# freudh/lbt

Measured on NVIDIA B200. Metric: quantized train imgs/sec, higher is better.
Workload: dtype s8/u8 mantissas, s32 accumulate (8-bit dfxp); fp32 master weights

## Files before the change

include/lbt.h:

```cpp
#ifndef LBT_H_
#define LBT_H_

#include <stddef.h>
#include <stdint.h>

#ifdef __cplusplus
extern "C" {
#endif

#define LBT_VERSION 100

enum lbt_status {
  LBT_OK = 0,
  LBT_EINVAL = -1,
  LBT_EUNSUPPORTED = -2,
  LBT_EARCH = -3,
  LBT_ECUDA = -4,
  LBT_EWORKSPACE = -5
};

enum lbt_round_mode {
  LBT_ROUND_NEAREST = 0,
  LBT_ROUND_STOCHASTIC_NOISE = 1,
  LBT_ROUND_STOCHASTIC_PHILOX = 2,
  LBT_STATS_MINMAX = 0x100
};

enum lbt_mant_kind {
  LBT_MANT_NONE = 0,
  LBT_MANT_S8 = 1,
  LBT_MANT_U8 = 2,
  LBT_MANT_S16 = 3,
  LBT_MANT_S9C3 = 4,
  LBT_MANT_PREPARED = 0x100
};

#define LBT_CNT_OVER 0
#define LBT_CNT_OVER_HALF 1
#define LBT_CNT_NUMEL 2
#define LBT_CNT_TICKET 3
#define LBT_CNT_WORDS 4

int lbt_version(void);
const char* lbt_strerror(int status);
const char* lbt_last_cuda_error(void);
uint64_t lbt_launch_count(void);

int lbt_quantize(const float* x, size_t n_outer, size_t n_inner, int bits, int32_t* integer_bits,
                 float target_overflow_rate, int mode, const float* noise, uint64_t seed,
                 uint64_t offset, const uint64_t* dev_step, float* out_fp32, void* out_mant,
                 int mant_kind, uint64_t* counters, int update_range, void* stream);

int lbt_noise_fill(float* u, size_t n_inner, uint64_t seed, uint64_t offset, const uint64_t* dev_step,
                   void* stream);

int lbt_update_ranges(int32_t* ranges, uint64_t* counters, const int32_t* bits, const float* target,
                      size_t n, void* stream);

int lbt_step_advance(uint64_t* dev_step, void* stream);

typedef struct lbt_qsite {
  int32_t bits;
  int32_t stats_minmax;
  const int32_t* ib;
  const float* noise;
  uint64_t seed, offset;
  const uint64_t* dev_step;
  uint64_t* counters;
} lbt_qsite;

enum lbt_gemm_epilogue {
  LBT_EPI_F32 = 0,
  LBT_EPI_ACC64 = 1
};

int lbt_gemm_i8(const void* A, int a_kind, size_t lda, const void* B, int b_kind, size_t ldb, size_t M,
                size_t N, size_t K, int epilogue, const int32_t* ibA, const int32_t* ibB, int exp_const,
                const float* bias, float* out_f32, int64_t* acc64, size_t ldc, int alpha, int k_splits,
                const lbt_qsite* q_out, int8_t* k_out, int64_t* sums, size_t rows_per_image, const float* addend,
                void* stream);

int lbt_gemm_i8_dual(const int8_t* A_hi, const uint8_t* A_lo, size_t lda, const void* B, int b_kind, size_t ldb, size_t M,
                     size_t N, size_t K, const int32_t* ibA, const int32_t* ibB, int exp_const, float* out_f32, size_t ldc,
                     const float* addend, void* stream);

int lbt_acc64_finalize(const int64_t* acc64, size_t n, const int32_t* ibA, const int32_t* ibB, int exp_const,
                       const float* add, float add_scale, float* out, void* stream);

int lbt_im2col_i8(const void* src, int src_kind, int N, int H, int W, int C, int OH, int OW, int kh, int kw,
                  int sh, int sw, int pad_top, int pad_left, int transposed, void* out, size_t ld,
                  void* stream);

int lbt_conv_i8_fprop(const void* src, int src_kind, int N, int H, int W, int C, const void* wp, int w_kind,
                      size_t ldw, int Cout, int kh, int kw, int sh, int sw, int pad_top, int pad_left, int OH,
                      int OW, const int32_t* ib_src, const int32_t* ib_w, int exp_const, const float* bias,
                      float* out, size_t ldc, const lbt_qsite* q_out, int8_t* k_out, int64_t* sums, const float* addend,
                      void* stream);

int lbt_conv_i8_fprop_dual(const int8_t* src_hi, const uint8_t* src_lo, int N, int H, int W, int C, const void* wp, int w_kind,
                           size_t ldw, int Cout, int kh, int kw, int pad_top, int pad_left, int OH, int OW,
                           const int32_t* ib_src, const int32_t* ib_w, int exp_const, float* out, size_t ldc,
                           const float* addend, void* stream);

int lbt_conv_i8_dgrad(const void* g, int g_kind, int N, int OH, int OW, int Cout, const void* wp, int w_kind,
                      size_t ldw, int Cin, int kh, int kw, int sh, int sw, int pad_top, int pad_left, int H, int W,
                      const int32_t* ib_g, const int32_t* ib_w, int exp_const, float* dx, size_t ldc, const float* addend,
                      void* stream);

int lbt_conv_i8_wgrad(const void* src, int src_kind, int N, int H, int W, int C, const void* g, int g_kind, int Cout,
                      int kh, int kw, int sh, int sw, int pad_top, int pad_left, int OH, int OW, int64_t* acc64,
                      int alpha, int k_splits, void* stream);

int lbt_conv_i8_wgrad_dual(const void* src, int src_kind, int N, int H, int W, int C, const int8_t* g_hi, const uint8_t* g_lo,
                           int Cout, int kh, int kw, int sh, int sw, int pad_top, int pad_left, int OH, int OW,
                           int64_t* acc64, int alpha, int k_splits, void* stream);

size_t lbt_stem_pack8_bytes(int N, int H, int OW);
int lbt_stem_pack8(const int8_t* x16, int N, int H, int W, int OW, int pad_left, int8_t* work8, void* stream);
int lbt_conv_i8_wgrad_c3(const int8_t* x16, int N, int H, int W, const void* g, int g_kind, int Cout, int kh, int kw,
                         int pad_top, int pad_left, int OH, int OW, int8_t* work8, int repack, int64_t* acc8, int alpha,
                         void* stream);

int lbt_split_s16(const int16_t* in, size_t n, int8_t* hi, uint8_t* lo, void* stream);

int lbt_transpose_i8(const void* in, size_t R, size_t C, size_t ld_in, void* out, size_t ld_out,
                     void* stream);

int lbt_colsum_i(const void* in, int kind, size_t R, size_t C, int64_t* acc64, void* stream);

typedef struct lbt_finalize_job {
  const int64_t* acc64;
  uint64_t n;
  const int32_t* ibA;
  const int32_t* ibB;
  int32_t exp_const;
  float add_scale;
  const float* add;
  float* out;
  uint64_t start;
} lbt_finalize_job;
int lbt_finalize_multi(const lbt_finalize_job* jobs_dev, size_t njobs, uint64_t total, void* stream);

typedef struct lbt_noise_job {
  float* u;
  uint64_t n;
  uint64_t offset;
  uint64_t start;
} lbt_noise_job;
int lbt_noise_fill_multi(const lbt_noise_job* jobs_dev, size_t njobs, uint64_t total_groups, uint64_t seed,
                         const uint64_t* dev_step, void* stream);

enum lbt_prep_layout { LBT_PREP_VECTOR = 0, LBT_PREP_CONV = 1, LBT_PREP_DENSE = 2 };
typedef struct lbt_prep_job {
  const float* x;
  uint64_t n_outer, n_inner;
  const int32_t* ib;
  uint64_t* counters;
  uint64_t offset;
  float* out_f32;
  int8_t* out_a;
  int8_t* out_b;
  uint64_t ld_a, ld_b;
  int32_t bits, layout;
  uint32_t kh, kw, Cin, Cout;
  int32_t c3pad, rot180;
  int32_t sh, sw;
} lbt_prep_job;
int lbt_param_prep(const lbt_prep_job* jobs_dev, const uint32_t* block_job_dev, const uint32_t* block_chunk_dev,
                   size_t nblocks, uint32_t chunk_elems, uint64_t seed, const uint64_t* dev_step, void* stream);

int lbt_sgd_momentum(float* w, float* accum, const float* grad, size_t n, float lr, const float* dev_lr,
                     float momentum, float grad_scale, void* stream);

int lbt_bn_fwd_quant_stats(const float* x, size_t n_outer, size_t n_inner, int C, int bits, const int32_t* ib,
                           const float* noise, uint64_t seed, uint64_t offset, const uint64_t* dev_step,
                           int8_t* k1, int64_t* sums, uint64_t* counters, int stats_minmax, void* stream);
int lbt_bn_fwd_apply(const int8_t* k1, size_t n_outer, size_t n_inner, int C, int bits1, const int32_t* ib1,
                     const int64_t* sums, float eps, int bits2, const int32_t* ib2, const float* noise2,
                     uint64_t seed, uint64_t offset2, const uint64_t* dev_step, uint64_t* counters2,
                     const float* gamma_q, const float* beta_q, const float* add, int relu, int8_t* k2,
                     float* out, float* batch_mean, float* batch_var, float* run_mean, float* run_var,
                     double momentum, int stats_minmax, const lbt_qsite* q_next, void* next_mant, int next_kind,
                     void* stream);
int lbt_bn_fwd_apply2(const int8_t* k1, size_t n_outer, size_t n_inner, int C, int bits1, const int32_t* ib1,
                      const int64_t* sums, float eps, int bits2, const int32_t* ib2, const float* noise2,
                      uint64_t seed, uint64_t offset2, const uint64_t* dev_step, uint64_t* counters2,
                      const float* gamma_q, const float* beta_q, const float* add, int relu, int8_t* k2,
                      float* out, float* batch_mean, float* batch_var, float* run_mean, float* run_var,
                      double momentum, int stats_minmax, const lbt_qsite* q_next, void* next_mant, int next_kind,
                      const lbt_qsite* q_next2, void* next_mant2, int next_kind2, void* stream);
int lbt_bn_fwd_apply_pooled(const int8_t* k1, size_t n_outer, int H, int W, int C, int bits1, const int32_t* ib1,
                            const int64_t* sums, float eps, int bits2, const int32_t* ib2, const float* noise2,
                            uint64_t seed, uint64_t offset2, const uint64_t* dev_step, uint64_t* counters2,
                            const float* gamma_q, const float* beta_q, int relu, int8_t* k2, float* run_mean,
                            float* run_var, double momentum, int stats_minmax, int k, int s, int pad_top, int pad_left,
                            int POH, int POW, float* pooled, uint8_t* pidx, const lbt_qsite* q_next, void* next_mant,
                            int next_kind, void* stream);
int lbt_bn_fwd_apply_running(const int8_t* k1, size_t n_outer, size_t n_inner, int C, int bits1, const int32_t* ib1,
                             const float* run_mean, const float* run_var, float eps, int bits2, const int32_t* ib2,
                             const float* noise2, uint64_t seed, uint64_t offset2, const uint64_t* dev_step,
                             uint64_t* counters2, const float* gamma_q, const float* beta_q, const float* add, int relu,
                             int8_t* k2, float* out, int stats_minmax, const lbt_qsite* q_next, void* next_mant,
                             int next_kind, const lbt_qsite* q_next2, void* next_mant2, int next_kind2, void* stream);
int lbt_bn_fwd_apply_running_pooled(const int8_t* k1, size_t n_outer, int H, int W, int C, int bits1, const int32_t* ib1,
                                    const float* run_mean, const float* run_var, float eps, int bits2, const int32_t* ib2,
                                    const float* noise2, uint64_t seed, uint64_t offset2, const uint64_t* dev_step,
                                    uint64_t* counters2, const float* gamma_q, const float* beta_q, int relu, int8_t* k2,
                                    int stats_minmax, int k, int s, int pad_top, int pad_left, int POH, int POW,
                                    float* pooled, uint8_t* pidx, const lbt_qsite* q_next, void* next_mant, int next_kind,
                                    void* stream);
int lbt_bn_bwd_quant_stats(const float* g, const float* out, int relu, const int8_t* k2, const int8_t* k1,
                           size_t n_outer, size_t n_inner, int C, int bits2, const int32_t* ib2,
                           const float* gamma_q, const float* beta_q, int bits_g2, const int32_t* ib_g2,
                           const float* noise_g2, uint64_t offset_g2, uint64_t* counters_g2, int bits_g1,
                           const int32_t* ib_g1, const float* noise_g1, uint64_t offset_g1,
                           uint64_t* counters_g1, uint64_t seed, const uint64_t* dev_step, float* d_add,
                           void* kg1, int64_t* sums, int stats_minmax, int kg1_kind, void* stream);
typedef struct lbt_pool_geom {
  const uint8_t* idx;
  int32_t H, W;
  int32_t k, s, pad_top, pad_left;
  int32_t OH, OW;
} lbt_pool_geom;
int lbt_bn_bwd_quant_stats_pooled(const float* g_pooled, const lbt_pool_geom* pool, int relu, const int8_t* k2,
                                  const int8_t* k1, size_t n_outer, size_t n_inner, int C, int bits2, const int32_t* ib2,
                                  const float* gamma_q, const float* beta_q, int bits_g2, const int32_t* ib_g2,
                                  const float* noise_g2, uint64_t offset_g2, uint64_t* counters_g2, int bits_g1,
                                  const int32_t* ib_g1, const float* noise_g1, uint64_t offset_g1,
                                  uint64_t* counters_g1, uint64_t seed, const uint64_t* dev_step, void* kg1,
                                  int64_t* sums, int stats_minmax, int kg1_kind, void* stream);
int lbt_bn_bwd_apply(const void* kg1, const int8_t* k1, size_t n_outer, size_t n_inner, int C, int bits1,
                     const int32_t* ib1, const int64_t* fwd_sums, float eps, int bits_g1, const int32_t* ib_g1,
                     const int64_t* bwd_sums, float* dx, const lbt_qsite* q_grad, int8_t* g_mant, int kg1_kind,
                     uint8_t* g_mant_lo, void* stream);

typedef struct lbt_bn_bwd_args {
  const float* g;
  const float* out;
  const int8_t* k2;
  const int8_t* k1;
  uint64_t n_outer, n_inner;
  int32_t C, relu;
  int32_t bits2, bits1;
  const int32_t* ib2;
  const int32_t* ib1;
  const float* gamma_q;
  const float* beta_q;
  lbt_qsite q_g2, q_g1;
  float* d_add;
  int64_t* bwd_sums;
  const int64_t* fwd_sums;
  float eps;
  int32_t has_q_grad;
  lbt_qsite q_grad;
  float* dx;
  int8_t* g_mant;
  uint64_t* barrier;
} lbt_bn_bwd_args;
int lbt_bn_bwd_fused(const lbt_bn_bwd_args* args, void* stream);

int lbt_maxpool_fwd(const float* x, int N, int H, int W, int C, int k, int s, int pad_top, int pad_left, int OH, int OW,
                    float* out, uint8_t* idx, void* stream);
int lbt_maxpool_bwd(const float* g, const uint8_t* idx, int N, int H, int W, int C, int k, int s, int pad_top,
                    int pad_left, int OH, int OW, float* dx, void* stream);

int lbt_avgpool_fwd(const float* x, int N, int H, int W, int C, int k, int s, int OH, int OW, float* out, void* stream);
int lbt_avgpool_bwd(const float* g, int N, int H, int W, int C, int k, int s, int OH, int OW, float* dx, void* stream);

int lbt_softmax_xent_fwd(const float* logits, const int64_t* labels, int B, int C, float* probs, float* loss, void* stream);
int lbt_softmax_xent_bwd(const float* probs, const int64_t* labels, const float* grad_loss, int B, int C, float* dlogits,
// ... 65 lines not shown
```

lbt_b200/_lib.py:

```python
import ctypes
import os

import torch

_HERE = os.path.dirname(os.path.abspath(__file__))
LIB_PATH = os.environ.get('LBT_LIB') or os.path.join(_HERE, 'liblbt_b200.so')

c_void_p, c_int, c_size_t, c_float = ctypes.c_void_p, ctypes.c_int, ctypes.c_size_t, ctypes.c_float
c_u64, c_char_p = ctypes.c_uint64, ctypes.c_char_p

SIGNATURES = {
    'lbt_version': (c_int, []),
    'lbt_strerror': (c_char_p, [c_int]),
    'lbt_last_cuda_error': (c_char_p, []),
    'lbt_launch_count': (c_u64, []),
    'lbt_quantize': (c_int, [c_void_p, c_size_t, c_size_t, c_int, c_void_p, c_float, c_int, c_void_p, c_u64, c_u64,
                             c_void_p, c_void_p, c_void_p, c_int, c_void_p, c_int, c_void_p]),
    'lbt_noise_fill': (c_int, [c_void_p, c_size_t, c_u64, c_u64, c_void_p, c_void_p]),
    'lbt_update_ranges': (c_int, [c_void_p, c_void_p, c_void_p, c_void_p, c_size_t, c_void_p]),
    'lbt_step_advance': (c_int, [c_void_p, c_void_p]),
    'lbt_gemm_i8': (c_int, [c_void_p, c_int, c_size_t, c_void_p, c_int, c_size_t, c_size_t, c_size_t, c_size_t, c_int,
                            c_void_p, c_void_p, c_int, c_void_p, c_void_p, c_void_p, c_size_t, c_int, c_int,
                            c_void_p, c_void_p, c_void_p, c_size_t, c_void_p, c_void_p]),
    'lbt_gemm_i8_dual': (c_int, [c_void_p, c_void_p, c_size_t, c_void_p, c_int, c_size_t, c_size_t, c_size_t, c_size_t, c_void_p,
                                 c_void_p, c_int, c_void_p, c_size_t, c_void_p, c_void_p]),
    'lbt_acc64_finalize': (c_int, [c_void_p, c_size_t, c_void_p, c_void_p, c_int, c_void_p, c_float, c_void_p,
                                   c_void_p]),
    'lbt_im2col_i8': (c_int, [c_void_p, c_int] + [c_int] * 13 + [c_void_p, c_size_t, c_void_p]),
    'lbt_conv_i8_fprop': (c_int, [c_void_p, c_int, c_int, c_int, c_int, c_int, c_void_p, c_int, c_size_t] + [c_int] * 9 +
                          [c_void_p, c_void_p, c_int, c_void_p, c_void_p, c_size_t, c_void_p, c_void_p, c_void_p, c_void_p,
                           c_void_p]),
    'lbt_conv_i8_fprop_dual': (c_int, [c_void_p, c_void_p, c_int, c_int, c_int, c_int, c_void_p, c_int, c_size_t] + [c_int] * 7 +
                               [c_void_p, c_void_p, c_int, c_void_p, c_size_t, c_void_p, c_void_p]),
    'lbt_conv_i8_dgrad': (c_int, [c_void_p, c_int, c_int, c_int, c_int, c_int, c_void_p, c_int, c_size_t] + [c_int] * 9 +
                          [c_void_p, c_void_p, c_int, c_void_p, c_size_t, c_void_p, c_void_p]),
    'lbt_conv_i8_wgrad': (c_int, [c_void_p, c_int, c_int, c_int, c_int, c_int, c_void_p, c_int] + [c_int] * 9 +
                          [c_void_p, c_int, c_int, c_void_p]),
    'lbt_conv_i8_wgrad_dual': (c_int, [c_void_p, c_int, c_int, c_int, c_int, c_int, c_void_p, c_void_p] + [c_int] * 9 +
                               [c_void_p, c_int, c_int, c_void_p]),
    'lbt_stem_pack8_bytes': (c_size_t, [c_int, c_int, c_int]),
    'lbt_stem_pack8': (c_int, [c_void_p, c_int, c_int, c_int, c_int, c_int, c_void_p, c_void_p]),
    'lbt_conv_i8_wgrad_c3': (c_int, [c_void_p, c_int, c_int, c_int, c_void_p] + [c_int] * 8 + [c_void_p, c_int, c_void_p, c_int, c_void_p]),
    'lbt_split_s16': (c_int, [c_void_p, c_size_t, c_void_p, c_void_p, c_void_p]),
    'lbt_transpose_i8': (c_int, [c_void_p, c_size_t, c_size_t, c_size_t, c_void_p, c_size_t, c_void_p]),
    'lbt_colsum_i': (c_int, [c_void_p, c_int, c_size_t, c_size_t, c_void_p, c_void_p]),
    'lbt_bn_bwd_fused': (c_int, [c_void_p, c_void_p]),
    'lbt_maxpool_fwd': (c_int, [c_void_p] + [c_int] * 10 + [c_void_p, c_void_p, c_void_p]),
    'lbt_maxpool_bwd': (c_int, [c_void_p, c_void_p] + [c_int] * 10 + [c_void_p, c_void_p]),
    'lbt_avgpool_fwd': (c_int, [c_void_p] + [c_int] * 8 + [c_void_p, c_void_p]),
    'lbt_avgpool_bwd': (c_int, [c_void_p] + [c_int] * 8 + [c_void_p, c_void_p]),
    'lbt_softmax_xent_fwd': (c_int, [c_void_p, c_void_p, c_int, c_int, c_void_p, c_void_p, c_void_p]),
    'lbt_softmax_xent_bwd': (c_int, [c_void_p, c_void_p, c_void_p, c_int, c_int, c_void_p, c_void_p]),
    'lbt_relu': (c_int, [c_void_p, c_void_p, c_void_p, c_size_t, c_void_p]),
    'lbt_dropout': (c_int, [c_void_p, c_void_p, c_float, c_u64, c_u64, c_void_p, c_void_p, c_size_t, c_void_p]),
    'lbt_sgd_momentum': (c_int, [c_void_p, c_void_p, c_void_p, c_size_t, c_float, c_void_p, c_float, c_float,
                                 c_void_p]),
    'lbt_finalize_multi': (c_int, [c_void_p, c_size_t, c_u64, c_void_p]),
    'lbt_noise_fill_multi': (c_int, [c_void_p, c_size_t, c_u64, c_u64, c_void_p, c_void_p]),
    'lbt_param_prep': (c_int, [c_void_p, c_void_p, c_void_p, c_size_t, ctypes.c_uint32, c_u64, c_void_p, c_void_p]),
    'lbt_bn_fwd_quant_stats': (c_int, [c_void_p, c_size_t, c_size_t, c_int, c_int, c_void_p, c_void_p, c_u64, c_u64,
                                       c_void_p, c_void_p, c_void_p, c_void_p, c_int, c_void_p]),
    'lbt_bn_fwd_apply': (c_int, [c_void_p, c_size_t, c_size_t, c_int, c_int, c_void_p, c_void_p, c_float, c_int,
                                 c_void_p, c_void_p, c_u64, c_u64, c_void_p, c_void_p, c_void_p, c_void_p, c_void_p,
                                 c_int, c_void_p, c_void_p, c_void_p, c_void_p, c_void_p, c_void_p, ctypes.c_double, c_int,
                                 c_void_p, c_void_p, c_int, c_void_p]),
    'lbt_bn_fwd_apply2': (c_int, [c_void_p, c_size_t, c_size_t, c_int, c_int, c_void_p, c_void_p, c_float, c_int,
                                  c_void_p, c_void_p, c_u64, c_u64, c_void_p, c_void_p, c_void_p, c_void_p, c_void_p,
                                  c_int, c_void_p, c_void_p, c_void_p, c_void_p, c_void_p, c_void_p, ctypes.c_double, c_int,
                                  c_void_p, c_void_p, c_int, c_void_p, c_void_p, c_int, c_void_p]),
    'lbt_bn_fwd_apply_pooled': (c_int, [c_void_p, c_size_t, c_int, c_int, c_int, c_int, c_void_p, c_void_p, c_float, c_int,
                                        c_void_p, c_void_p, c_u64, c_u64, c_void_p, c_void_p, c_void_p, c_void_p, c_int,
                                        c_void_p, c_void_p, c_void_p, ctypes.c_double, c_int, c_int, c_int, c_int, c_int,
                                        c_int, c_int, c_void_p, c_void_p, c_void_p, c_void_p, c_int, c_void_p]),
    'lbt_bn_fwd_apply_running': (c_int, [c_void_p, c_size_t, c_size_t, c_int, c_int, c_void_p, c_void_p, c_void_p, c_float, c_int,
                                         c_void_p, c_void_p, c_u64, c_u64, c_void_p, c_void_p, c_void_p, c_void_p, c_void_p, c_int,
                                         c_void_p, c_void_p, c_int, c_void_p, c_void_p, c_int, c_void_p, c_void_p, c_int, c_void_p]),
    'lbt_bn_fwd_apply_running_pooled': (c_int, [c_void_p, c_size_t, c_int, c_int, c_int, c_int, c_void_p, c_void_p, c_void_p,
                                                c_float, c_int, c_void_p, c_void_p, c_u64, c_u64, c_void_p, c_void_p, c_void_p,
                                                c_void_p, c_int, c_void_p, c_int, c_int, c_int, c_int, c_int, c_int, c_int,
                                                c_void_p, c_void_p, c_void_p, c_void_p, c_int, c_void_p]),
    'lbt_bn_bwd_quant_stats': (c_int, [c_void_p, c_void_p, c_int, c_void_p, c_void_p, c_size_t, c_size_t, c_int, c_int,
                                       c_void_p, c_void_p, c_void_p, c_int, c_void_p, c_void_p, c_u64, c_void_p, c_int,
                                       c_void_p, c_void_p, c_u64, c_void_p, c_u64, c_void_p, c_void_p, c_void_p,
                                       c_void_p, c_int, c_int, c_void_p]),
    'lbt_bn_bwd_quant_stats_pooled': (c_int, [c_void_p, c_void_p, c_int, c_void_p, c_void_p, c_size_t, c_size_t, c_int, c_int,
                                              c_void_p, c_void_p, c_void_p, c_int, c_void_p, c_void_p, c_u64, c_void_p, c_int,
                                              c_void_p, c_void_p, c_u64, c_void_p, c_u64, c_void_p, c_void_p,
                                              c_void_p, c_int, c_int, c_void_p]),
    'lbt_bn_bwd_apply': (c_int, [c_void_p, c_void_p, c_size_t, c_size_t, c_int, c_int, c_void_p, c_void_p, c_float,
                                 c_int, c_void_p, c_void_p, c_void_p, c_void_p, c_void_p, c_int, c_void_p, c_void_p]),
    'lbt_conv_i8_dgrad_strided_dual': (c_int, [c_void_p, c_void_p, c_int, c_int, c_int, c_int, c_void_p, c_int, c_size_t] + [c_int] * 9 +
                                       [c_void_p, c_void_p, c_int, c_void_p, c_size_t, c_void_p, c_void_p]),
    'lbt_conv_i8_dgrad_strided': (c_int, [c_void_p, c_int, c_int, c_int, c_int, c_int, c_void_p, c_int, c_size_t, c_int, c_int, c_int,
                                          c_int, c_int, c_int, c_int, c_int, c_int, c_void_p, c_void_p, c_int, c_void_p, c_size_t,
                                          c_void_p, c_void_p]),
    'lbt_dp_step': (c_int, [c_void_p, c_void_p, c_size_t, c_float, c_void_p, c_float, c_int, c_void_p, c_void_p, c_void_p,
                            c_size_t, c_void_p, c_void_p]),
    'lbt_dp_export': (c_int, [c_void_p, c_void_p, c_void_p]),
    'lbt_dp_open': (c_int, [c_void_p, c_void_p]),
    'lbt_dp_close': (c_int, [c_void_p]),
    'lbt_conv_i8_dgrad_bn': (c_int, [c_void_p, c_int, c_int, c_int, c_int, c_int, c_void_p, c_int, c_size_t] + [c_int] * 7 +
                             [c_void_p, c_void_p, c_int, c_void_p, c_void_p]),
    'lbt_quantize_residual': (c_int, [c_void_p, c_size_t, c_void_p, c_size_t, c_size_t, c_int, c_void_p, c_int, c_void_p, c_u64,
                                      c_u64, c_void_p, c_void_p, c_void_p, c_void_p]),
    'lbt_augment_batch': (c_int, [c_void_p, c_void_p, c_void_p, c_int, c_int, c_int, c_int, c_int, c_int, c_void_p, c_u64, c_u64,
                                  c_void_p, c_void_p, c_void_p, c_void_p]),
}

_INTERNAL = {
    'lbt_quantize_tune': (c_int, [c_int, c_int]),
    'lbt_gemm_debug_error': (c_int, []),
    'lbt_conv_debug_error': (c_int, []),
    'lbt_conv_ldg_debug_error': (c_int, []),
    'lbt_conv_set_path': (c_int, [c_int]),
    'lbt_conv_set_halo': (c_int, [c_int]),
    'lbt_conv_halo_launches': (ctypes.c_longlong, []),
    'lbt_gemm_set_pair': (c_int, [c_int]),
    'lbt_set_pdl': (c_int, [c_int]),
    'lbt_set_carveout': (c_int, [c_int]),
    'lbt_test_fdiv': (c_int, [c_u64, c_u64, c_void_p, c_void_p, c_void_p]),
    'lbt_bn_set_debug': (c_int, [c_void_p]),
    'lbt_conv_ldg_set_debug': (c_int, [c_void_p]),
    'lbt_dp_tune': (c_int, [c_int]),
    'lbt_dp_emulate_scratch_bytes': (c_size_t, [c_int]),
    'lbt_dp_step_emulate': (c_int, [c_int, c_void_p, c_void_p, c_size_t, c_float, c_void_p, c_float, c_int, c_void_p, c_void_p,
                                    c_void_p, c_size_t, c_void_p, c_void_p, c_void_p]),
    'lbt_bn_debug_error': (c_int, []),
}


class LbtError(RuntimeError):
    pass


class FinalizeJob(ctypes.Structure):
    _fields_ = [('acc64', c_void_p), ('n', c_u64), ('ibA', c_void_p), ('ibB', c_void_p), ('exp_const', ctypes.c_int32),
                ('add_scale', c_float), ('add', c_void_p), ('out', c_void_p), ('start', c_u64)]


class QSiteStruct(ctypes.Structure):
    _fields_ = [('bits', ctypes.c_int32), ('stats_minmax', ctypes.c_int32), ('ib', c_void_p), ('noise', c_void_p),
                ('seed', c_u64), ('offset', c_u64), ('dev_step', c_void_p), ('counters', c_void_p)]


class PoolGeom(ctypes.Structure):
    _fields_ = [('idx', c_void_p), ('H', ctypes.c_int32), ('W', ctypes.c_int32), ('k', ctypes.c_int32), ('s', ctypes.c_int32),
                ('pad_top', ctypes.c_int32), ('pad_left', ctypes.c_int32), ('OH', ctypes.c_int32), ('OW', ctypes.c_int32)]


class BnBwdLink(ctypes.Structure):
    _fields_ = [('q_g2', QSiteStruct), ('q_g1', QSiteStruct), ('bits2', ctypes.c_int32), ('relu', ctypes.c_int32), ('ib2', c_void_p),
                ('gamma_q', c_void_p), ('beta_q', c_void_p), ('k2', c_void_p), ('k1', c_void_p), ('kg1', c_void_p), ('sums', c_void_p)]


class BnBwdArgs(ctypes.Structure):
    _fields_ = [('g', c_void_p), ('out', c_void_p), ('k2', c_void_p), ('k1', c_void_p), ('n_outer', c_u64), ('n_inner', c_u64),
                ('C', ctypes.c_int32), ('relu', ctypes.c_int32), ('bits2', ctypes.c_int32), ('bits1', ctypes.c_int32),
                ('ib2', c_void_p), ('ib1', c_void_p), ('gamma_q', c_void_p), ('beta_q', c_void_p), ('q_g2', QSiteStruct),
                ('q_g1', QSiteStruct), ('d_add', c_void_p), ('bwd_sums', c_void_p), ('fwd_sums', c_void_p), ('eps', c_float),
                ('has_q_grad', ctypes.c_int32), ('q_grad', QSiteStruct), ('dx', c_void_p), ('g_mant', c_void_p),
                ('barrier', c_void_p)]


DP_MAX_WORLD, DP_PAD_WORDS, DP_PAD_ERROR, DP_HANDLE_BYTES = 8, 32, 18, 64


class DpPeers(ctypes.Structure):
    _fields_ = [('world', ctypes.c_int32), ('rank', ctypes.c_int32), ('grad', c_void_p * DP_MAX_WORLD),
                ('w', c_void_p * DP_MAX_WORLD), ('counters', c_void_p * DP_MAX_WORLD), ('pad', c_void_p * DP_MAX_WORLD)]


class NoiseJob(ctypes.Structure):
    _fields_ = [('u', c_void_p), ('n', c_u64), ('offset', c_u64), ('start', c_u64)]


class PrepJob(ctypes.Structure):
    _fields_ = [('x', c_void_p), ('n_outer', c_u64), ('n_inner', c_u64), ('ib', c_void_p), ('counters', c_void_p),
                ('offset', c_u64), ('out_f32', c_void_p), ('out_a', c_void_p), ('out_b', c_void_p), ('ld_a', c_u64),
                ('ld_b', c_u64), ('bits', ctypes.c_int32), ('layout', ctypes.c_int32), ('kh', ctypes.c_uint32),
                ('kw', ctypes.c_uint32), ('Cin', ctypes.c_uint32), ('Cout', ctypes.c_uint32), ('c3pad', ctypes.c_int32),
                ('rot180', ctypes.c_int32), ('sh', ctypes.c_int32), ('sw', ctypes.c_int32)]


def to_device_table(structs, device, keep=None):
    arr = (type(structs[0]) * len(structs))(*structs)
    host = torch.frombuffer(bytearray(bytes(arr)), dtype=torch.uint8).pin_memory()
    if keep is not None:
        keep.append(host)
    return host.to(device, non_blocking=True)


_lib = None


# ... 96 lines not shown
```

lbt_b200/csrc/conv_i8.cu:

```cuda
#include "conv_internal.h"
#include "qsite.cuh"
#include "tcgen05.cuh"

namespace lbt {
namespace {

using namespace tc;

constexpr int kBlockM = 128;
constexpr int kStageK = 128;
constexpr int kThreads = 192;
constexpr int kEpiWarps = 8;
constexpr int kThreadsF = 32 * (2 + kEpiWarps);

__device__ int g_conv_error = 0;

struct ConvParams {
  uint32_t M, N;
  uint32_t OW, OHW;
  FastDiv d_OW, d_OHW;
  int lower_w, lower_h;
  int sw, sh;
  uint32_t kw;
  uint32_t taps, cchunks;
// ... 442 lines not shown
      bool ok = true;
      for (uint32_t item = blockIdx.x; item < total_items && ok; item += gridDim.x) {
        const uint32_t ks = (item / p.m_tiles) / p.n_tiles;
        const uint32_t pb0 = ks * p.blocks_per_split, pb1 = min(pb0 + p.blocks_per_split, p.pix_blocks);
        if (!(ok = mbar_wait(&tmem_empty_bar[acc], acc_phase ^ 1, abort_flag, &g_conv_error))) break;
        fence_after();
        const uint32_t d_tmem = tmem_base + acc * C::kAccW;
        for (uint32_t pb = pb0; pb < pb1; ++pb) {
          if (!(ok = mbar_wait(&full_bar[stage], phase, abort_flag, &g_conv_error))) break;
          fence_after();
          const uint32_t sa = smem_u32(smem + stage * C::kStageBytes);
          const uint32_t sb = sa + C::kStageA;
#pragma unroll
          for (uint32_t kk = 0; kk < kBlockM / 32; ++kk) {
            const uint64_t da = make_desc_mnmajor(sa + kk * 32 * p.cb, (int)p.mode_a, a_block);
            umma_i8(d_tmem, da, make_desc_mnmajor(sb + kk * 32 * p.cbn, (int)p.mode_b, b_block), p.idesc, (pb > pb0 || kk > 0) ? 1u : 0u);
            if (DUAL)
              umma_i8(d_tmem + BN, da, make_desc_mnmajor(sb + C::kStageB1 + kk * 32 * p.cbn, (int)p.mode_b, b_block), p.idesc2,
                      (pb > pb0 || kk > 0) ? 1u : 0u);
          }
          umma_commit(&empty_bar[stage]);
          if (++stage == C::kStages) {
            stage = 0;
            phase ^= 1;
          }
        }
        if (!ok) break;
        umma_commit(&tmem_full_bar[acc]);
        if (++acc == C::kAccStages) {
          acc = 0;
          acc_phase ^= 1;
        }
      }
    }
  } else {
    const uint32_t quad = warp & 3;
    uint32_t acc = 0, acc_phase = 0;
    bool ok = true;
    for (uint32_t item = blockIdx.x; item < total_items && ok; item += gridDim.x) {
      const uint32_t m_tile = item % p.m_tiles, rest = item / p.m_tiles;
      const uint32_t n_tile = rest % p.n_tiles;
      ok = mbar_wait(&tmem_full_bar[acc], acc_phase, abort_flag, &g_conv_error);
      ok = __all_sync(0xffffffffu, ok);
      if (!ok) break;
      fence_after();
      const uint32_t row = m_tile * kBlockM + quad * 32 + lane;
      const uint32_t col0 = n_tile * BN;
      const uint32_t taddr = tmem_base + acc * C::kAccW + ((quad * 32u) << 16);
#pragma unroll 1
      for (int c = 0; c < BN; c += 16) {
        uint32_t v[16], w[DUAL ? 16 : 1];
        tmem_ld16(taddr + c, v);
        if constexpr (DUAL) tmem_ld16(taddr + BN + c, w);
        tmem_ld_wait();
        if (row < p.Kf && col0 + c < p.N) {
          const uint32_t ncol = min(16u, p.N - (col0 + c));
          unsigned long long* o = reinterpret_cast<unsigned long long*>(p.acc64) + (size_t)row * p.N + col0 + c;
#pragma unroll
          for (int j = 0; j < 16; ++j)
            if (j < (int)ncol) {
              long long a = (long long)(int)v[j];
              if constexpr (DUAL) a = a * 256ll + (long long)(int)w[j];
              a *= (long long)p.alpha;
              if (a != 0) atomicAdd(o + j, (unsigned long long)a);
            }
        }
      }
      fence_before();
      __syncwarp();
      if (lane == 0) mbar_arrive(&tmem_empty_bar[acc]);
      if (++acc == C::kAccStages) {
        acc = 0;
        acc_phase ^= 1;
      }
    }
  }

  fence_before();
  __syncthreads();
  fence_after();
  if (warp == 1) tmem_dealloc(tmem_base, C::kTmemCols);
}

typedef CUresult (*EncodeTiledFn)(CUtensorMap*, CUtensorMapDataType, cuuint32_t, void*, const cuuint64_t*, const cuuint64_t*,
                                  const cuuint32_t*, const cuuint32_t*, CUtensorMapInterleave, CUtensorMapSwizzle,
                                  CUtensorMapL2promotion, CUtensorMapFloatOOBfill);
typedef CUresult (*EncodeIm2colFn)(CUtensorMap*, CUtensorMapDataType, cuuint32_t, void*, const cuuint64_t*, const cuuint64_t*,
                                   const int*, const int*, cuuint32_t, cuuint32_t, const cuuint32_t*, CUtensorMapInterleave,
                                   CUtensorMapSwizzle, CUtensorMapL2promotion, CUtensorMapFloatOOBfill);

void* driver_fn(const char* name) {
  void* f = nullptr;
  cudaDriverEntryPointQueryResult q;
  if (cudaGetDriverEntryPoint(name, &f, cudaEnableDefault, &q) != cudaSuccess || q != cudaDriverEntryPointSuccess) return nullptr;
  return f;
}

CUtensorMapSwizzle swizzle_of(uint32_t mode) {
  switch (mode) {
    case 0: return CU_TENSOR_MAP_SWIZZLE_NONE;
    case 1: return CU_TENSOR_MAP_SWIZZLE_32B;
    case 2: return CU_TENSOR_MAP_SWIZZLE_64B;
    default: return CU_TENSOR_MAP_SWIZZLE_128B;
  }
}

template <int BN, bool DUAL = false>
int launch(const CUtensorMap& ta, const CUtensorMap& ta2, const CUtensorMap& tb, const ConvParams& p, unsigned grid, cudaStream_t st) {
  static bool attr_done[16] = {};
  const int dev = device_info().device;
  if (!attr_done[dev]) {
    cudaError_t e = cudaFuncSetAttribute(conv_fprop_kernel<BN, DUAL>, cudaFuncAttributeMaxDynamicSharedMemorySize, FCfg<BN, DUAL>::kSmemBytes);
    if (e != cudaSuccess) {
      set_cuda_error(e, "cudaFuncSetAttribute(conv_fprop_kernel)");
      return LBT_ECUDA;
    }
    attr_done[dev] = true;
  }
  launch_pdl(conv_fprop_kernel<BN, DUAL>, grid, kThreadsF, FCfg<BN, DUAL>::kSmemBytes, st, ta, ta2, tb, p);
  return check_launch(DUAL ? "lbt_conv_i8_fprop_dual" : "lbt_conv_i8_fprop");
}

}
}

using namespace lbt;

extern "C" int lbt_conv_i8_fprop(const void* src, int src_kind, int N, int H, int W, int C, const void* wp, int w_kind,
                                 size_t ldw, int Cout, int kh, int kw, int sh, int sw, int pad_top, int pad_left, int OH,
                                 int OW, const int32_t* ib_src, const int32_t* ib_w, int exp_const, const float* bias,
                                 float* out, size_t ldc, const lbt_qsite* q_out, int8_t* k_out, int64_t* sums,
                                 const float* addend, void* stream) {
  return conv_fprop_run(src, src_kind, N, H, W, C, wp, w_kind, ldw, Cout, kh, kw, sh, sw, pad_top, pad_left, OH, OW, ib_src, ib_w,
                        exp_const, bias, out, ldc, q_out, k_out, sums, addend, stream, nullptr, nullptr);
}

extern "C" int lbt_conv_i8_fprop_dual(const int8_t* src_hi, const uint8_t* src_lo, int N, int H, int W, int C, const void* wp, int w_kind,
                                      size_t ldw, int Cout, int kh, int kw, int pad_top, int pad_left, int OH, int OW,
                                      const int32_t* ib_src, const int32_t* ib_w, int exp_const, float* out, size_t ldc,
                                      const float* addend, void* stream) {
  if (!src_hi || !src_lo || !wp || !out) return LBT_EINVAL;
  if (ldc < (size_t)Cout) return LBT_EINVAL;
  return conv_fprop_run(src_hi, LBT_MANT_S8, N, H, W, C, wp, w_kind, ldw, Cout, kh, kw, 1, 1, pad_top, pad_left, OH, OW, ib_src, ib_w,
                        exp_const, nullptr, out, ldc, nullptr, nullptr, nullptr, addend, stream, nullptr, src_lo);
}

int lbt::conv_fprop_run(const void* src, int src_kind, int N, int H, int W, int C, const void* wp, int w_kind, size_t ldw, int Cout,
                        int kh, int kw, int sh, int sw, int pad_top, int pad_left, int OH, int OW, const int32_t* ib_src,
                        const int32_t* ib_w, int exp_const, const float* bias, float* out, size_t ldc, const lbt_qsite* q_out,
                        int8_t* k_out, int64_t* sums, const float* addend, void* stream, const OutRemap* remap, const void* src_lo) {
  const bool w_prepared = (w_kind & LBT_MANT_PREPARED) != 0;
  w_kind &= ~LBT_MANT_PREPARED;
  const bool dual = src_lo != nullptr;
  if (!src || !wp) return LBT_EINVAL;
  if (dual && (q_out || bias || !out || src_kind != LBT_MANT_S8 || (reinterpret_cast<uintptr_t>(src_lo) & 15))) return LBT_EUNSUPPORTED;
  if (q_out) {
    if (!k_out || !sums || !q_out->ib) return LBT_EINVAL;
    if (q_out->bits < 2 || q_out->bits > 8 || (Cout & 3)) return LBT_EUNSUPPORTED;
  } else if (!out) {
    return LBT_EINVAL;
  }
  if ((src_kind != LBT_MANT_S8 && src_kind != LBT_MANT_U8) || (w_kind != LBT_MANT_S8 && w_kind != LBT_MANT_U8)) return LBT_EINVAL;
  if (N <= 0 || H <= 0 || W <= 0 || C <= 0 || Cout <= 0 || kh <= 0 || kw <= 0 || sh <= 0 || sw <= 0 || OH <= 0 || OW <= 0)
    return LBT_EINVAL;
  if (C % 16) return LBT_EUNSUPPORTED;
  if (remap && q_out) return LBT_EINVAL;
  if (!dual && !remap && conv_ldg_enabled() && (C <= 32 || (C == 64 && conv_ldg_c64_halo() && conv_ldg_halo_applies(N, OH, OW, kh, kw, sh, sw, C))) &&
      conv_ldg_ok(C, Cout, kh, kw) && !(reinterpret_cast<uintptr_t>(src) & 15) &&
      !(reinterpret_cast<uintptr_t>(wp) & 15) && !(ldw & 15) && ldw >= (size_t)kh * kw * C && (q_out || ldc >= (size_t)Cout)) {
    LBT_REQUIRE_ARCH();
    return conv_ldg_run(src, src_kind, N, H, W, C, wp, w_kind, ldw, Cout, kh, kw, sh, sw, pad_top, pad_left, OH, OW, 0, ib_src,
                        ib_w, exp_const, bias, out, ldc, q_out, k_out, sums, addend, stream, nullptr, w_prepared);
  }
  const uint32_t cb = C >= 128 ? 128u : (uint32_t)C;
  if (cb != 16 && cb != 32 && cb != 64 && cb != 128) return LBT_EUNSUPPORTED;
  if (C % cb) return LBT_EUNSUPPORTED;
  if ((reinterpret_cast<uintptr_t>(src) & 15) || (reinterpret_cast<uintptr_t>(wp) & 15) || (ldw & 15)) return LBT_EUNSUPPORTED;
  if (!q_out && ldc < (size_t)Cout) return LBT_EINVAL;
  const size_t Ktot = (size_t)kh * kw * C;
  if (ldw < Ktot) return LBT_EINVAL;
  if (conv_halo_applies(N, OH, OW, C, Cout, kh, kw, sh, sw)) {
    LBT_REQUIRE_ARCH();
    const int rc = conv_halo_run(src, src_kind, N, H, W, C, wp, w_kind, ldw, Cout, kh, kw, pad_top, pad_left, OH, OW, ib_src, ib_w,
                                 exp_const, bias, out, ldc, q_out, k_out, sums, addend, stream, remap, src_lo);
    if (!(dual && rc == LBT_EUNSUPPORTED)) return rc;
  }
  if (Ktot > 65536) return LBT_EUNSUPPORTED;
  if (kh > 255 || kw > 255) return LBT_EUNSUPPORTED;
  LBT_REQUIRE_ARCH();
  const DeviceInfo& di = device_info();
  static EncodeTiledFn enc_tiled = reinterpret_cast<EncodeTiledFn>(driver_fn("cuTensorMapEncodeTiled"));
  static EncodeIm2colFn enc_im2col = reinterpret_cast<EncodeIm2colFn>(driver_fn("cuTensorMapEncodeIm2col"));
  if (!enc_tiled || !enc_im2col) return LBT_ECUDA;

  int bn = 256;
  for (int c : {16, 32, 64, 128, 256})
    if (c >= Cout) {
      bn = c;
      break;
    }
  if (dual && bn > 128) bn = 128;
  if (dual && bn < 64) return LBT_EUNSUPPORTED;
  uint32_t mode = 0;
  while ((16u << mode) < cb) ++mode;

  ConvParams p{};
  p.M = (uint32_t)((size_t)N * OH * OW);
  p.N = (uint32_t)Cout;
  p.OW = (uint32_t)OW;
  p.OHW = (uint32_t)(OH * OW);
  p.d_OW = make_fastdiv(p.OW);
  p.d_OHW = make_fastdiv(p.OHW);
  if ((size_t)N * OH * OW >= (1ull << 31)) return LBT_EUNSUPPORTED;
  p.lower_w = -pad_left;
  p.lower_h = -pad_top;
  p.sw = sw;
  p.sh = sh;
  p.kw = (uint32_t)kw;
  p.taps = (uint32_t)(kh * kw);
  p.cchunks = (uint32_t)C / cb;
  p.ksteps_real = p.taps * p.cchunks;
  p.ksteps = p.ksteps_real + ((cb == 16 && (p.ksteps_real & 1)) ? 1 : 0);
  p.cb = cb;
  p.mode = mode;
  p.C = (uint32_t)C;
  p.m_tiles = (p.M + kBlockM - 1) / kBlockM;
  p.n_tiles = ((uint32_t)Cout + bn - 1) / bn;
  p.ibA = ib_src;
  p.ibB = ib_w;
  p.exp_const = exp_const;
  p.bias = bias;
  p.addend = q_out ? nullptr : addend;
  p.out = out;
  p.ldc = ldc;
  p.idesc = tc::make_idesc_i8(src_kind == LBT_MANT_S8, w_kind == LBT_MANT_S8, false, false, bn, kBlockM);
  p.idesc2 = tc::make_idesc_i8(false, w_kind == LBT_MANT_S8, false, false, bn, kBlockM);
  p.bnq.q = site_from_abi(q_out);
  p.bnq.k = k_out;
  p.bnq.sums = reinterpret_cast<long long*>(sums);
  p.bnq.rows_per_image = (uint32_t)(OH * OW);
  if (remap) {
    p.remap = 1;
    p.rs_n = remap->sn;
    p.rs_y = remap->sy;
    p.rs_x = remap->sx;
  }

  CUtensorMap ta, ta2, tb;
  {
    cuuint64_t gdim[4] = {(cuuint64_t)C, (cuuint64_t)W, (cuuint64_t)H, (cuuint64_t)N};
    cuuint64_t gstr[3] = {(cuuint64_t)C, (cuuint64_t)W * C, (cuuint64_t)H * W * C};
    const int upper_w = (OW - 1) * sw + 1 - W - pad_left;
    const int upper_h = (OH - 1) * sh + 1 - H - pad_top;
    int lower[2] = {-pad_left, -pad_top};
    int upper[2] = {upper_w, upper_h};
    cuuint32_t estr[4] = {1, (cuuint32_t)sw, (cuuint32_t)sh, 1};
    CUresult r = enc_im2col(&ta, CU_TENSOR_MAP_DATA_TYPE_UINT8, 4, const_cast<void*>(src), gdim, gstr, lower, upper, cb, kBlockM,
                            estr, CU_TENSOR_MAP_INTERLEAVE_NONE, swizzle_of(mode), CU_TENSOR_MAP_L2_PROMOTION_L2_128B,
                            CU_TENSOR_MAP_FLOAT_OOB_FILL_NONE);
    if (r != CUDA_SUCCESS) {
      set_cuda_error(cudaErrorInvalidValue, "cuTensorMapEncodeIm2col");
      return LBT_ECUDA;
    }
    ta2 = ta;
    if (dual) {
      r = enc_im2col(&ta2, CU_TENSOR_MAP_DATA_TYPE_UINT8, 4, const_cast<void*>(src_lo), gdim, gstr, lower, upper, cb, kBlockM,
                     estr, CU_TENSOR_MAP_INTERLEAVE_NONE, swizzle_of(mode), CU_TENSOR_MAP_L2_PROMOTION_L2_128B,
                     CU_TENSOR_MAP_FLOAT_OOB_FILL_NONE);
      if (r != CUDA_SUCCESS) {
        set_cuda_error(cudaErrorInvalidValue, "cuTensorMapEncodeIm2col(low plane)");
        return LBT_ECUDA;
      }
    }
  }
  {
    cuuint64_t gdim[2] = {(cuuint64_t)Ktot, (cuuint64_t)Cout};
    cuuint64_t gstr[1] = {(cuuint64_t)ldw};
    cuuint32_t box[2] = {cb, (cuuint32_t)bn};
    cuuint32_t estr[2] = {1, 1};
    CUresult r = enc_tiled(&tb, CU_TENSOR_MAP_DATA_TYPE_UINT8, 2, const_cast<void*>(wp), gdim, gstr, box, estr,
                           CU_TENSOR_MAP_INTERLEAVE_NONE, swizzle_of(mode), CU_TENSOR_MAP_L2_PROMOTION_L2_256B,
                           CU_TENSOR_MAP_FLOAT_OOB_FILL_NONE);
    if (r != CUDA_SUCCESS) {
      set_cuda_error(cudaErrorInvalidValue, "cuTensorMapEncodeTiled(weights)");
      return LBT_ECUDA;
    }
  }
  const uint64_t tiles = (uint64_t)p.m_tiles * p.n_tiles;
  const uint64_t cap = (uint64_t)di.sm_count * (dual ? 1 : ctas_per_sm(bn));
  const unsigned grid = (unsigned)(tiles < cap ? tiles : cap);
  cudaStream_t st = reinterpret_cast<cudaStream_t>(stream);
  if (dual) return bn == 64 ? launch<64, true>(ta, ta2, tb, p, grid, st) : launch<128, true>(ta, ta2, tb, p, grid, st);
  switch (bn) {
    case 16: return launch<16>(ta, ta2, tb, p, grid, st);
    case 32: return launch<32>(ta, ta2, tb, p, grid, st);
    case 64: return launch<64>(ta, ta2, tb, p, grid, st);
    case 128: return launch<128>(ta, ta2, tb, p, grid, st);
    default: return launch<256>(ta, ta2, tb, p, grid, st);
  }
}

namespace lbt {
namespace {
template <int BN, bool DUAL = false>
int launch_wgrad(const CUtensorMap& tx, const CUtensorMap& tg, const CUtensorMap& tg2, const WgradParams& p, unsigned grid, cudaStream_t st) {
  static bool attr_done[16] = {};
// ... 174 lines not shown
```

lbt_b200/csrc/conv_internal.h:

```cpp
#pragma once

#include <stddef.h>
#include <stdint.h>

#include "../../include/lbt.h"

namespace lbt {

struct OutRemap {
  long long sn, sy, sx;
};

bool conv_ldg_ok(int C, int Cout, int kh, int kw);
bool conv_ldg_enabled();
bool conv_ldg_halo_applies(int N, int OH, int OW, int kh, int kw, int sh, int sw, int C);
int conv_ldg_c64_halo();
int conv_ldg_run(const void* src, int src_kind, int N, int SH, int SW, int C, const void* wp, int w_kind, size_t ldw, int Cout,
                 int kh, int kw, int sh, int sw, int pt, int pl, int OH, int OW, int gather, const int32_t* ibA,
                 const int32_t* ibB, int exp_const, const float* bias, float* out, size_t ldc, const lbt_qsite* q_out,
                 int8_t* k_out, int64_t* sums, const float* addend, void* stream, const lbt_bn_bwd_link* link = nullptr,
                 bool w_prepared = false);

bool conv_halo_applies(int N, int OH, int OW, int C, int Cout, int kh, int kw, int sh, int sw);
void conv_halo_enable(int mode);
int conv_halo_debug_error();
int conv_stem_debug_error();
int conv_halo_run(const void* src, int src_kind, int N, int H, int W, int C, const void* wp, int w_kind, size_t ldw, int Cout, int kh,
                  int kw, int pt, int pl, int OH, int OW, const int32_t* ibA, const int32_t* ibB, int exp_const, const float* bias,
                  float* out, size_t ldc, const lbt_qsite* q_out, int8_t* k_out, int64_t* sums, const float* addend, void* stream,
                  const OutRemap* remap = nullptr, const void* src_lo = nullptr);
int conv_fprop_run(const void* src, int src_kind, int N, int H, int W, int C, const void* wp, int w_kind, size_t ldw, int Cout, int kh,
                   int kw, int sh, int sw, int pad_top, int pad_left, int OH, int OW, const int32_t* ib_src, const int32_t* ib_w,
                   int exp_const, const float* bias, float* out, size_t ldc, const lbt_qsite* q_out, int8_t* k_out, int64_t* sums,
                   const float* addend, void* stream, const OutRemap* remap, const void* src_lo = nullptr);

bool conv_wgrad_ldg_ok(int C, int Cout, int kh, int kw);
int conv_wgrad_ldg_run(const void* src, int src_kind, int N, int H, int W, int C, const void* g, int g_kind, int Cout, int kh, int kw,
                       int sh, int sw, int pt, int pl, int OH, int OW, int64_t* acc64, int alpha, void* stream);

}
```

lbt_b200/csrc/conv_stem.cu:

```cuda
#include <atomic>

#include "conv_internal.h"
#include "tcgen05.cuh"

namespace lbt {
namespace {

using namespace tc;

constexpr int kPix = 128;
constexpr int kPatchOH = 8, kPatchOW = 16;
constexpr int kRowBytes = 64;
constexpr int kBlock = kPix * kRowBytes;
constexpr int kTapRows = 8;
constexpr int kStemStages = 3;
constexpr int kStemThreads = 192;

__device__ int g_stem_error = 0;

struct StemParams {
  uint32_t patches, per_cta;
  uint32_t tiles_x, tiles_img;
  FastDiv d_tiles_x, d_tiles_img;
  int pt;
  uint32_t kh, kw, N;
  long long* acc8;
  int alpha;
  uint32_t idesc;
};

__device__ __forceinline__ void tma_load_tiled_4d(const CUtensorMap* map, uint64_t* bar, void* dst, int c0, int c1, int c2, int c3) {
  asm volatile(
      "cp.async.bulk.tensor.4d.shared::cluster.global.mbarrier::complete_tx::bytes [%0], [%1, {%3, %4, %5, %6}], [%2];" ::"r"(
          smem_u32(dst)),
      "l"(reinterpret_cast<uint64_t>(map)), "r"(smem_u32(bar)), "r"(c0), "r"(c1), "r"(c2), "r"(c3)
      : "memory");
}
__device__ __forceinline__ void tma_load_tiled_5d(const CUtensorMap* map, uint64_t* bar, void* dst, int c0, int c1, int c2, int c3, int c4) {
  asm volatile(
      "cp.async.bulk.tensor.5d.shared::cluster.global.mbarrier::complete_tx::bytes [%0], [%1, {%3, %4, %5, %6, %7}], [%2];" ::"r"(
          smem_u32(dst)),
      "l"(reinterpret_cast<uint64_t>(map)), "r"(smem_u32(bar)), "r"(c0), "r"(c1), "r"(c2), "r"(c3), "r"(c4)
      : "memory");
}

__global__ void __launch_bounds__(256) stem_pack8_kernel(const uint4* __restrict__ x16, int H, int W, int Wp, int ml, size_t total,
                                                         uint2* __restrict__ out) {
  pdl_trigger();
  pdl_wait();
  for (size_t i = (size_t)blockIdx.x * 256 + threadIdx.x; i < total; i += (size_t)gridDim.x * 256) {
    const size_t row = i / (size_t)Wp;
    const int wp = (int)(i - row * (size_t)Wp), w = wp - ml;
    uint2 o = make_uint2(0u, 0u);
    if (w >= 0 && w < W) {
      const uint4 v = __ldcs(x16 + row * (size_t)W + w);
      o.x = v.x & 0x00ffffffu;
      o.y = (v.y >> 16) | ((v.z & 0xffu) << 16);
    }
    out[i] = o;
  }
}

template <int BN>
__global__ void __launch_bounds__(kStemThreads, 1)
stem_wgrad_kernel(const __grid_constant__ CUtensorMap tmX, const __grid_constant__ CUtensorMap tmG, const StemParams p) {
  constexpr int kStageBytes = kTapRows * kBlock + kBlock;
  constexpr int kTmemCols = 4 * BN;
  extern __shared__ uint8_t smem_raw[];
  uint8_t* smem = reinterpret_cast<uint8_t*>((reinterpret_cast<uintptr_t>(smem_raw) + 1023) & ~uintptr_t(1023));
  __shared__ __align__(8) uint64_t full_bar[kStemStages];
  __shared__ __align__(8) uint64_t empty_bar[kStemStages];
  __shared__ __align__(8) uint64_t done_bar;
  __shared__ uint32_t tmem_slot;
  __shared__ int s_abort;

  const int warp = threadIdx.x >> 5, lane = threadIdx.x & 31;
  if (threadIdx.x == 0) {
    for (int s = 0; s < kStemStages; ++s) {
      mbar_init(&full_bar[s], 1);
      mbar_init(&empty_bar[s], 1);
    }
    mbar_init(&done_bar, 1);
    s_abort = 0;
    fence_barrier_init();
    tma_prefetch_desc(&tmX);
    tma_prefetch_desc(&tmG);
  }
  if (warp == 1) tmem_alloc(&tmem_slot, kTmemCols);
  pdl_trigger();
  fence_before();
  __syncthreads();
  fence_after();
  pdl_wait();
  const uint32_t tmem_base = *reinterpret_cast<volatile uint32_t*>(&tmem_slot);
  volatile int* abort_flag = &s_abort;

  const uint32_t p0 = blockIdx.x * p.per_cta, p1 = min(p0 + p.per_cta, p.patches);
  const bool has_work = p0 < p1;

  if (warp == 0) {
    if (lane == 0) {
      uint32_t stage = 0, phase = 0;
      bool ok = true;
      for (uint32_t pa = p0; pa < p1 && ok; ++pa) {
        if (!(ok = mbar_wait(&empty_bar[stage], phase ^ 1, abort_flag, &g_stem_error))) break;
        uint8_t* sa = smem + (size_t)stage * kStageBytes;
        uint8_t* sb = sa + kTapRows * kBlock;
        const uint32_t img = fastdiv(pa, p.d_tiles_img), t2 = pa - img * p.tiles_img;
        const uint32_t ty = fastdiv(t2, p.d_tiles_x), tx = t2 - ty * p.tiles_x;
        const int oh0 = (int)ty * kPatchOH, ow0 = (int)tx * kPatchOW;
        mbar_expect_tx(&full_bar[stage], (p.kh + 1) * (uint32_t)kBlock);
        for (uint32_t r = 0; r < p.kh; ++r) {
          const int d = (int)r - p.pt;
          tma_load_tiled_5d(&tmX, &full_bar[stage], sa + r * kBlock, 0, ow0, d & 1, oh0 + (d >> 1), (int)img);
        }
        tma_load_tiled_4d(&tmG, &full_bar[stage], sb, 0, ow0, oh0, (int)img);
        if (++stage == kStemStages) {
          stage = 0;
          phase ^= 1;
        }
      }
    }
  } else if (warp == 1) {
    if (lane == 0 && has_work) {
      uint32_t stage = 0, phase = 0;
      bool ok = true;
      for (uint32_t pa = p0; pa < p1 && ok; ++pa) {
        if (!(ok = mbar_wait(&full_bar[stage], phase, abort_flag, &g_stem_error))) break;
        fence_after();
        const uint32_t sa = smem_u32(smem + (size_t)stage * kStageBytes);
        const uint32_t sb = sa + kTapRows * kBlock;
#pragma unroll
        for (uint32_t t = 0; t < 4; ++t) {
          if (2 * t >= p.kh) break;
#pragma unroll
          for (uint32_t kk = 0; kk < kPix / 32; ++kk) {
            umma_i8(tmem_base + t * BN, make_desc_mnmajor(sa + 2 * t * kBlock + kk * 32 * kRowBytes, 2, kBlock),
                    make_desc_mnmajor(sb + kk * 32 * kRowBytes, 2, kBlock), p.idesc, (pa > p0 || kk > 0) ? 1u : 0u);
          }
        }
        umma_commit(&empty_bar[stage]);
        if (++stage == kStemStages) {
          stage = 0;
          phase ^= 1;
        }
      }
      if (ok) umma_commit(&done_bar);
    }
  } else if (has_work) {
    const uint32_t quad = warp & 3;
    bool ok = mbar_wait(&done_bar, 0, abort_flag, &g_stem_error);
    ok = __all_sync(0xffffffffu, ok);
    if (ok) {
      fence_after();
      const uint32_t m = quad * 32 + lane;
      const uint32_t b = m & 7u, s = (m >> 3) & 7u;
      for (uint32_t t = 0; t < 4; ++t) {
        const uint32_t r = 2 * t + (m >> 6);
        const bool real = r < p.kh && s < p.kw && (b & 3u) != 3u;
        const uint32_t taddr = tmem_base + t * BN + ((quad * 32u) << 16);
#pragma unroll 1
        for (int c = 0; c < BN; c += 16) {
          uint32_t v[16];
          tmem_ld16(taddr + c, v);
          tmem_ld_wait();
          if (real && (uint32_t)c < p.N) {
            unsigned long long* o = reinterpret_cast<unsigned long long*>(p.acc8) + (size_t)(t * 128 + m) * p.N + c;
            const uint32_t ncol = min(16u, p.N - (uint32_t)c);
#pragma unroll
            for (int j = 0; j < 16; ++j)
              if (j < (int)ncol && v[j] != 0u) atomicAdd(o + j, (unsigned long long)((long long)(int)v[j] * (long long)p.alpha));
          }
        }
      }
    }
  }

  fence_before();
  __syncthreads();
  fence_after();
  if (warp == 1) tmem_dealloc(tmem_base, kTmemCols);
}

typedef CUresult (*EncodeTiledFn)(CUtensorMap*, CUtensorMapDataType, cuuint32_t, void*, const cuuint64_t*, const cuuint64_t*,
                                  const cuuint32_t*, const cuuint32_t*, CUtensorMapInterleave, CUtensorMapSwizzle,
                                  CUtensorMapL2promotion, CUtensorMapFloatOOBfill);

void* stem_driver_fn(const char* name) {
  void* f = nullptr;
  cudaDriverEntryPointQueryResult q;
  if (cudaGetDriverEntryPoint(name, &f, cudaEnableDefault, &q) != cudaSuccess || q != cudaDriverEntryPointSuccess) return nullptr;
  return f;
}

}
}

using namespace lbt;

extern "C" size_t lbt_stem_pack8_bytes(int N, int H, int OW) {
  if (N <= 0 || H <= 0 || OW <= 0) return 0;
  return (size_t)N * H * (size_t)(2 * OW + 6) * 8;
}

extern "C" int lbt_stem_pack8(const int8_t* x16, int N, int H, int W, int OW, int pad_left, int8_t* work8, void* stream) {
  if (!x16 || !work8) return LBT_EINVAL;
  if (N <= 0 || H <= 0 || W <= 0 || OW <= 0 || pad_left < 0) return LBT_EINVAL;
  const int Wp = 2 * OW + 6;
  if (pad_left + W > Wp) return LBT_EUNSUPPORTED;
  if ((reinterpret_cast<uintptr_t>(x16) & 15) || (reinterpret_cast<uintptr_t>(work8) & 15)) return LBT_EUNSUPPORTED;
  LBT_REQUIRE_ARCH();
  const size_t total = (size_t)N * H * Wp;
  const size_t blocks = (total + 255) / 256, cap = (size_t)device_info().sm_count * 16;
  launch_pdl(stem_pack8_kernel, (unsigned)(blocks < cap ? blocks : cap), 256, 0, reinterpret_cast<cudaStream_t>(stream),
             reinterpret_cast<const uint4*>(x16), H, W, Wp, pad_left, total, reinterpret_cast<uint2*>(work8));
  return check_launch("lbt_stem_pack8");
}

extern "C" int lbt_conv_i8_wgrad_c3(const int8_t* x16, int N, int H, int W, const void* g, int g_kind, int Cout, int kh, int kw,
                                    int pad_top, int pad_left, int OH, int OW, int8_t* work8, int repack, int64_t* acc8, int alpha,
                                    void* stream) {
  if (!x16 || !g || !work8 || !acc8) return LBT_EINVAL;
  if (g_kind != LBT_MANT_S8 && g_kind != LBT_MANT_U8) return LBT_EINVAL;
  if (N <= 0 || H <= 0 || W <= 0 || Cout <= 0 || kh <= 0 || kw <= 0 || OH <= 0 || OW <= 0 || pad_top < 0 || pad_left < 0) return LBT_EINVAL;
  if (kh > 8 || kw > 8 || Cout != 64 || (H & 1)) return LBT_EUNSUPPORTED;
  const int Wp = 2 * OW + 6;
  if (pad_left + W > Wp || 2 * (OW - 1) + kw > Wp) return LBT_EUNSUPPORTED;
  if ((reinterpret_cast<uintptr_t>(x16) & 15) || (reinterpret_cast<uintptr_t>(g) & 15) || (reinterpret_cast<uintptr_t>(work8) & 15))
    return LBT_EUNSUPPORTED;
  LBT_REQUIRE_ARCH();
  const DeviceInfo& di = device_info();
  static EncodeTiledFn enc_tiled = reinterpret_cast<EncodeTiledFn>(stem_driver_fn("cuTensorMapEncodeTiled"));
  if (!enc_tiled) return LBT_ECUDA;
  cudaStream_t st = reinterpret_cast<cudaStream_t>(stream);

  StemParams p{};
  p.tiles_x = (uint32_t)((OW + kPatchOW - 1) / kPatchOW);
  const uint32_t tiles_y = (uint32_t)((OH + kPatchOH - 1) / kPatchOH);
  p.tiles_img = p.tiles_x * tiles_y;
  if ((uint64_t)N * p.tiles_img >= (1ull << 31)) return LBT_EUNSUPPORTED;
  p.patches = (uint32_t)N * p.tiles_img;
  const uint32_t ctas = (uint32_t)di.sm_count;
  p.per_cta = (p.patches + ctas - 1) / ctas;
  if (p.per_cta > 65536 / kPix) return LBT_EUNSUPPORTED;
  p.d_tiles_x = make_fastdiv(p.tiles_x);
  p.d_tiles_img = make_fastdiv(p.tiles_img);
  p.pt = pad_top;
  p.kh = (uint32_t)kh;
  p.kw = (uint32_t)kw;
  p.N = (uint32_t)Cout;
  p.acc8 = reinterpret_cast<long long*>(acc8);
  p.alpha = alpha;
  p.idesc = tc::make_idesc_i8(true, g_kind == LBT_MANT_S8, true, true, 64, 128);

  if (repack) {
    int rc = lbt_stem_pack8(x16, N, H, W, OW, pad_left, work8, stream);
    if (rc) return rc;
  }
  CUtensorMap tx, tg;
  const size_t pitch = (size_t)Wp * 8;
  {
    cuuint64_t gdim[5] = {64, (cuuint64_t)OW, 2, (cuuint64_t)(H / 2), (cuuint64_t)N};
    cuuint64_t gstr[4] = {16, (cuuint64_t)pitch, (cuuint64_t)(2 * pitch), (cuuint64_t)((size_t)H * pitch)};
    cuuint32_t box[5] = {64, (cuuint32_t)kPatchOW, 1, (cuuint32_t)kPatchOH, 1};
    cuuint32_t estr[5] = {1, 1, 1, 1, 1};
    CUresult r = enc_tiled(&tx, CU_TENSOR_MAP_DATA_TYPE_UINT8, 5, work8, gdim, gstr, box, estr, CU_TENSOR_MAP_INTERLEAVE_NONE,
                           CU_TENSOR_MAP_SWIZZLE_64B, CU_TENSOR_MAP_L2_PROMOTION_L2_128B, CU_TENSOR_MAP_FLOAT_OOB_FILL_NONE);
    if (r != CUDA_SUCCESS) return LBT_EUNSUPPORTED;
  }
  {
    cuuint64_t gdim[4] = {64, (cuuint64_t)OW, (cuuint64_t)OH, (cuuint64_t)N};
    cuuint64_t gstr[3] = {64, (cuuint64_t)OW * 64, (cuuint64_t)OH * OW * 64};
    cuuint32_t box[4] = {64, (cuuint32_t)kPatchOW, (cuuint32_t)kPatchOH, 1};
    cuuint32_t estr[4] = {1, 1, 1, 1};
    CUresult r = enc_tiled(&tg, CU_TENSOR_MAP_DATA_TYPE_UINT8, 4, const_cast<void*>(g), gdim, gstr, box, estr,
                           CU_TENSOR_MAP_INTERLEAVE_NONE, CU_TENSOR_MAP_SWIZZLE_64B, CU_TENSOR_MAP_L2_PROMOTION_L2_128B,
                           CU_TENSOR_MAP_FLOAT_OOB_FILL_NONE);
    if (r != CUDA_SUCCESS) return LBT_EUNSUPPORTED;
  }
  constexpr size_t smem = (size_t)kStemStages * (kTapRows + 1) * kBlock + 1024;
  static bool attr_done[16] = {};
  if (!attr_done[di.device]) {
    cudaError_t e = cudaFuncSetAttribute(stem_wgrad_kernel<64>, cudaFuncAttributeMaxDynamicSharedMemorySize, (int)smem);
    if (e != cudaSuccess) {
      set_cuda_error(e, "cudaFuncSetAttribute(stem_wgrad_kernel)");
      return LBT_ECUDA;
    }
    attr_done[di.device] = true;
  }
  const unsigned grid = (p.patches + p.per_cta - 1) / p.per_cta;
  launch_pdl(stem_wgrad_kernel<64>, grid, kStemThreads, smem, st, tx, tg, p);
  return check_launch("lbt_conv_i8_wgrad_c3");
}

namespace lbt {
int conv_stem_debug_error() {
  int v = 0, zero = 0;
  if (cudaMemcpyFromSymbol(&v, g_stem_error, sizeof(int)) != cudaSuccess) return -1;
  cudaMemcpyToSymbol(g_stem_error, &zero, sizeof(int));
  return v;
}
}
```

lbt_b200/csrc/quantize.cu:

```cuda
#include "common.cuh"

namespace lbt {

namespace {

constexpr int kThreads = 256;
constexpr int kRowsUnroll = 8;

int g_blocks_per_sm = 8;
int g_rows_per_group = 32;

struct QParams {
  const float* x;
  size_t n_outer, n_inner;
  int bits;
  int32_t* ib;
  float target;
  const float* noise;
  uint64_t seed, offset;
  const uint64_t* dev_step;
  float* out;
  void* mant;
  int mant_kind;
  unsigned long long* counters;
  int update_range;
  uint32_t n_vec, chunks, rows_per_group;
  uint64_t total_tiles;
};

struct QConst {
  float m, inv_m, L, hi, half;
};

__device__ __forceinline__ QConst make_const(int bits, int ib) {
  QConst c;
  int f = bits - ib - 1;
  f = max(-126, min(126, f));
  c.m = exp2i(f);
  c.inv_m = exp2i(-f);
  c.L = exp2i(bits - 1);
  c.hi = c.L - 1.0f;
  c.half = c.L * 0.5f;
  return c;
}

template <int MODE>
__device__ __forceinline__ float quant1(float x, float u, const QConst& c, uint32_t& n1, uint32_t& n2) {
  const float y = __fmul_rn(x, c.m);
  n1 += (uint32_t)(y >= c.L) + (uint32_t)(y < -c.L);
  n2 += (uint32_t)(y >= c.half) + (uint32_t)(y < -c.half);
  float k;
  if (MODE == LBT_ROUND_NEAREST) {
    k = rintf(fminf(fmaxf(y, -c.L), c.hi));
  } else {
    const float t = __fadd_rn(y, u);
    k = floorf(fminf(fmaxf(t, -c.L), c.hi));
  }
  return k;
}

template <int MODE>
__device__ __forceinline__ float quant1_mm(float x, float u, const QConst& c, float& mx, float& mn) {
  const float y = __fmul_rn(x, c.m);
  mx = fmaxf(mx, y);
  mn = fminf(mn, y);
  if (MODE == LBT_ROUND_NEAREST) return rintf(fminf(fmaxf(y, -c.L), c.hi));
  return floorf(fminf(fmaxf(__fadd_rn(y, u), -c.L), c.hi));
}

__device__ __forceinline__ void finish_stats(uint32_t n1, uint32_t n2, const QParams& p, int ib_at_launch) {
  if (p.counters == nullptr) return;
  __shared__ uint32_t s1[kThreads / 32], s2[kThreads / 32];
  n1 = warp_sum(n1);
  n2 = warp_sum(n2);
  const int lane = threadIdx.x & 31, w = threadIdx.x >> 5;
  if (lane == 0) {
    s1[w] = n1;
    s2[w] = n2;
  }
  __syncthreads();
  if (threadIdx.x == 0) {
    uint32_t b1 = 0, b2 = 0;
#pragma unroll
    for (int i = 0; i < kThreads / 32; ++i) {
      b1 += s1[i];
      b2 += s2[i];
    }
    unsigned long long* c = p.counters;
    if (b1) atomicAdd(c + LBT_CNT_OVER, (unsigned long long)b1);
    if (b2) atomicAdd(c + LBT_CNT_OVER_HALF, (unsigned long long)b2);
    __threadfence();
    const unsigned long long t = atomicAdd(c + LBT_CNT_TICKET, 1ull);
    if (t == (unsigned long long)gridDim.x - 1ull) {
      __threadfence();
      const unsigned long long numel =
          atomicAdd(c + LBT_CNT_NUMEL, 0ull) + (unsigned long long)p.n_outer * (unsigned long long)p.n_inner;
      if (p.update_range) {
        const unsigned long long c1 = atomicAdd(c + LBT_CNT_OVER, 0ull);
        const unsigned long long c2 = atomicAdd(c + LBT_CNT_OVER_HALF, 0ull);
        const float n = (float)(numel ? numel : 1ull);
        const float r1 = __fdiv_rn((float)c1, n), r2 = __fdiv_rn((float)c2, n);
        const int delta = (r1 > p.target) ? 1 : ((r2 <= p.target) ? -1 : 0);
        *p.ib = min(p.bits - 1, ib_at_launch + delta);
        c[LBT_CNT_OVER] = 0ull;
        c[LBT_CNT_OVER_HALF] = 0ull;
        c[LBT_CNT_NUMEL] = 0ull;
      } else {
        c[LBT_CNT_NUMEL] = numel;
      }
      c[LBT_CNT_TICKET] = 0ull;
    }
  }
}

__device__ __forceinline__ void store_mant4(void* mant, int kind, size_t idx, float k0, float k1, float k2, float k3) {
  const int i0 = __float2int_rn(k0), i1 = __float2int_rn(k1), i2 = __float2int_rn(k2), i3 = __float2int_rn(k3);
  if (kind == LBT_MANT_S16) {
    uint2 v;
    v.x = (uint32_t)(i0 & 0xffff) | ((uint32_t)(i1 & 0xffff) << 16);
    v.y = (uint32_t)(i2 & 0xffff) | ((uint32_t)(i3 & 0xffff) << 16);
    *reinterpret_cast<uint2*>(reinterpret_cast<int16_t*>(mant) + idx) = v;
  } else {
    const uint32_t v = (uint32_t)(i0 & 0xff) | ((uint32_t)(i1 & 0xff) << 8) | ((uint32_t)(i2 & 0xff) << 16) |
                       ((uint32_t)(i3 & 0xff) << 24);
    *reinterpret_cast<uint32_t*>(reinterpret_cast<uint8_t*>(mant) + idx) = v;
  }
}

template <int MODE, bool MM>
__global__ void __launch_bounds__(kThreads) quantize_vec_kernel(const QParams p) {
  pdl_trigger();
  pdl_wait();
  const int ib = *reinterpret_cast<volatile const int32_t*>(p.ib);
  const QConst c = make_const(p.bits, ib);
  uint64_t off = p.offset;
  if (MODE == LBT_ROUND_STOCHASTIC_PHILOX && p.dev_step) off += (*p.dev_step) << 32;
  uint32_t n1 = 0, n2 = 0;
  float mx = -INFINITY, mn = INFINITY;

  for (uint64_t tile = blockIdx.x; tile < p.total_tiles; tile += gridDim.x) {
    const uint32_t rg = (uint32_t)(tile / p.chunks), ch = (uint32_t)(tile % p.chunks);
    const uint32_t v = ch * kThreads + threadIdx.x;
    if (v >= p.n_vec) continue;
    float4 u = make_float4(0.f, 0.f, 0.f, 0.f);
    if (MODE == LBT_ROUND_STOCHASTIC_NOISE) u = __ldg(reinterpret_cast<const float4*>(p.noise) + v);
    if (MODE == LBT_ROUND_STOCHASTIC_PHILOX) u = philox_noise4(v, p.seed, off);
    const size_t r0 = (size_t)rg * p.rows_per_group;
    const size_t r1 = min(r0 + (size_t)p.rows_per_group, p.n_outer);
    for (size_t r = r0; r < r1; r += kRowsUnroll) {
      float4 xv[kRowsUnroll];
#pragma unroll
      for (int i = 0; i < kRowsUnroll; ++i)
        if (r + i < r1) xv[i] = __ldcs(reinterpret_cast<const float4*>(p.x + (r + i) * p.n_inner) + v);
#pragma unroll
      for (int i = 0; i < kRowsUnroll; ++i) {
        if (r + i < r1) {
          float k0, k1, k2, k3;
          if (MM) {
            k0 = quant1_mm<MODE>(xv[i].x, u.x, c, mx, mn);
            k1 = quant1_mm<MODE>(xv[i].y, u.y, c, mx, mn);
            k2 = quant1_mm<MODE>(xv[i].z, u.z, c, mx, mn);
            k3 = quant1_mm<MODE>(xv[i].w, u.w, c, mx, mn);
          } else {
            k0 = quant1<MODE>(xv[i].x, u.x, c, n1, n2);
            k1 = quant1<MODE>(xv[i].y, u.y, c, n1, n2);
            k2 = quant1<MODE>(xv[i].z, u.z, c, n1, n2);
            k3 = quant1<MODE>(xv[i].w, u.w, c, n1, n2);
          }
          const size_t idx = (r + i) * p.n_inner + 4 * (size_t)v;
          if (p.out)
            *reinterpret_cast<float4*>(p.out + idx) =
                make_float4(k0 * c.inv_m, k1 * c.inv_m, k2 * c.inv_m, k3 * c.inv_m);
          if (p.mant) store_mant4(p.mant, p.mant_kind, idx, k0, k1, k2, k3);
        }
      }
    }
  }
  if (MM) {
    n1 = (mx >= c.L || mn < -c.L) ? 1u : 0u;
    n2 = (mx >= c.half || mn < -c.half) ? 1u : 0u;
  }
  finish_stats(n1, n2, p, ib);
}

template <int MODE>
__global__ void __launch_bounds__(kThreads) quantize_scalar_kernel(const QParams p) {
  const int ib = *reinterpret_cast<volatile const int32_t*>(p.ib);
  const QConst c = make_const(p.bits, ib);
  uint64_t off = p.offset;
  if (MODE == LBT_ROUND_STOCHASTIC_PHILOX && p.dev_step) off += (*p.dev_step) << 32;
  uint32_t n1 = 0, n2 = 0;
  const size_t n = p.n_outer * p.n_inner;
  for (size_t i = (size_t)blockIdx.x * kThreads + threadIdx.x; i < n; i += (size_t)gridDim.x * kThreads) {
    const size_t col = i % p.n_inner;
    float u = 0.f;
    if (MODE == LBT_ROUND_STOCHASTIC_NOISE) u = __ldg(p.noise + col);
    if (MODE == LBT_ROUND_STOCHASTIC_PHILOX) {
      const float4 u4 = philox_noise4(col >> 2, p.seed, off);
      const int l = (int)(col & 3);
      u = l == 0 ? u4.x : (l == 1 ? u4.y : (l == 2 ? u4.z : u4.w));
    }
    const float k = quant1<MODE>(p.x[i], u, c, n1, n2);
    if (p.out) p.out[i] = k * c.inv_m;
    if (p.mant) {
      const int ki = __float2int_rn(k);
      if (p.mant_kind == LBT_MANT_S16)
        reinterpret_cast<int16_t*>(p.mant)[i] = (int16_t)ki;
      else
        reinterpret_cast<uint8_t*>(p.mant)[i] = (uint8_t)(ki & 0xff);
    }
  }
  finish_stats(n1, n2, p, ib);
}

template <int MODE>
__global__ void __launch_bounds__(kThreads) quantize_c3_kernel(const QParams p) {
  const int ib = *reinterpret_cast<volatile const int32_t*>(p.ib);
  const QConst c = make_const(p.bits, ib);
  uint64_t off = p.offset;
  if (MODE == LBT_ROUND_STOCHASTIC_PHILOX && p.dev_step) off += (*p.dev_step) << 32;
  uint32_t n1 = 0, n2 = 0;
  const size_t ppr = p.n_inner / 3, npix = p.n_outer * ppr;
  for (size_t pix = (size_t)blockIdx.x * kThreads + threadIdx.x; pix < npix; pix += (size_t)gridDim.x * kThreads) {
    const size_t row = pix / ppr, j0 = (pix % ppr) * 3;
    int k[3];
#pragma unroll
    for (int ch = 0; ch < 3; ++ch) {
      const size_t col = j0 + ch;
      float u = 0.f;
      if (MODE == LBT_ROUND_STOCHASTIC_NOISE) u = __ldg(p.noise + col);
      if (MODE == LBT_ROUND_STOCHASTIC_PHILOX) {
        const float4 u4 = philox_noise4(col >> 2, p.seed, off);
        const int l = (int)(col & 3);
        u = l == 0 ? u4.x : (l == 1 ? u4.y : (l == 2 ? u4.z : u4.w));
      }
      k[ch] = __float2int_rn(quant1<MODE>(p.x[row * p.n_inner + col], u, c, n1, n2));
    }
    uint32_t w[4] = {0, 0, 0, 0};
    uint8_t b[16];
#pragma unroll
    for (int i = 0; i < 16; ++i) b[i] = 0;
#pragma unroll
    for (int ch = 0; ch < 3; ++ch) {
      b[ch] = b[3 + ch] = (uint8_t)((k[ch] >> 1) & 0xff);
      b[6 + ch] = (uint8_t)(k[ch] & 1);
    }
#pragma unroll
    for (int i = 0; i < 16; ++i) w[i >> 2] |= (uint32_t)b[i] << (8 * (i & 3));
    reinterpret_cast<uint4*>(p.mant)[pix] = make_uint4(w[0], w[1], w[2], w[3]);
  }
  finish_stats(n1, n2, p, ib);
}

template <int MODE>
__global__ void __launch_bounds__(kThreads) quantize_c3v_kernel(const QParams p) {
  pdl_trigger();
  pdl_wait();
  const int ib = *reinterpret_cast<volatile const int32_t*>(p.ib);
  const QConst c = make_const(p.bits, ib);
  uint64_t off = p.offset;
  if (MODE == LBT_ROUND_STOCHASTIC_PHILOX && p.dev_step) off += (*p.dev_step) << 32;
  uint32_t n1 = 0, n2 = 0;
  const uint32_t nv4 = (uint32_t)(p.n_inner / 4);
  for (uint64_t tile = blockIdx.x; tile < p.total_tiles; tile += gridDim.x) {
    const uint32_t rg = (uint32_t)(tile / p.chunks), v = (uint32_t)(tile % p.chunks) * kThreads + threadIdx.x;
    if (v >= p.n_vec) continue;
    float u[12];
#pragma unroll
    for (int g = 0; g < 3; ++g) {
      float4 t = make_float4(0.f, 0.f, 0.f, 0.f);
      if (MODE == LBT_ROUND_STOCHASTIC_NOISE) t = __ldg(reinterpret_cast<const float4*>(p.noise) + 3 * (size_t)v + g);
      if (MODE == LBT_ROUND_STOCHASTIC_PHILOX) t = philox_noise4(3ull * v + g, p.seed, off);
      u[4 * g] = t.x; u[4 * g + 1] = t.y; u[4 * g + 2] = t.z; u[4 * g + 3] = t.w;
    }
    const uint32_t r0 = rg * p.rows_per_group, r1 = min(r0 + p.rows_per_group, (uint32_t)p.n_outer);
    for (uint32_t r = r0; r < r1; ++r) {
      const float4* xr = reinterpret_cast<const float4*>(p.x) + ((size_t)r * nv4 + 3 * (size_t)v);
      const float4 a = __ldcs(xr), b = __ldcs(xr + 1), d = __ldcs(xr + 2);
      const float xs[12] = {a.x, a.y, a.z, a.w, b.x, b.y, b.z, b.w, d.x, d.y, d.z, d.w};
      int k[12];
#pragma unroll
      for (int i = 0; i < 12; ++i) k[i] = __float2int_rn(quant1<MODE>(xs[i], u[i], c, n1, n2));
      uint4* o = reinterpret_cast<uint4*>(p.mant) + ((size_t)r * (nv4 / 3) * 4 + 4 * (size_t)v);
#pragma unroll
      for (int q = 0; q < 4; ++q) {
        const uint32_t h0 = (uint32_t)(k[3 * q] >> 1) & 0xffu, h1 = (uint32_t)(k[3 * q + 1] >> 1) & 0xffu,
                       h2 = (uint32_t)(k[3 * q + 2] >> 1) & 0xffu;
        const uint32_t l0 = (uint32_t)k[3 * q] & 1u, l1 = (uint32_t)k[3 * q + 1] & 1u, l2 = (uint32_t)k[3 * q + 2] & 1u;
        o[q] = make_uint4(h0 | (h1 << 8) | (h2 << 16) | (h0 << 24), h1 | (h2 << 8) | (l0 << 16) | (l1 << 24), l2, 0u);
      }
    }
  }
  finish_stats(n1, n2, p, ib);
}

template <int MODE>
__global__ void __launch_bounds__(kThreads) quantize_residual_kernel(const QParams p, float* __restrict__ buffer, size_t n_grad_rows) {
  const int ib = *reinterpret_cast<volatile const int32_t*>(p.ib);
  const QConst c = make_const(p.bits, ib);
  uint64_t off = p.offset;
  if (MODE == LBT_ROUND_STOCHASTIC_PHILOX && p.dev_step) off += (*p.dev_step) << 32;
  uint32_t n1 = 0, n2 = 0;
  const size_t n = p.n_outer * p.n_inner, n_grad = n_grad_rows * p.n_inner;
  for (size_t i = (size_t)blockIdx.x * kThreads + threadIdx.x; i < n; i += (size_t)gridDim.x * kThreads) {
    const size_t col = i % p.n_inner;
    float u = 0.f;
    if (MODE == LBT_ROUND_STOCHASTIC_NOISE) u = __ldg(p.noise + col);
    if (MODE == LBT_ROUND_STOCHASTIC_PHILOX) {
      const float4 u4 = philox_noise4(col >> 2, p.seed, off);
      const int l = (int)(col & 3);
      u = l == 0 ? u4.x : (l == 1 ? u4.y : (l == 2 ? u4.z : u4.w));
    }
    const float total = __fadd_rn(i < n_grad ? p.x[i] : 0.f, buffer[i]);
    const float q = quant1<MODE>(total, u, c, n1, n2) * c.inv_m;
    buffer[i] = __fsub_rn(total, q);
    if (i < n_grad) p.out[i] = q;
  }
  finish_stats(n1, n2, p, ib);
}

__global__ void noise_fill_kernel(float* u, size_t n_inner, uint64_t seed, uint64_t offset, const uint64_t* dev_step) {
  uint64_t off = offset;
  if (dev_step) off += (*dev_step) << 32;
  const size_t ng = (n_inner + 3) / 4;
  for (size_t g = (size_t)blockIdx.x * blockDim.x + threadIdx.x; g < ng; g += (size_t)gridDim.x * blockDim.x) {
    const float4 v = philox_noise4(g, seed, off);
    const size_t j = 4 * g;
    if (j + 0 < n_inner) u[j + 0] = v.x;
    if (j + 1 < n_inner) u[j + 1] = v.y;
    if (j + 2 < n_inner) u[j + 2] = v.z;
    if (j + 3 < n_inner) u[j + 3] = v.w;
  }
}

__global__ void update_ranges_kernel(int32_t* ranges, unsigned long long* counters, const int32_t* bits,
                                     const float* target, size_t n) {
  const size_t i = (size_t)blockIdx.x * blockDim.x + threadIdx.x;
  if (i >= n) return;
  unsigned long long* c = counters + i * LBT_CNT_WORDS;
  const unsigned long long numel = c[LBT_CNT_NUMEL];
  if (numel == 0ull) return;
  const float nn = (float)numel;
  const float r1 = __fdiv_rn((float)c[LBT_CNT_OVER], nn), r2 = __fdiv_rn((float)c[LBT_CNT_OVER_HALF], nn);
  const float t = target ? target[i] : 0.f;
  const int delta = (r1 > t) ? 1 : ((r2 <= t) ? -1 : 0);
  ranges[i] = min(bits[i] - 1, ranges[i] + delta);
  c[LBT_CNT_OVER] = 0ull;
  c[LBT_CNT_OVER_HALF] = 0ull;
  c[LBT_CNT_NUMEL] = 0ull;
  c[LBT_CNT_TICKET] = 0ull;
}

__global__ void step_advance_kernel(uint64_t* s) { *s += 1; }

inline bool aligned16(const void* p) { return (reinterpret_cast<uintptr_t>(p) & 15u) == 0; }

}

}

using namespace lbt;

extern "C" int lbt_quantize_tune(int blocks_per_sm, int rows_per_group) {
  if (blocks_per_sm > 0) g_blocks_per_sm = blocks_per_sm;
  if (rows_per_group > 0) g_rows_per_group = rows_per_group;
  return LBT_OK;
}

extern "C" int lbt_quantize(const float* x, size_t n_outer, size_t n_inner, int bits, int32_t* integer_bits,
                            float target_overflow_rate, int mode, const float* noise, uint64_t seed, uint64_t offset,
                            const uint64_t* dev_step, float* out_fp32, void* out_mant, int mant_kind,
                            uint64_t* counters, int update_range, void* stream) {
  if (!x || !integer_bits) return LBT_EINVAL;
  if (bits < 1 || bits > 31) return LBT_EINVAL;
  const bool minmax = (mode & LBT_STATS_MINMAX) != 0 && target_overflow_rate == 0.0f && counters != nullptr;
  mode &= ~LBT_STATS_MINMAX;
  if (mode < 0 || mode > 2) return LBT_EINVAL;
  if (mode == LBT_ROUND_STOCHASTIC_NOISE && !noise) return LBT_EINVAL;
  if (!out_fp32 && !out_mant && !counters) return LBT_EINVAL;
  if (out_mant && (mant_kind < LBT_MANT_S8 || mant_kind > LBT_MANT_S9C3)) return LBT_EINVAL;
  if (mant_kind == LBT_MANT_S9C3 && (bits > 9 || n_inner % 3 != 0 || out_fp32 || (reinterpret_cast<uintptr_t>(out_mant) & 15)))
    return LBT_EINVAL;
  if (!out_mant) mant_kind = LBT_MANT_NONE;
  if (mant_kind == LBT_MANT_S8 && bits > 8) return LBT_EINVAL;
  if (mant_kind == LBT_MANT_U8 && bits > 9) return LBT_EINVAL;
  if (mant_kind == LBT_MANT_S16 && bits > 16) return LBT_EINVAL;
  if (update_range && !counters) return LBT_EINVAL;
  if (n_outer == 0 || n_inner == 0) return LBT_OK;
  LBT_REQUIRE_ARCH();
  const DeviceInfo& di = device_info();
  cudaStream_t st = reinterpret_cast<cudaStream_t>(stream);

  QParams p{};
  p.x = x;
  p.n_outer = n_outer;
  p.n_inner = n_inner;
  p.bits = bits;
  p.ib = integer_bits;
  p.target = target_overflow_rate;
  p.noise = noise;
  p.seed = seed;
  p.offset = offset;
  p.dev_step = dev_step;
  p.out = out_fp32;
  p.mant = out_mant;
  p.mant_kind = mant_kind;
  p.counters = reinterpret_cast<unsigned long long*>(counters);
  p.update_range = update_range;

  const bool vec = (n_inner % 4 == 0) && (n_inner / 4 < 0xffffffffull) && aligned16(x) && (!out_fp32 || aligned16(out_fp32)) &&
                   (!out_mant || aligned16(out_mant)) && (mode != LBT_ROUND_STOCHASTIC_NOISE || aligned16(noise));
  const uint64_t cap = (uint64_t)di.sm_count * (uint64_t)g_blocks_per_sm;
  if (mant_kind == LBT_MANT_S9C3 && vec && n_inner % 12 == 0 && n_outer < (1ull << 31)) {
    p.n_vec = (uint32_t)(n_inner / 12);
    p.chunks = (p.n_vec + kThreads - 1) / kThreads;
    uint64_t groups = ((uint64_t)di.sm_count * 8 + p.chunks - 1) / p.chunks;
    if (groups > (n_outer + 3) / 4) groups = (n_outer + 3) / 4;
    if (groups < 1) groups = 1;
    const uint64_t rpg = (n_outer + groups - 1) / groups;
    p.rows_per_group = (uint32_t)rpg;
    p.total_tiles = (uint64_t)p.chunks * ((n_outer + rpg - 1) / rpg);
    const unsigned grid = (unsigned)(p.total_tiles < cap ? p.total_tiles : cap);
    switch (mode) {
      case LBT_ROUND_NEAREST: launch_pdl(quantize_c3v_kernel<0>, grid, kThreads, 0, st, p); break;
      case LBT_ROUND_STOCHASTIC_NOISE: launch_pdl(quantize_c3v_kernel<1>, grid, kThreads, 0, st, p); break;
      default: launch_pdl(quantize_c3v_kernel<2>, grid, kThreads, 0, st, p); break;
    }
    return check_launch("lbt_quantize(c3, 4 pixels per thread)");
  }
  if (mant_kind == LBT_MANT_S9C3) {
    const uint64_t npix = (uint64_t)n_outer * (n_inner / 3);
    const uint64_t blocks = (npix + kThreads - 1) / kThreads;
    const unsigned grid = (unsigned)(blocks < cap ? blocks : cap);
    switch (mode) {
      case LBT_ROUND_NEAREST: quantize_c3_kernel<0><<<grid, kThreads, 0, st>>>(p); break;
      case LBT_ROUND_STOCHASTIC_NOISE: quantize_c3_kernel<1><<<grid, kThreads, 0, st>>>(p); break;
      default: quantize_c3_kernel<2><<<grid, kThreads, 0, st>>>(p); break;
    }
    return check_launch("lbt_quantize(c3)");
  }
  if (vec) {
    p.n_vec = (uint32_t)(n_inner / 4);
    p.chunks = (p.n_vec + kThreads - 1) / kThreads;
    void (*kern)(const QParams) = nullptr;
    switch (mode) {
      case LBT_ROUND_NEAREST: kern = minmax ? quantize_vec_kernel<0, true> : quantize_vec_kernel<0, false>; break;
      case LBT_ROUND_STOCHASTIC_NOISE: kern = minmax ? quantize_vec_kernel<1, true> : quantize_vec_kernel<1, false>; break;
      default: kern = minmax ? quantize_vec_kernel<2, true> : quantize_vec_kernel<2, false>; break;
    }
    static int occ_cache[16][3][2] = {};
    int& occ = occ_cache[di.device][mode][minmax ? 1 : 0];
    if (occ == 0) {
      int n = 0;
      if (cudaOccupancyMaxActiveBlocksPerMultiprocessor(&n, kern, kThreads, 0) != cudaSuccess || n < 1) n = 1;
      occ = n;
    }
    const uint64_t wave = (uint64_t)di.sm_count * (uint64_t)(g_blocks_per_sm < occ ? g_blocks_per_sm : occ);
    uint64_t rpg, grid64;
    const uint64_t big_tiles = (uint64_t)p.chunks * ((n_outer + g_rows_per_group - 1) / g_rows_per_group);
    if (big_tiles >= 4 * wave) {
      rpg = (uint64_t)g_rows_per_group;
      grid64 = (uint64_t)di.sm_count * (uint64_t)g_blocks_per_sm;
    } else {
      uint64_t groups = wave / p.chunks;
      if (groups < 1) groups = 1;
      if (groups > n_outer) groups = n_outer;
      rpg = (n_outer + groups - 1) / groups;
      grid64 = wave;
    }
    p.rows_per_group = (uint32_t)rpg;
    p.total_tiles = (uint64_t)p.chunks * ((n_outer + rpg - 1) / rpg);
    const unsigned grid = (unsigned)(p.total_tiles < grid64 ? p.total_tiles : grid64);
    launch_pdl(kern, grid, kThreads, 0, st, p);
  } else {
    const uint64_t n = (uint64_t)n_outer * n_inner;
    const uint64_t blocks = (n + kThreads - 1) / kThreads;
    const unsigned grid = (unsigned)(blocks < cap ? blocks : cap);
    switch (mode) {
      case LBT_ROUND_NEAREST: quantize_scalar_kernel<0><<<grid, kThreads, 0, st>>>(p); break;
      case LBT_ROUND_STOCHASTIC_NOISE: quantize_scalar_kernel<1><<<grid, kThreads, 0, st>>>(p); break;
      default: quantize_scalar_kernel<2><<<grid, kThreads, 0, st>>>(p); break;
    }
  }
  return check_launch("lbt_quantize");
}

extern "C" int lbt_quantize_residual(const float* grad, size_t n_grad_rows, float* buffer, size_t n_outer, size_t n_inner, int bits,
                                     int32_t* integer_bits, int mode, const float* noise, uint64_t seed, uint64_t offset,
                                     const uint64_t* dev_step, float* out, uint64_t* counters, void* stream) {
  if (!buffer || !integer_bits || (n_grad_rows && (!grad || !out))) return LBT_EINVAL;
  if (bits < 1 || bits > 31 || mode < 0 || mode > 2 || n_grad_rows > n_outer) return LBT_EINVAL;
  if (mode == LBT_ROUND_STOCHASTIC_NOISE && !noise) return LBT_EINVAL;
  if (n_outer == 0 || n_inner == 0) return LBT_OK;
  LBT_REQUIRE_ARCH();
  const DeviceInfo& di = device_info();
  QParams p{};
  p.x = grad;
  p.n_outer = n_outer;
  p.n_inner = n_inner;
  p.bits = bits;
  p.ib = integer_bits;
  p.noise = noise;
  p.seed = seed;
  p.offset = offset;
  p.dev_step = dev_step;
  p.out = out;
  p.counters = reinterpret_cast<unsigned long long*>(counters);
  const uint64_t n = (uint64_t)n_outer * n_inner, blocks = (n + kThreads - 1) / kThreads;
  const uint64_t cap = (uint64_t)di.sm_count * 8;
  const unsigned grid = (unsigned)(blocks < cap ? blocks : cap);
  cudaStream_t st = reinterpret_cast<cudaStream_t>(stream);
  switch (mode) {
    case LBT_ROUND_NEAREST: quantize_residual_kernel<0><<<grid, kThreads, 0, st>>>(p, buffer, n_grad_rows); break;
    case LBT_ROUND_STOCHASTIC_NOISE: quantize_residual_kernel<1><<<grid, kThreads, 0, st>>>(p, buffer, n_grad_rows); break;
    default: quantize_residual_kernel<2><<<grid, kThreads, 0, st>>>(p, buffer, n_grad_rows); break;
  }
  return check_launch("lbt_quantize_residual");
}

extern "C" int lbt_noise_fill(float* u, size_t n_inner, uint64_t seed, uint64_t offset, const uint64_t* dev_step,
                              void* stream) {
  if (!u) return LBT_EINVAL;
  if (n_inner == 0) return LBT_OK;
  LBT_REQUIRE_ARCH();
  const size_t ng = (n_inner + 3) / 4;
  const unsigned grid = (unsigned)((ng + 255) / 256 < 4096 ? (ng + 255) / 256 : 4096);
  noise_fill_kernel<<<grid, 256, 0, reinterpret_cast<cudaStream_t>(stream)>>>(u, n_inner, seed, offset, dev_step);
  return check_launch("lbt_noise_fill");
}

extern "C" int lbt_update_ranges(int32_t* ranges, uint64_t* counters, const int32_t* bits, const float* target,
                                 size_t n, void* stream) {
  if (!ranges || !counters || !bits) return LBT_EINVAL;
  if (n == 0) return LBT_OK;
  LBT_REQUIRE_ARCH();
  update_ranges_kernel<<<(unsigned)((n + 127) / 128), 128, 0, reinterpret_cast<cudaStream_t>(stream)>>>(
      ranges, reinterpret_cast<unsigned long long*>(counters), bits, target, n);
  return check_launch("lbt_update_ranges");
}

extern "C" int lbt_step_advance(uint64_t* dev_step, void* stream) {
  if (!dev_step) return LBT_EINVAL;
  LBT_REQUIRE_ARCH();
  step_advance_kernel<<<1, 1, 0, reinterpret_cast<cudaStream_t>(stream)>>>(dev_step);
  return check_launch("lbt_step_advance");
}
```

lbt_b200/dfxp.py:

```python
import contextlib
import ctypes
import os
import math

import torch
import torch.nn as nn

from . import _lib, gemm as G, quantizer as Q




class Runtime:

    def __init__(self, seed=0):
        self.seed = int(seed)
        self.sites = []
        self.dev_step = None
        self.noise_fn = None
        self.flat = None
        self.grad_sink = None
        self.prep = None
        self._arena = None
        self._arena_off = 0
# ... 129 lines not shown
        self.flat = dict(ranges=ranges, counters=counters, bits=bits, target=target)
        self.dev_step = torch.zeros(1, dtype=torch.int64, device=device)
        return self

    def update_ranges(self):
        f = self.flat
        _lib.call('lbt_update_ranges', _lib.ptr(f['ranges']), _lib.ptr(f['counters']), _lib.ptr(f['bits']),
                                       _lib.ptr(f['target']), len(self.sites), _lib.stream())
        _lib.call('lbt_step_advance', _lib.ptr(self.dev_step), _lib.stream())
        self.close_step()

    def close_step(self):
        self.join_prep()
        self._arena_on = False
        self._prep_valid = False
        self._noise_valid = False

    def ranges(self):
        vals = self.flat['ranges'].cpu().tolist() if self.flat is not None else [int(s.range) for s in self.sites]
        return {s.name: v for s, v in zip(self.sites, vals)}


class ParamPrep:

    CHUNK = 4096

    def __init__(self, model, runtime, device):
        self.rt = runtime
        self.entries = {}
        self._njobs_of = {}
        self.head, self.head_blocks = set(), 0
        jobs = []

        def job(site, x, layout=0, **kw):
            n_outer, n_inner = Q.rows_view(x)
            j = _lib.PrepJob(x=x.data_ptr(), n_outer=n_outer, n_inner=n_inner, ib=site.range.data_ptr(),
                             counters=site.counters.data_ptr(), offset=Q.make_offset(site.qid, 0), bits=site.bits,
                             layout=layout, **kw)
            jobs.append(j)

        def vec(site, p):
            out = torch.empty_like(p.data)
            job(site, p.data, out_f32=out.data_ptr())
            return out

        for m in model.modules():
            n_before = len(jobs)
            if isinstance(m, Conv2d_q) and m.qW.bits <= 8:
                kh, kw, Cin, Cout = m.weight.shape
                e = {}
                c3 = bool(m.input_signed and m.qX.bits == 9 and Cin == 3 and m.implicit and _implicit_ok(Cout, 1, 1))
                Ka = kh * kw * (16 if c3 else Cin)
                e['c3'] = c3
                e['wt'] = torch.zeros(Cout, _pitch16(Ka), dtype=torch.int8, device=device)[:, :Ka]
                rot = bool(m.implicit and m.stride == (1, 1) and _implicit_ok(Cout, kh, kw) and not (kh == 1 and kw == 1))
                cls = _dgrad_classes_ok(m, Cin, Cout, kh, kw, m.stride[0], m.stride[1])
                K2 = kh * kw * Cout
                e['rot180'] = rot
                e['classes'] = cls
                e['w2'] = None if c3 else torch.zeros(Cin, _pitch16(K2), dtype=torch.int8, device=device)[:, :K2]
                job(m.qW, m.weight.data, layout=1, kh=kh, kw=kw, Cin=Cin, Cout=Cout, c3pad=int(c3), rot180=2 if cls else int(rot),
                    sh=m.stride[0], sw=m.stride[1],
                    out_a=e['wt'].data_ptr(), ld_a=e['wt'].stride(0),
                    out_b=0 if e['w2'] is None else e['w2'].data_ptr(), ld_b=0 if e['w2'] is None else e['w2'].stride(0))
                if m.bias is not None:
                    e['bq'] = vec(m.qb, m.bias)
                self.entries[m] = e
            elif isinstance(m, Linear_q) and m.qW.bits <= 8:
                In, Out = m.weight.shape
                e = {}
                e['wt'] = torch.zeros(Out, _pitch16(In), dtype=torch.int8, device=device)[:, :In]
                e['w2'] = torch.zeros(In, _pitch16(Out), dtype=torch.int8, device=device)[:, :Out]
                job(m.qW, m.weight.data, layout=2, Cin=In, Cout=Out, out_a=e['wt'].data_ptr(), ld_a=e['wt'].stride(0),
                    out_b=e['w2'].data_ptr(), ld_b=e['w2'].stride(0))
                if m.bias is not None:
                    e['bq'] = vec(m.qb, m.bias)
                self.entries[m] = e
            elif isinstance(m, Rescale_q):
                self.entries[m] = dict(gq=vec(m.qg, m.gamma), bq=vec(m.qb, m.beta))
            if m in self.entries:
                self._njobs_of[m] = len(jobs) - n_before
        self.njobs = len(jobs)
        if not jobs:
            return
        ents = list(self.entries)
        self.head = set(ents[:1])
        if len(ents) > 1 and isinstance(ents[1], Rescale_q):
            self.head.add(ents[1])
        head_jobs = sum(self._njobs_of[m] for m in self.head)
        bj, bc = [], []
        self.head_blocks = 0
        for i, j in enumerate(jobs):
            n = j.n_outer * j.n_inner
            for c in range(-(-n // self.CHUNK)):
                bj.append(i)
                bc.append(c)
            if i + 1 == head_jobs:
                self.head_blocks = len(bj)
        self.jobs_dev = _lib.to_device_table(jobs, device)
        self.block_job = torch.tensor(bj, dtype=torch.int32, device=device)
        self.block_chunk = torch.tensor(bc, dtype=torch.int32, device=device)
        self._keep = jobs

    def run(self, part=None):
        if not self.njobs:
            return
        rt = self.rt
        nb, hb = self.block_job.numel(), self.head_blocks
        lo, hi = (0, nb) if part is None else ((0, hb) if part == 'head' else (hb, nb))
        if hi <= lo:
            return
        _lib.call('lbt_param_prep', _lib.ptr(self.jobs_dev), self.block_job.data_ptr() + 4 * lo, self.block_chunk.data_ptr() + 4 * lo,
                  hi - lo, self.CHUNK, rt.seed, _lib.ptr(rt.dev_step), _lib.stream())


def _prepared(layer):
    rt = layer.qX.runtime
    if rt.prep is None or rt.noise_fn is not None or not getattr(rt, '_prep_valid', False):
        return None
    rt.join_prep(layer)
    return rt.prep.entries.get(layer)


def _emit_grad(rt, param, acc, *, ibA=None, ibB=None, exp_const=0, add_scale=0.0, shape=None):
    sink = rt.grad_sink
    if sink is not None and sink.accepts(param):
        sink.add(param, acc, ibA, ibB, exp_const, add_scale)
        return None
    g = G.acc64_finalize(acc, ibA=ibA, ibB=ibB, exp_const=exp_const, add=param.detach().reshape(-1) if add_scale else None,
                         add_scale=add_scale)
    return g.view(shape if shape is not None else param.shape)


_default_runtime = Runtime()


def default_runtime():
    return _default_runtime


class QuantSite(nn.Module):

    def __init__(self, runtime, name, bits, init_range=2, target_overflow_rate=0.0):
        super().__init__()
        assert 1 <= bits <= 32, 'invalid value for bits: %d' % bits
        self.runtime = runtime
        self.name = name
        self.bits = int(bits)
        self.target = float(target_overflow_rate)
        self.register_buffer('range', torch.tensor(int(init_range), dtype=torch.int32))
        self.register_buffer('counters', torch.zeros(Q.CNT_WORDS, dtype=torch.int64))
        runtime.register(self)

    def quantize(self, x, want_fp32=True, mant_kind=Q.MANT_NONE, out_mant=None):
        rt = self.runtime
        kw = dict(target_overflow_rate=self.target, want_fp32=want_fp32, mant_kind=mant_kind, counters=self.counters,
                  update_range=False, out_mant=out_mant)
        if rt.noise_fn is not None:
            n_inner = Q.rows_view(x)[1]
            kw.update(mode=Q.ROUND_NOISE, noise=rt.noise_fn(self, n_inner, x.device))
        else:
            kw.update(mode=Q.ROUND_PHILOX, seed=rt.seed, offset=Q.make_offset(self.qid, 0), dev_step=rt.dev_step)
        if self.target == 0.0:
            kw['mode'] |= Q.STATS_MINMAX
        return Q.quantize(x, self.bits, self.range, **kw)

    def abi(self, n_inner, device, arena=False):
        rt = self.runtime
        qs = _lib.QSiteStruct(bits=self.bits, stats_minmax=int(self.target == 0.0), ib=self.range.data_ptr(),
                              noise=0, seed=rt.seed, offset=Q.make_offset(self.qid, 0),
                              dev_step=_lib.ptr(rt.dev_step) or 0, counters=self.counters.data_ptr())
        if rt.noise_fn is not None:
            nz = rt.noise_fn(self, n_inner, device).contiguous()
            qs.noise, qs.offset = nz.data_ptr(), 0
            qs._keep = nz
        elif arena:
            nz = rt.noise_for(self, n_inner, device)
            if nz is not None:
                qs.noise = nz.data_ptr()
        return qs

    def extra_repr(self):
        return '%s bits=%d' % (self.name, self.bits)


class _QuantSTE(torch.autograd.Function):

    @staticmethod
    def forward(ctx, x, site):
        q, _ = site.quantize(x)
        return q

    @staticmethod
    def backward(ctx, dy):
        return dy, None


class _GradQuant(torch.autograd.Function):

    @staticmethod
    def forward(ctx, y, site):
        ctx.site = site
        return y.view_as(y)

    @staticmethod
    def backward(ctx, dy):
        dy = _mem_contig(dy)
        q, _ = ctx.site.quantize(dy)
        return q, None


def _require_cuda_f32(x, who):
    if not x.is_cuda or x.dtype != torch.float32:
        raise _lib.LbtError('%s: expects an fp32 CUDA tensor (got %s on %s); there is no CPU or PyTorch fallback'
                            % (who, x.dtype, x.device))


def _mem_contig(x):
    if x.dim() == 4:
        return x if x.is_contiguous(memory_format=torch.channels_last) else x.contiguous(memory_format=torch.channels_last)
    return x.contiguous()


def same_pad(in_size, k, s):
    out = -(-in_size // s)
    total = max((out - 1) * s + k - in_size, 0)
    return out, total // 2, total - total // 2


def _pitch16(k):
    return -(-k // 16) * 16


def _as_operand(t):
    rows, K = t.shape
    if t.stride(1) == 1 and t.stride(0) % 16 == 0 and t.data_ptr() % 16 == 0:
        return t
    buf = torch.zeros(rows, _pitch16(K), dtype=t.dtype, device=t.device)
    buf[:, :K] = t
    return buf[:, :K]


def _transpose_bytes(t):
    R, C = t.shape
    assert t.stride(1) == 1
    out = torch.empty(C, _pitch16(R), dtype=t.dtype, device=t.device)
    _lib.call('lbt_transpose_i8', _lib.ptr(t), R, C, t.stride(0), _lib.ptr(out), out.stride(0), _lib.stream())
    return out[:, :R]


def _im2col(src_nhwc, src_kind, OH, OW, kh, kw, sh, sw, pt, pl, transposed):
    N, H, W, C = src_nhwc.shape
    segs = 3 if src_kind == Q.MANT_S16 else 1
    K = kh * kw * C * segs
    M = N * OH * OW
    out = torch.empty(M, _pitch16(K), dtype=torch.int8 if src_kind != Q.MANT_U8 else torch.uint8, device=src_nhwc.device)
    _lib.call('lbt_im2col_i8', _lib.ptr(src_nhwc), src_kind, N, H, W, C, OH, OW, kh, kw, sh, sw, pt, pl,
                                        1 if transposed else 0, _lib.ptr(out), out.stride(0), _lib.stream())
    return out[:, :K]


def _colsum(mant2d, kind, rt=None):
    acc = (rt.zeros_i64(mant2d.shape[1], mant2d.device) if rt is not None
           else torch.zeros(mant2d.shape[1], dtype=torch.int64, device=mant2d.device))
    _lib.call('lbt_colsum_i', _lib.ptr(mant2d), kind, mant2d.shape[0], mant2d.shape[1], _lib.ptr(acc),
                                       _lib.stream())
    return acc


def _implicit_ok(C, kh, kw):
    return (C in (16, 32, 64) or (C >= 128 and C % 128 == 0)) and kh * kw * C <= 65536 and kh <= 255 and kw <= 255


def _gather_ok(C, Cout, kh, kw):
    if C not in (16, 32, 64) or not 1 <= Cout <= 128:
        return False
    kcp = (kh * kw * (C // 16) + 1) & ~1
    bn = 16 if Cout <= 16 else (32 if Cout <= 32 else (64 if Cout <= 64 else 128))
    return kcp * bn * 16 + 2 * 16384 + 1024 <= 200 * 1024 and kh * kw * C <= 65536 and kcp <= 256 and kh * kw <= 64 and kh <= 16 and kw <= 16


def _class_perm(kh, kw, sh, sw):
    perm = []
    for r0 in range(sh):
        for s0 in range(sw):
            for r in reversed(range(r0, kh, sh)):
                for s_ in reversed(range(s0, kw, sw)):
                    perm.append(r * kw + s_)
    return perm


DGRAD_CLASSES = True


def _dgrad_classes_ok(layer, Cin, Cout, kh, kw, sh, sw):
    if layer.qG.bits > 8:
        return (DGRAD_CLASSES and DUAL_HALO and layer.implicit and (sh, sw) != (1, 1) and sh <= 4 and sw <= 4 and layer.qG.bits <= 16 and
                layer.qW.bits <= 8 and (Cout == 64 or Cout % 128 == 0) and Cin >= 64 and Cin % 4 == 0)
    return (DGRAD_CLASSES and layer.implicit and (sh, sw) != (1, 1) and sh <= 4 and sw <= 4 and layer.qG.bits <= 8 and
            layer.qW.bits <= 8 and (Cout in (16, 32, 64) or Cout % 128 == 0) and Cin % 4 == 0 and
            not _gather_ok(Cout, Cin, kh, kw))


FUSE_POOL_FWD = os.environ.get('LBT_FUSE_POOL_FWD', '1') != '0'

STEM_WGRAD = os.environ.get('LBT_STEM_WGRAD', '1') != '0'

_W_PREPARED = 0x100 if os.environ.get('LBT_W_PREFETCH', '0') == '1' else 0


def _conv_implicit(src_nhwc, src_kind, wp, Cout, kh, kw, sh, sw, pt, pl, OH, OW, ib_src, ib_w, exp_const, bias, out2d,
                   bnq=None, addend=None, w_prepared=False):
    N, H, W, C = src_nhwc.shape
    qs, k_out, sums = bnq if bnq is not None else (None, None, None)
    _lib.call('lbt_conv_i8_fprop', _lib.ptr(src_nhwc), src_kind, N, H, W, C, _lib.ptr(wp), Q.MANT_S8 | (_W_PREPARED if w_prepared else 0),
              wp.stride(0), Cout,
              kh, kw, sh, sw, pt, pl, OH, OW, _lib.ptr(ib_src), _lib.ptr(ib_w), int(exp_const), _lib.ptr(bias),
              _lib.ptr(out2d), out2d.stride(0) if out2d is not None else Cout,
              ctypes.addressof(qs) if qs is not None else None, _lib.ptr(k_out), _lib.ptr(sums), _lib.ptr(addend), _lib.stream(),
              meta=dict(ops=2 * N * OH * OW * Cout * kh * kw * C,
                        bytes=N * H * W * C + Cout * kh * kw * C + N * OH * OW * Cout * (1 if qs is not None else 4)))




def _conv_geom(layer, x, weight):
    N, Cin, H, W = x.shape
    kh, kw, _, Cout = weight.shape
    sh, sw = layer.stride
    if layer.padding == 'SAME':
        OH, pt, _ = same_pad(H, kh, sh)
        OW, pl, _ = same_pad(W, kw, sw)
    else:
        pt = pl = layer.pad_int
        OH = (H + 2 * pt - kh) // sh + 1
        OW = (W + 2 * pl - kw) // sw + 1
    return (N, H, W, Cin, Cout, kh, kw, sh, sw, pt, pl, OH, OW)


def _conv_xkind(layer, geom):
    N, H, W, Cin, Cout, kh, kw = geom[:7]
    xb = layer.qX.bits
    if layer.qW.bits > 8 or xb > 16:
        raise _lib.LbtError('Conv2d_q: weights wider than 8 bits need the hi/lo GEMM split (not built yet)')
    if xb <= 8:
        return Q.MANT_S8
    if xb <= 9 and not layer.input_signed:
        return Q.MANT_U8
    if xb <= 9 and Cin == 3 and layer.implicit and kh * kw * 16 <= 65536 and _implicit_ok(Cout, 1, 1):
        return Q.MANT_S9C3
    return Q.MANT_S16


def _conv_quantize_input(layer, x, geom):
    xkind = _conv_xkind(layer, geom)
    pre = getattr(x, '_lbt_q', None)
    if pre is not None and id(layer.qX) in pre:
        xm, kind = pre[id(layer.qX)]
        assert kind == xkind, (kind, xkind)
        return xm, xkind
    if getattr(x, '_lbt_hollow', False):
        raise _lib.LbtError('Conv2d_q: got a mantissa-only activation made for a different quantiser')
    N, H, W = geom[:3]
    x_nhwc = _mem_contig(x).permute(0, 2, 3, 1)
    if xkind == Q.MANT_S9C3:
        xm = torch.empty(N, H, W, 16, dtype=torch.int8, device=x.device)
        layer.qX.quantize(x_nhwc, want_fp32=False, mant_kind=xkind, out_mant=xm)
        return xm, xkind
    _, xm = layer.qX.quantize(x_nhwc, want_fp32=False, mant_kind=xkind)
    return xm, xkind


def _stem_applies(geom):
    N, H, W, Cin, Cout, kh, kw, sh, sw = geom[:9]
    return STEM_WGRAD and sh == 2 and sw == 2 and kh <= 8 and kw <= 8 and Cout == 64 and H % 2 == 0


def _stem_work(layer, geom, dev):
    N, H, OW = geom[0], geom[1], geom[12]
    nb = int(_lib.lib().lbt_stem_pack8_bytes(N, H, OW))
    work = getattr(layer, '_stem_work8', None)
    if work is None or work.numel() != nb or work.device != torch.device(dev):
        work = layer._stem_work8 = torch.empty(nb, dtype=torch.int8, device=dev)
        layer._stem_packed = False
    return work, nb


def _stem_prepack(layer, xm, xkind, geom):
    rt = layer.qX.runtime
    if (xkind != Q.MANT_S9C3 or not _stem_applies(geom) or not torch.is_grad_enabled() or not layer.weight.requires_grad or
            not (rt.overlap and rt._arena_on and rt.grad_sink is not None and rt.grad_sink.active and _lib.profiler is None)):
        return
    N, H, W = geom[:3]
    dev = xm.device
    work, _ = _stem_work(layer, geom, dev)
    main, side = torch.cuda.current_stream(dev), rt.side_stream(dev)
    side.wait_stream(main)
    with torch.cuda.stream(side):
        layer._stem_packed = _lib.try_call('lbt_stem_pack8', _lib.ptr(xm), N, H, W, geom[12], geom[10], _lib.ptr(work), _lib.stream(),
                                           meta=dict(bytes=N * H * W * 16 + work.numel()))
    xm.record_stream(side)
    rt._side_pending = True


def _flush_head_beside(rt, fork, main, side):
    sink = rt.grad_sink
    if sink is None or not sink.active:
        return
    if fork:
        ev = torch.cuda.Event()
        ev.record(side)
        with torch.cuda.stream(main):
            main.wait_event(ev)
            sink.flush_head()
    else:
        sink.flush_head()


def _conv_params(layer, weight, bias):
    if not weight.is_contiguous():
        weight = weight.contiguous()
    prep = _prepared(layer)
    bq = wm = None
    if prep is None:
        _, wm = layer.qW.quantize(weight, want_fp32=False, mant_kind=Q.MANT_S8)
        if bias is not None:
            bq, _ = layer.qb.quantize(bias)
    else:
        bq = prep.get('bq')
    return prep, wm, bq


def _conv_fprop(layer, geom, xm, xkind, prep, wm, bq, out2d, bnq=None):
    N, H, W, Cin, Cout, kh, kw, sh, sw, pt, pl, OH, OW = geom
    e = -(layer.qX.bits - 1) - (layer.qW.bits - 1)
    Kf = kh * kw * Cin
    ibx, ibw = layer.qX.range, layer.qW.range
    if xkind == Q.MANT_S9C3:
        if prep is not None:
            wt = prep['wt']
        else:
            w3 = wm.view(kh * kw, 3, Cout)
            w16 = torch.cat([w3, w3, w3, torch.zeros(kh * kw, 7, Cout, dtype=torch.int8, device=xm.device)], dim=1)
            wt = _transpose_bytes(w16.view(kh * kw * 16, Cout))
        _conv_implicit(xm, Q.MANT_S8, wt, Cout, kh, kw, sh, sw, pt, pl, OH, OW, ibx, ibw, e, bq, out2d, bnq, w_prepared=prep is not None)
        return
    segs = 3 if xkind == Q.MANT_S16 else 1
    wt = prep['wt'] if prep is not None else _transpose_bytes(wm.view(Kf, Cout))
    if segs == 3:
        wt = _as_operand(torch.cat([wt, wt, wt], dim=1))
    gbnq = None if bnq is None else (bnq[0], bnq[1], bnq[2], OH * OW)
    if kh == 1 and kw == 1 and sh == 1 and sw == 1 and segs == 1 and Cin % 16 == 0 and pt == 0 and pl == 0:
        G.gemm_i8(xm.reshape(N * H * W, Cin), wt, ibA=ibx, ibB=ibw, exp_const=e, bias=bq, out=out2d, bnq=gbnq)
    elif layer.implicit and segs == 1 and _implicit_ok(Cin, kh, kw):
        _conv_implicit(xm, xkind, wt, Cout, kh, kw, sh, sw, pt, pl, OH, OW, ibx, ibw, e, bq, out2d, bnq,
                       w_prepared=prep is not None)
    else:
        A = _im2col(xm, xkind, OH, OW, kh, kw, sh, sw, pt, pl, False)
        G.gemm_i8(A, wt, ibA=ibx, ibB=ibw, exp_const=e, bias=bq, out=out2d, bnq=gbnq)


def _conv_backward(layer, geom, xm, xkind, wm, prep, gm, need_dx, need_dw, need_db, addend=None, link=None):
    N, H, W, Cin, Cout, kh, kw, sh, sw, pt, pl, OH, OW = geom
    xb, wb, gb = layer.qX.bits, layer.qW.bits, layer.qG.bits
    dev = gm.device
    M = N * OH * OW
    g2 = gm.view(M, Cout)
    Kf = kh * kw * Cin
    dW = db = dx = None
    rt = layer.qX.runtime
    fork = need_dw and rt.overlap and rt._arena_on and rt.grad_sink is not None and rt.grad_sink.active and _lib.profiler is None
    main = torch.cuda.current_stream(dev) if fork else None
    side = rt.side_stream(dev) if fork else None
    if fork:
        side.wait_stream(main)
    if need_dw:
      with (torch.cuda.stream(side) if fork else contextlib.nullcontext()):
          acc = rt.zeros_i64(Kf * Cout, dev).view(Kf, Cout)
          at = gt = None
          if xkind == Q.MANT_S9C3:
              if not _implicit_ok(Cout, 1, 1):
                  raise _lib.LbtError('first-layer implicit wgrad needs Cout in {16,32,64} or a multiple of 128')
              done = False
              _flush_head_beside(rt, fork, main, side)
              if _stem_applies(geom):
                  work, nb = _stem_work(layer, geom, dev)
                  repack = 0 if getattr(layer, '_stem_packed', False) else 1
                  layer._stem_packed = False
                  acc8 = rt.zeros_i64(512 * Cout, dev)
                  done = _lib.try_call('lbt_conv_i8_wgrad_c3', _lib.ptr(xm), N, H, W, _lib.ptr(g2), Q.MANT_S8, Cout, kh, kw, pt, pl,
                                       OH, OW, _lib.ptr(work), repack, _lib.ptr(acc8), 1, _lib.stream(),
                                       meta=dict(ops=2 * M * Cout * Kf, bytes=N * H * W * 16 + nb + M * Cout + 8 * 512 * Cout))
                  if done:
                      a = acc8.view(8, 8, 8, Cout)[:kh, :kw]
                      acc = (2 * a[:, :, 0:3] + a[:, :, 4:7]).reshape(Kf, Cout).contiguous()
              if not done:
                  acc16 = rt.zeros_i64(kh * kw * 16 * Cout, dev).view(kh * kw * 16, Cout)
                  _lib.call('lbt_conv_i8_wgrad', _lib.ptr(xm), Q.MANT_S8, N, H, W, 16, _lib.ptr(g2), Q.MANT_S8, Cout, kh, kw,
                            sh, sw, pt, pl, OH, OW, _lib.ptr(acc16), 1, 0, _lib.stream(),
                            meta=dict(ops=2 * M * Cout * Kf, bytes=N * H * W * 16 + M * Cout + 8 * kh * kw * 16 * Cout))
                  a = acc16.view(kh * kw, 16, Cout)
                  acc = (a[:, 0:3] + a[:, 3:6] + a[:, 6:9]).reshape(Kf, Cout).contiguous()
          elif layer.implicit and xkind != Q.MANT_S16 and _implicit_ok(Cin, kh, kw) and _implicit_ok(Cout, 1, 1):
              _lib.call('lbt_conv_i8_wgrad', _lib.ptr(xm), xkind, N, H, W, Cin, _lib.ptr(g2), Q.MANT_S8, Cout, kh, kw,
                        sh, sw, pt, pl, OH, OW, _lib.ptr(acc), 1, 0, _lib.stream(),
                        meta=dict(ops=2 * M * Cout * Kf, bytes=N * H * W * Cin + M * Cout + 8 * Kf * Cout))
          else:
              gt = _transpose_bytes(g2)
              A = _im2col(xm, xkind, OH, OW, kh, kw, sh, sw, pt, pl, False)
              at = _transpose_bytes(A)
          if at is None:
              pass
          elif xkind == Q.MANT_S16:
              G.gemm_i8_acc64(at[:Kf], gt, acc, alpha=2)
              G.gemm_i8_acc64(at[2 * Kf:], gt, acc, alpha=1)
          else:
              G.gemm_i8_acc64(at, gt, acc, alpha=1)
          dW = _emit_grad(rt, layer.weight, acc, ibA=layer.qX.range, ibB=layer.qG.range, exp_const=-(xb - 1) - (gb - 1),
                          add_scale=2 * layer.weight_decay, shape=(kh, kw, Cin, Cout))
    if need_db:
        db = _emit_grad(rt, layer.bias, _colsum(g2, Q.MANT_S8, rt), ibA=layer.qG.range, exp_const=-(gb - 1))
    linked = False
    if (need_dx and link is not None and link.k1 is not None and addend is None and layer.implicit and sh == 1 and sw == 1 and
            kh * kw > 1 and _implicit_ok(Cout, kh, kw) and tuple(link.k1.shape) == (N, H, W, Cin)):
        K2 = kh * kw * Cout
        pw2 = prep['w2'] if prep is not None else None
        w2 = pw2 if pw2 is not None else _as_operand(wm.flip(0, 1).permute(2, 0, 1, 3).reshape(Cin, K2))
        rt = layer.qX.runtime
        kg1 = torch.empty_like(link.k1)
        bsums = rt.zeros_i64(4 * Cin + 2, dev)
        ls = link.struct(H * W * Cin, dev, kg1, bsums)
        linked = _lib.try_call('lbt_conv_i8_dgrad_bn', _lib.ptr(gm), Q.MANT_S8, N, OH, OW, Cout, _lib.ptr(w2),
                               Q.MANT_S8 | (_W_PREPARED if pw2 is not None else 0), w2.stride(0), Cin, kh, kw, kh - 1 - pt, kw - 1 - pl, H, W, _lib.ptr(layer.qG.range),
                               _lib.ptr(layer.qW.range), int(-(gb - 1) - (wb - 1)), ctypes.addressof(ls), _lib.stream(),
                               meta=dict(ops=2 * N * H * W * Cin * K2, bytes=N * OH * OW * Cout + Cin * K2 + 3 * N * H * W * Cin))
        if linked:
            global _link_count
            _link_count += 1
            link.kg1, link.bsums, link.done = kg1, bsums, True
            dx = torch.empty(1, dtype=torch.float32, device=dev).expand(N, H, W, Cin)
    if need_dx and not linked:
        K2 = kh * kw * Cout
        dx = torch.empty(N, H, W, Cin, dtype=torch.float32, device=dev)
        ad2 = addend.reshape(N * H * W, Cin) if addend is not None else None
        e = -(gb - 1) - (wb - 1)
        pw2 = prep['w2'] if prep is not None else None
        if prep is not None and pw2 is None:
            raise _lib.LbtError('Conv2d_q: no input gradient for a 3-channel first-layer convolution')
        if kh == 1 and kw == 1 and sh == 1 and sw == 1 and Cout % 16 == 0 and pt == 0 and pl == 0:
            w2 = pw2 if pw2 is not None else _as_operand(wm.view(Cin, Cout))
            G.gemm_i8(g2, w2, ibA=layer.qG.range, ibB=layer.qW.range, exp_const=e, out=dx.view(N * H * W, Cin), addend=ad2)
        elif layer.implicit and sh == 1 and sw == 1 and _implicit_ok(Cout, kh, kw):
            w2 = pw2 if pw2 is not None else _as_operand(wm.flip(0, 1).permute(2, 0, 1, 3).reshape(Cin, K2))
            _conv_implicit(gm, Q.MANT_S8, w2, Cin, kh, kw, 1, 1, kh - 1 - pt, kw - 1 - pl, H, W, layer.qG.range,
                           layer.qW.range, e, None, dx.view(N * H * W, Cin), addend=ad2, w_prepared=pw2 is not None)
        elif layer.implicit and _gather_ok(Cout, Cin, kh, kw) and sh <= 4 and sw <= 4:
            w2 = pw2 if pw2 is not None else _as_operand(wm.view(kh * kw, Cin, Cout).permute(1, 0, 2).reshape(Cin, K2))
            _lib.call('lbt_conv_i8_dgrad', _lib.ptr(gm), Q.MANT_S8, N, OH, OW, Cout, _lib.ptr(w2),
                      Q.MANT_S8 | (_W_PREPARED if pw2 is not None else 0), w2.stride(0),
                      Cin, kh, kw, sh, sw, pt, pl, H, W, _lib.ptr(layer.qG.range), _lib.ptr(layer.qW.range), int(e),
                      _lib.ptr(dx), Cin, _lib.ptr(ad2), _lib.stream(),
                      meta=dict(ops=2 * N * H * W * Cin * K2, bytes=N * OH * OW * Cout + Cin * K2 + N * H * W * Cin * 4))
        elif (prep['classes'] if prep is not None else _dgrad_classes_ok(layer, Cin, Cout, kh, kw, sh, sw)):
            if pw2 is not None:
                w2 = pw2
            else:
                perm = torch.tensor(_class_perm(kh, kw, sh, sw), device=dev)
                w2 = _as_operand(wm.view(kh * kw, Cin, Cout).index_select(0, perm).permute(1, 0, 2).reshape(Cin, K2))
            _lib.call('lbt_conv_i8_dgrad_strided', _lib.ptr(gm), Q.MANT_S8, N, OH, OW, Cout, _lib.ptr(w2),
                      Q.MANT_S8 | (_W_PREPARED if pw2 is not None else 0), w2.stride(0),
                      Cin, kh, kw, sh, sw, pt, pl, H, W, _lib.ptr(layer.qG.range), _lib.ptr(layer.qW.range), int(e),
                      _lib.ptr(dx), Cin, _lib.ptr(ad2), _lib.stream(),
                      meta=dict(ops=2 * N * OH * OW * Cin * K2, bytes=N * OH * OW * Cout * min(sh * sw, kh * kw) + Cin * K2 + N * H * W * Cin * 4))
        else:
            w2 = pw2 if pw2 is not None else _as_operand(wm.view(kh * kw, Cin, Cout).permute(1, 0, 2).reshape(Cin, K2))
            A2 = _im2col(gm, Q.MANT_S8, H, W, kh, kw, sh, sw, pt, pl, True)
            G.gemm_i8(A2, w2, ibA=layer.qG.range, ibB=layer.qW.range, exp_const=e, out=dx.view(N * H * W, Cin), addend=ad2)
    if fork:
        for t in (xm, gm):
            t.record_stream(side)
        rt._side_pending = True
    return dx, dW, db


def _check_layer_bits(who, bits, grad_bits):
    if not 2 <= int(bits) <= 8:
        raise _lib.LbtError('%s: bits=%d — the integer tensor-core layers take 2..8-bit weights/activations '
                            '(gradients up to 16 bits via grad_bits); wider DFXP only through weight_quantization()' % (who, bits))
    if grad_bits is not None and not 2 <= int(grad_bits) <= 16:
        raise _lib.LbtError('%s: grad_bits=%d — gradient quantisers take 2..16 bits' % (who, grad_bits))


def _split16(gm16):
    hi = torch.empty(gm16.shape, dtype=torch.int8, device=gm16.device)
    lo = torch.empty(gm16.shape, dtype=torch.uint8, device=gm16.device)
    _lib.call('lbt_split_s16', _lib.ptr(gm16), gm16.numel(), _lib.ptr(hi), _lib.ptr(lo), _lib.stream(),
              meta=dict(bytes=gm16.numel() * 4))
    return hi, lo


def _conv_backward16(layer, geom, xm, xkind, wm, prep, hi, lo, need_dx, need_dw, need_db, gm16=None, addend=None):
    N, H, W, Cin, Cout, kh, kw, sh, sw, pt, pl, OH, OW = geom
    xb, wb, gb = layer.qX.bits, layer.qW.bits, layer.qG.bits
    dev = hi.device
    M = N * OH * OW
    Kf = kh * kw * Cin
    rt = layer.qX.runtime
    halves = ((hi, Q.MANT_S8, 256), (lo, Q.MANT_U8, 1))
    dW = db = dx = None
    fork = need_dw and rt.overlap and rt._arena_on and rt.grad_sink is not None and rt.grad_sink.active and _lib.profiler is None
    main = torch.cuda.current_stream(dev) if fork else None
    side = rt.side_stream(dev) if fork else None
    if fork:
        side.wait_stream(main)
    if need_dw:
      with (torch.cuda.stream(side) if fork else contextlib.nullcontext()):
        acc = rt.zeros_i64(Kf * Cout, dev).view(Kf, Cout)
        if xkind == Q.MANT_S9C3:
            if not _implicit_ok(Cout, 1, 1):
                raise _lib.LbtError('first-layer implicit wgrad needs Cout in {16,32,64} or a multiple of 128')
            done = False
            _flush_head_beside(rt, fork, main, side)
            if _stem_applies(geom):
                work, nb = _stem_work(layer, geom, dev)
                repack = 0 if getattr(layer, '_stem_packed', False) else 1
                layer._stem_packed = False
                acc8 = rt.zeros_i64(512 * Cout, dev)
                done = True
                for i, (g_, kind, alpha) in enumerate(halves):
                    done = done and _lib.try_call('lbt_conv_i8_wgrad_c3', _lib.ptr(xm), N, H, W, _lib.ptr(g_), kind, Cout, kh, kw, pt,
                                                  pl, OH, OW, _lib.ptr(work), repack if i == 0 else 0, _lib.ptr(acc8), alpha, _lib.stream(),
                                                  meta=dict(ops=M * Cout * Kf, bytes=(N * H * W * 16 + nb if i == 0 else 0) + nb + M * Cout))
                if done:
                    a = acc8.view(8, 8, 8, Cout)[:kh, :kw]
                    acc = (2 * a[:, :, 0:3] + a[:, :, 4:7]).reshape(Kf, Cout).contiguous()
            if not done:
                acc16 = rt.zeros_i64(kh * kw * 16 * Cout, dev).view(kh * kw * 16, Cout)
                for g_, kind, alpha in halves:
                    _lib.call('lbt_conv_i8_wgrad', _lib.ptr(xm), Q.MANT_S8, N, H, W, 16, _lib.ptr(g_), kind, Cout, kh, kw, sh, sw,
                              pt, pl, OH, OW, _lib.ptr(acc16), alpha, 0, _lib.stream(),
                              meta=dict(ops=M * Cout * Kf, bytes=N * H * W * 16 + M * Cout + 8 * kh * kw * 16 * Cout))
                a = acc16.view(kh * kw, 16, Cout)
                acc = (a[:, 0:3] + a[:, 3:6] + a[:, 6:9]).reshape(Kf, Cout).contiguous()
        elif layer.implicit and xkind != Q.MANT_S16 and _implicit_ok(Cin, kh, kw) and _implicit_ok(Cout, 1, 1):
            done = DUAL_WGRAD and _lib.try_call('lbt_conv_i8_wgrad_dual', _lib.ptr(xm), xkind, N, H, W, Cin, _lib.ptr(hi), _lib.ptr(lo),
                                                Cout, kh, kw, sh, sw, pt, pl, OH, OW, _lib.ptr(acc), 1, 0, _lib.stream(),
                                                meta=dict(ops=2 * M * Cout * Kf, bytes=N * H * W * Cin + 2 * M * Cout + 8 * Kf * Cout))
            for g_, kind, alpha in (() if done else halves):
                _lib.call('lbt_conv_i8_wgrad', _lib.ptr(xm), xkind, N, H, W, Cin, _lib.ptr(g_), kind, Cout, kh, kw, sh, sw,
                          pt, pl, OH, OW, _lib.ptr(acc), alpha, 0, _lib.stream(),
                          meta=dict(ops=M * Cout * Kf, bytes=N * H * W * Cin + M * Cout + 8 * Kf * Cout))
        else:
            A = _im2col(xm, xkind, OH, OW, kh, kw, sh, sw, pt, pl, False)
            at = _transpose_bytes(A)
            for g_, kind, alpha in halves:
                gt = _transpose_bytes(g_.view(M, Cout))
                if xkind == Q.MANT_S16:
                    G.gemm_i8_acc64(at[:Kf], gt, acc, alpha=2 * alpha)
                    G.gemm_i8_acc64(at[2 * Kf:], gt, acc, alpha=alpha)
                else:
                    G.gemm_i8_acc64(at, gt, acc, alpha=alpha)
        dW = _emit_grad(rt, layer.weight, acc, ibA=layer.qX.range, ibB=layer.qG.range, exp_const=-(xb - 1) - (gb - 1),
                        add_scale=2 * layer.weight_decay, shape=(kh, kw, Cin, Cout))
    if need_db:
        if gm16 is None:
            raise _lib.LbtError('Conv2d_q: the bias gradient of a 16-bit gradient needs the s16 mantissas')
        db = _emit_grad(rt, layer.bias, _colsum(gm16.view(M, Cout), Q.MANT_S16, rt), ibA=layer.qG.range, exp_const=-(gb - 1))
    if need_dx:
        K2 = kh * kw * Cout
        e = -(gb - 1) - (wb - 1)
        pw2 = prep['w2'] if prep is not None else None
        if prep is not None and pw2 is None:
            raise _lib.LbtError('Conv2d_q: no input gradient for a 3-channel first-layer convolution')
        dx = torch.empty(N, H, W, Cin, dtype=torch.float32, device=dev)
        ad2 = addend.reshape(N * H * W, Cin) if addend is not None else None
        one_by_one = kh == 1 and kw == 1 and sh == 1 and sw == 1 and Cout % 16 == 0 and pt == 0 and pl == 0
        rot = bool(prep is not None and prep.get('rot180'))
        done = False
        if one_by_one:
            w2 = pw2 if pw2 is not None else _as_operand(wm.view(Cin, Cout))
            a_hi, a_lo = hi.view(M, Cout), lo.view(M, Cout)
        elif rot:
            w2 = pw2
            done = DUAL_HALO and _lib.try_call(
                'lbt_conv_i8_fprop_dual', _lib.ptr(hi), _lib.ptr(lo), N, OH, OW, Cout, _lib.ptr(w2),
                Q.MANT_S8, w2.stride(0), Cin, kh, kw, kh - 1 - pt, kw - 1 - pl, H, W, _lib.ptr(layer.qG.range),
                _lib.ptr(layer.qW.range), int(e), _lib.ptr(dx), Cin, _lib.ptr(ad2), _lib.stream(),
                meta=dict(ops=2 * 2 * N * H * W * Cin * K2, bytes=2 * N * OH * OW * Cout + Cin * K2 + N * H * W * Cin * 4))
            if not done:
                a_hi = _im2col(hi, Q.MANT_S8, H, W, kh, kw, 1, 1, kh - 1 - pt, kw - 1 - pl, False)
                a_lo = _im2col(lo, Q.MANT_U8, H, W, kh, kw, 1, 1, kh - 1 - pt, kw - 1 - pl, False)
        elif prep is not None and prep.get('classes'):
            _lib.call('lbt_conv_i8_dgrad_strided_dual', _lib.ptr(hi), _lib.ptr(lo), N, OH, OW, Cout, _lib.ptr(pw2), Q.MANT_S8,
                      pw2.stride(0), Cin, kh, kw, sh, sw, pt, pl, H, W, _lib.ptr(layer.qG.range), _lib.ptr(layer.qW.range), int(e),
                      _lib.ptr(dx), Cin, _lib.ptr(ad2), _lib.stream(),
                      meta=dict(ops=2 * 2 * N * OH * OW * Cin * K2, bytes=2 * N * OH * OW * Cout * min(sh * sw, kh * kw) + Cin * K2 + N * H * W * Cin * 4))
            done = True
        else:
            w2 = pw2 if pw2 is not None else _as_operand(wm.view(kh * kw, Cin, Cout).permute(1, 0, 2).reshape(Cin, K2))
            a_hi = _im2col(hi, Q.MANT_S8, H, W, kh, kw, sh, sw, pt, pl, True)
            a_lo = _im2col(lo, Q.MANT_U8, H, W, kh, kw, sh, sw, pt, pl, True)
        if not done:
            G.gemm_i8_dual(a_hi, a_lo, w2, ibA=layer.qG.range, ibB=layer.qW.range, exp_const=e, out=dx.view(N * H * W, Cin), addend=ad2)
    if fork:
        for t in (xm, hi, lo):
            t.record_stream(side)
        rt._side_pending = True
    return dx, dW, db


class _QConv2dFn(torch.autograd.Function):

    @staticmethod
    def forward(ctx, x, weight, bias, layer):
        geom = _conv_geom(layer, x, weight)
        N, H, W, Cin, Cout, kh, kw, sh, sw, pt, pl, OH, OW = geom
        xm, xkind = _conv_quantize_input(layer, x, geom)
        prep, wm, bq = _conv_params(layer, weight, bias)
        _stem_prepack(layer, xm, xkind, geom)
        y = torch.empty(N, OH, OW, Cout, dtype=torch.float32, device=x.device)
        _conv_fprop(layer, geom, xm, xkind, prep, wm, bq, y.view(N * OH * OW, Cout))
        ctx.layer, ctx.geom, ctx.xkind, ctx.prep = layer, geom, xkind, prep
        ctx.save_for_backward(xm, wm)
        return y.permute(0, 3, 1, 2)

    @staticmethod
    def backward(ctx, dy):
        layer = ctx.layer
        xm, wm = ctx.saved_tensors
        dy = _mem_contig(dy).permute(0, 2, 3, 1)
        needs = (ctx.needs_input_grad[0], ctx.needs_input_grad[1], layer.qb is not None and ctx.needs_input_grad[2])
        if layer.qG.bits > 8:
            if layer.qG.bits > 16:
                raise _lib.LbtError('Conv2d_q: gradient quantisers wider than 16 bits are not supported')
            _, gm16 = layer.qG.quantize(dy, want_fp32=False, mant_kind=Q.MANT_S16)
            hi, lo = _split16(gm16)
            dx, dW, db = _conv_backward16(layer, ctx.geom, xm, ctx.xkind, wm, ctx.prep, hi, lo, *needs, gm16=gm16)
            return (dx.permute(0, 3, 1, 2) if dx is not None else None), dW, db, None
        _, gm = layer.qG.quantize(dy, want_fp32=False, mant_kind=Q.MANT_S8)
        dx, dW, db = _conv_backward(layer, ctx.geom, xm, ctx.xkind, wm, ctx.prep, gm, ctx.needs_input_grad[0],
                                    ctx.needs_input_grad[1], layer.qb is not None and ctx.needs_input_grad[2])
        return (dx.permute(0, 3, 1, 2) if dx is not None else None), dW, db, None


class Conv2d_q(nn.Module):

    def __init__(self, bits, in_channels, out_channels, kernel_size, stride=1, padding='SAME', bias=True, *,
                 weight_decay=0.0, target_overflow_rate=0.0, input_range=2, weight_range=2, bias_range=2, grad_range=2,
                 grad_bits=None, input_signed=True, name='conv', runtime=None, implicit=True):
        super().__init__()
        rt = runtime or default_runtime()
        _check_layer_bits('Conv2d_q', bits, grad_bits)
        kh, kw = (kernel_size, kernel_size) if isinstance(kernel_size, int) else kernel_size
        self.stride = (stride, stride) if isinstance(stride, int) else tuple(stride)
        if isinstance(padding, str):
            assert padding in ('SAME', 'VALID')
            self.padding, self.pad_int = ('SAME', 0) if padding == 'SAME' else ('INT', 0)
        else:
            self.padding, self.pad_int = 'INT', int(padding)
        self.bits, self.weight_decay, self.input_signed, self.name = bits, float(weight_decay), input_signed, name
        self.implicit = implicit
        self.fuse_bn = True
        limit = (3 / (kh * kw * in_channels)) ** 0.5
        self.weight = nn.Parameter(torch.empty(kh, kw, in_channels, out_channels).uniform_(-limit, limit))
        self.bias = nn.Parameter(torch.zeros(out_channels)) if bias else None
        self.qX = QuantSite(rt, name + '/X', bits + 1, input_range, target_overflow_rate)
        self.qW = QuantSite(rt, name + '/W', bits, weight_range, target_overflow_rate)
        self.qb = QuantSite(rt, name + '/b', bits, bias_range, target_overflow_rate) if bias else None
        self.qG = QuantSite(rt, name + '/grad', grad_bits or bits, grad_range, target_overflow_rate)

    def forward(self, x):
# ... 958 lines not shown
```

lbt_b200/quantizer.py:

```python
import torch

from . import _lib

ROUND_NEAREST, ROUND_NOISE, ROUND_PHILOX = 0, 1, 2
STATS_MINMAX = 0x100
MANT_NONE, MANT_S8, MANT_U8, MANT_S16, MANT_S9C3 = 0, 1, 2, 3, 4
_MANT_DTYPE = {MANT_S8: torch.int8, MANT_U8: torch.uint8, MANT_S16: torch.int16}
_MANT_BYTES = {MANT_NONE: 0, MANT_S8: 1, MANT_U8: 1, MANT_S16: 2, MANT_S9C3: 6}
CNT_WORDS = 4


def rows_view(x):
    if x.dim() == 0:
        return 1, 1
    if not (x.is_contiguous() or (x.dim() == 4 and x.is_contiguous(memory_format=torch.channels_last))):
        raise _lib.LbtError('lbt_b200.quantize needs a contiguous (or channels_last) tensor')
    n_outer = x.shape[0]
    n_inner = x.numel() // n_outer if n_outer else 0
    return n_outer, n_inner


def new_counters(device):
    return torch.zeros(CNT_WORDS, dtype=torch.int64, device=device)


def quantize(x, bits, integer_bits, *, target_overflow_rate=0.0, mode=ROUND_NEAREST, noise=None, seed=0, offset=0,
             dev_step=None, want_fp32=True, mant_kind=MANT_NONE, counters=None, update_range=True, out=None,
             out_mant=None):
    if x.dtype != torch.float32:
        raise _lib.LbtError('DFXP quantiser takes fp32 input (like the reference), got %s' % x.dtype)
    if integer_bits.dtype != torch.int32:
        raise _lib.LbtError('integer_bits must be an int32 CUDA tensor')
    n_outer, n_inner = rows_view(x)
    if want_fp32 and out is None:
        out = torch.empty_like(x)
    if mant_kind != MANT_NONE and out_mant is None:
        out_mant = torch.empty_like(x, dtype=_MANT_DTYPE[mant_kind])
    if counters is None and update_range:
        counters = new_counters(x.device)
    if noise is not None:
        if noise.numel() != n_inner or noise.dtype != torch.float32:
            raise _lib.LbtError('noise must be fp32 with X.shape[1:] elements (%d), got %d' % (n_inner, noise.numel()))
        noise = noise.contiguous()
    _lib.call('lbt_quantize', _lib.ptr(x), n_outer, n_inner, int(bits), _lib.ptr(integer_bits),
                              float(target_overflow_rate), int(mode), _lib.ptr(noise), int(seed), int(offset),
                              _lib.ptr(dev_step), _lib.ptr(out) if want_fp32 else None, _lib.ptr(out_mant),
                              int(mant_kind), _lib.ptr(counters), 1 if update_range else 0, _lib.stream(),
              meta=dict(bytes=n_outer * n_inner * (4 + (4 if want_fp32 else 0) + _MANT_BYTES[int(mant_kind)])))
    return (out if want_fp32 else None), out_mant


class _QuantizeSTE(torch.autograd.Function):

    @staticmethod
    def forward(ctx, x, bits, integer_bits, target, mode, noise, seed, offset):
        q, _ = quantize(x, bits, integer_bits, target_overflow_rate=target, mode=mode, noise=noise, seed=seed,
                        offset=offset)
        return q

    @staticmethod
    def backward(ctx, dy):
        return dy, None, None, None, None, None, None, None


def weight_quantization(X, target_overflow_rate, bits, integer_bits, stochastic=False, *, noise=None, seed=0,
                        offset=0):
    assert 1 <= bits <= 32, 'invalid value for bits: %d' % bits
    if bits == 32:
        return X
    mode = ROUND_NEAREST if not stochastic else (ROUND_NOISE if noise is not None else ROUND_PHILOX)
    return _QuantizeSTE.apply(X, bits, integer_bits, float(target_overflow_rate), mode, noise, seed, offset)


def _counts(X, bits, integer_bits):
    cnt = new_counters(X.device)
    quantize(X, int(bits), integer_bits, want_fp32=False, counters=cnt, update_range=False)
    return cnt


def overflow_rate(X, bits, integer_bits):
    cnt = _counts(X, bits, integer_bits)
    n = cnt[2].clamp(min=1).to(torch.float32)
    return cnt[0].to(torch.float32) / n, cnt[1].to(torch.float32) / n


def update_range(X, target_overflow_rate, bits, integer_bits):
    quantize(X, int(bits), integer_bits, target_overflow_rate=target_overflow_rate, want_fp32=False,
             update_range=True)
    return integer_bits


def noise_fill(n_inner, seed, offset, device='cuda', dev_step=None):
    u = torch.empty(int(n_inner), dtype=torch.float32, device=device)
    _lib.call('lbt_noise_fill', _lib.ptr(u), int(n_inner), int(seed), int(offset), _lib.ptr(dev_step),
                                         _lib.stream())
    return u


def make_offset(qid, step=0):
    return ((int(step) & 0xFFFFFFFF) << 32) | (int(qid) & 0xFFFFFFFF)
```

Before: 32400.

## Add packed 8-byte stem input format with dedicated tcgen05 stem fprop kernel

Introduces a new S9P8 mantissa format for the 3-channel first conv layer. The image is quantized straight into the packed 8-byte stem layout, and a new warp-specialized tcgen05 stem fprop kernel consumes it with TMA loads, multi-stage TMEM accumulators and optional fused noise/BN-quantize epilogue. The same packed buffer is reused by wgrad_c3 without a repack. This removes the 16-byte padded mantissa, the separate pack pass and the generic implicit-conv path for the stem, at the cost of a large new kernel and a new quantize entry point.

```diff
diff --git a/include/lbt.h b/include/lbt.h
--- a/include/lbt.h
+++ b/include/lbt.h
@@ -32,6 +32,7 @@
   LBT_MANT_U8 = 2,
   LBT_MANT_S16 = 3,
   LBT_MANT_S9C3 = 4,
+  LBT_MANT_S9P8 = 5,
   LBT_MANT_PREPARED = 0x100
 };
 
@@ -116,6 +117,9 @@
                            int64_t* acc64, int alpha, int k_splits, void* stream);
 
 size_t lbt_stem_pack8_bytes(int N, int H, int OW);
+int lbt_quantize_image8(const float* x, int N, int H, int W, int OW, int pad_left, int bits, int32_t* integer_bits,
+                        float target_overflow_rate, int mode, const float* noise, uint64_t seed, uint64_t offset,
+                        const uint64_t* dev_step, int8_t* out8, uint64_t* counters, int update_range, void* stream);
 int lbt_stem_pack8(const int8_t* x16, int N, int H, int W, int OW, int pad_left, int8_t* work8, void* stream);
 int lbt_conv_i8_wgrad_c3(const int8_t* x16, int N, int H, int W, const void* g, int g_kind, int Cout, int kh, int kw,
                          int pad_top, int pad_left, int OH, int OW, int8_t* work8, int repack, int64_t* acc8, int alpha,
diff --git a/lbt_b200/_lib.py b/lbt_b200/_lib.py
--- a/lbt_b200/_lib.py
+++ b/lbt_b200/_lib.py
@@ -40,6 +40,8 @@
                                [c_void_p, c_int, c_int, c_void_p]),
     'lbt_stem_pack8_bytes': (c_size_t, [c_int, c_int, c_int]),
     'lbt_stem_pack8': (c_int, [c_void_p, c_int, c_int, c_int, c_int, c_int, c_void_p, c_void_p]),
+    'lbt_quantize_image8': (c_int, [c_void_p] + [c_int] * 6 + [c_void_p, c_float, c_int, c_void_p, c_u64, c_u64, c_void_p, c_void_p,
+                                                            c_void_p, c_int, c_void_p]),
     'lbt_conv_i8_wgrad_c3': (c_int, [c_void_p, c_int, c_int, c_int, c_void_p] + [c_int] * 8 + [c_void_p, c_int, c_void_p, c_int, c_void_p]),
     'lbt_split_s16': (c_int, [c_void_p, c_size_t, c_void_p, c_void_p, c_void_p]),
     'lbt_transpose_i8': (c_int, [c_void_p, c_size_t, c_size_t, c_size_t, c_void_p, c_size_t, c_void_p]),
diff --git a/lbt_b200/csrc/conv_i8.cu b/lbt_b200/csrc/conv_i8.cu
--- a/lbt_b200/csrc/conv_i8.cu
+++ b/lbt_b200/csrc/conv_i8.cu
@@ -618,6 +618,11 @@
   const bool w_prepared = (w_kind & LBT_MANT_PREPARED) != 0;
   w_kind &= ~LBT_MANT_PREPARED;
   const bool dual = src_lo != nullptr;
+  if (src_kind == LBT_MANT_S9P8) {
+    if (dual || remap) return LBT_EINVAL;
+    return stem_fprop_run(src, N, H, W, C, wp, w_kind, ldw, Cout, kh, kw, sh, sw, pad_top, pad_left, OH, OW, ib_src, ib_w, exp_const,
+                          bias, out, ldc, q_out, k_out, sums, addend, stream);
+  }
   if (!src || !wp) return LBT_EINVAL;
   if (dual && (q_out || bias || !out || src_kind != LBT_MANT_S8 || (reinterpret_cast<uintptr_t>(src_lo) & 15))) return LBT_EUNSUPPORTED;
   if (q_out) {
diff --git a/lbt_b200/csrc/conv_internal.h b/lbt_b200/csrc/conv_internal.h
--- a/lbt_b200/csrc/conv_internal.h
+++ b/lbt_b200/csrc/conv_internal.h
@@ -25,6 +25,10 @@
 void conv_halo_enable(int mode);
 int conv_halo_debug_error();
 int conv_stem_debug_error();
+int stem_fprop_run(const void* src, int N, int H, int W, int C, const void* wp, int w_kind, size_t ldw, int Cout, int kh, int kw,
+                   int sh, int sw, int pad_top, int pad_left, int OH, int OW, const int32_t* ib_src, const int32_t* ib_w, int exp_const,
+                   const float* bias, float* out, size_t ldc, const lbt_qsite* q_out, int8_t* k_out, int64_t* sums,
+                   const float* addend, void* stream);
 int conv_halo_run(const void* src, int src_kind, int N, int H, int W, int C, const void* wp, int w_kind, size_t ldw, int Cout, int kh,
                   int kw, int pt, int pl, int OH, int OW, const int32_t* ibA, const int32_t* ibB, int exp_const, const float* bias,
                   float* out, size_t ldc, const lbt_qsite* q_out, int8_t* k_out, int64_t* sums, const float* addend, void* stream,
diff --git a/lbt_b200/csrc/conv_stem.cu b/lbt_b200/csrc/conv_stem.cu
--- a/lbt_b200/csrc/conv_stem.cu
+++ b/lbt_b200/csrc/conv_stem.cu
@@ -1,6 +1,7 @@
 #include <atomic>
 
 #include "conv_internal.h"
+#include "qsite.cuh"
 #include "tcgen05.cuh"
 
 namespace lbt {
@@ -29,6 +30,13 @@
   uint32_t idesc;
 };
 
+__device__ __forceinline__ void tma_load_tiled_3d(const CUtensorMap* map, uint64_t* bar, void* dst, int c0, int c1, int c2) {
+  asm volatile(
+      "cp.async.bulk.tensor.3d.shared::cluster.global.mbarrier::complete_tx::bytes [%0], [%1, {%3, %4, %5}], [%2];" ::"r"(
+          smem_u32(dst)),
+      "l"(reinterpret_cast<uint64_t>(map)), "r"(smem_u32(bar)), "r"(c0), "r"(c1), "r"(c2)
+      : "memory");
+}
 __device__ __forceinline__ void tma_load_tiled_4d(const CUtensorMap* map, uint64_t* bar, void* dst, int c0, int c1, int c2, int c3) {
   asm volatile(
       "cp.async.bulk.tensor.4d.shared::cluster.global.mbarrier::complete_tx::bytes [%0], [%1, {%3, %4, %5, %6}], [%2];" ::"r"(
@@ -43,6 +51,8 @@
       "l"(reinterpret_cast<uint64_t>(map)), "r"(smem_u32(bar)), "r"(c0), "r"(c1), "r"(c2), "r"(c3), "r"(c4)
       : "memory");
 }
+
+__device__ __forceinline__ void fence_proxy_async_smem() { asm volatile("fence.proxy.async.shared::cta;" ::: "memory"); }
 
 __global__ void __launch_bounds__(256) stem_pack8_kernel(const uint4* __restrict__ x16, int H, int W, int Wp, int ml, size_t total,
                                                          uint2* __restrict__ out) {
@@ -182,6 +192,280 @@
   if (warp == 1) tmem_dealloc(tmem_base, kTmemCols);
 }
 
+constexpr int kFpSlots = 10;
+constexpr int kFpAccStages = 4;
+constexpr int kFpBN = 64;
+constexpr int kFpBBlock = kFpBN * kRowBytes;
+constexpr int kFpEpi = 8;
+constexpr int kFpThreads = 32 * (3 + kFpEpi);
+constexpr int kFpNoiseBytes = 128 * kFpBN * 4;
+constexpr int kFpNoiseBufs = 2;
+constexpr size_t kFpSmem = (size_t)2 * kTapRows * kFpBBlock + (size_t)kFpSlots * kBlock + (size_t)kFpNoiseBufs * kFpNoiseBytes + 1024;
+
+struct StemFpParams {
+  uint32_t tiles, tiles_x, tiles_img;
+  FastDiv d_tiles_x, d_tiles_img;
+  int pt;
+  uint32_t kh, kw, OH, OW, OHW, M;
+  const int8_t* wp;
+  uint32_t ldw;
+  const int32_t* ibA;
+  const int32_t* ibB;
+  int exp_const;
+  const float* bias;
+  float* out;
+  size_t ldc;
+  uint32_t idesc;
+  BnqParams bnq;
+};
+
+template <bool NZ>
+__global__ void __launch_bounds__(kFpThreads, 1)
+stem_fprop_kernel(const __grid_constant__ CUtensorMap tmX, const __grid_constant__ CUtensorMap tmN, const StemFpParams p) {
+  constexpr int kSub = kFpEpi / 4;
+  constexpr int G = 16;
+  extern __shared__ uint8_t smem_raw[];
+  uint8_t* smem = reinterpret_cast<uint8_t*>((reinterpret_cast<uintptr_t>(smem_raw) + 1023) & ~uintptr_t(1023));
+  uint8_t* sB = smem;
+  uint8_t* sA = smem + 2 * kTapRows * kFpBBlock;
+  uint8_t* sN = sA + kFpSlots * kBlock;
+  __shared__ __align__(8) uint64_t full_bar[kFpSlots];
+  __shared__ __align__(8) uint64_t empty_bar[kFpSlots];
+  __shared__ __align__(8) uint64_t tmem_full_bar[kFpAccStages];
+  __shared__ __align__(8) uint64_t tmem_empty_bar[kFpAccStages];
+  __shared__ __align__(8) uint64_t nz_full_bar[kFpNoiseBufs];
+  __shared__ __align__(8) uint64_t nz_empty_bar[kFpNoiseBufs];
+  __shared__ __align__(8) uint64_t b_bar;
+  __shared__ uint32_t tmem_slot;
+  __shared__ int s_abort;
+  __shared__ int s_stat[kFpEpi][2 * kFpBN];
+  __shared__ unsigned long long s_tot[2 * kFpBN];
+
+  const int warp = threadIdx.x >> 5, lane = threadIdx.x & 31;
+  if (threadIdx.x == 0) {
+    for (int s = 0; s < kFpSlots; ++s) {
+      mbar_init(&full_bar[s], 1);
+      mbar_init(&empty_bar[s], 1);
+    }
+    for (int s = 0; s < kFpAccStages; ++s) {
+      mbar_init(&tmem_full_bar[s], 1);
+      mbar_init(&tmem_empty_bar[s], kFpEpi);
+    }
+    for (int s = 0; s < kFpNoiseBufs; ++s) {
+      mbar_init(&nz_full_bar[s], 1);
+      mbar_init(&nz_empty_bar[s], kFpEpi);
+    }
+    mbar_init(&b_bar, 32 * kFpEpi);
+    s_abort = 0;
+    fence_barrier_init();
+    tma_prefetch_desc(&tmX);
+    if (NZ) tma_prefetch_desc(&tmN);
+  }
+  if (warp == 1) tmem_alloc(&tmem_slot, kFpAccStages * kFpBN);
+  for (uint32_t i = threadIdx.x; i < 2 * kFpBN; i += kFpThreads) s_tot[i] = 0ull;
+  pdl_trigger();
+  fence_before();
+  __syncthreads();
+  fence_after();
+  pdl_wait();
+  const uint32_t tmem_base = *reinterpret_cast<volatile uint32_t*>(&tmem_slot);
+  volatile int* abort_flag = &s_abort;
+
+  if (warp == 0) {
+    if (lane == 0) {
+      uint32_t slot = 0, phase = 0;
+      bool ok = true;
+      for (uint32_t tile = blockIdx.x; tile < p.tiles && ok; tile += gridDim.x) {
+        const uint32_t img = fastdiv(tile, p.d_tiles_img), t2 = tile - img * p.tiles_img;
+        const uint32_t ty = fastdiv(t2, p.d_tiles_x), tx = t2 - ty * p.tiles_x;
+        const int oh0 = (int)ty * kPatchOH, ow0 = (int)tx * kPatchOW;
+        for (uint32_t r = 0; r < p.kh; ++r) {
+          if (!(ok = mbar_wait(&empty_bar[slot], phase ^ 1, abort_flag, &g_stem_error))) break;
+          mbar_expect_tx(&full_bar[slot], (uint32_t)kBlock);
+          const int d = (int)r - p.pt;
+          tma_load_tiled_5d(&tmX, &full_bar[slot], sA + (size_t)slot * kBlock, 0, ow0, d & 1, oh0 + (d >> 1), (int)img);
+          if (++slot == kFpSlots) {
+            slot = 0;
+            phase ^= 1;
+          }
+        }
+      }
+    }
+  } else if (warp == 1) {
+    if (lane == 0) {
+      uint32_t slot = 0, phase = 0, acc = 0, acc_phase = 0;
+      bool ok = mbar_wait(&b_bar, 0, abort_flag, &g_stem_error);
+      fence_after();
+      const uint32_t sa0 = smem_u32(sA), sb0 = smem_u32(sB);
+      for (uint32_t tile = blockIdx.x; tile < p.tiles && ok; tile += gridDim.x) {
+        if (!(ok = mbar_wait(&tmem_empty_bar[acc], acc_phase ^ 1, abort_flag, &g_stem_error))) break;
+        fence_after();
+        const uint32_t d_tmem = tmem_base + acc * kFpBN;
+        for (uint32_t r = 0; r < p.kh; ++r) {
+          if (!(ok = mbar_wait(&full_bar[slot], phase, abort_flag, &g_stem_error))) break;
+          fence_after();
+          const uint32_t sa = sa0 + slot * kBlock, sb = sb0 + 2 * r * kFpBBlock;
+#pragma unroll
+          for (uint32_t k = 0; k < 2; ++k) {
+            const uint64_t da = make_desc_kmajor(sa + 32 * k, 2, 16);
+            umma_i8(d_tmem, da, make_desc_kmajor(sb + 32 * k, 2, 16), p.idesc, (r > 0 || k > 0) ? 1u : 0u);
+            umma_i8(d_tmem, da, make_desc_kmajor(sb + kFpBBlock + 32 * k, 2, 16), p.idesc, 1u);
+          }
+          umma_commit(&empty_bar[slot]);
+          if (++slot == kFpSlots) {
+            slot = 0;
+            phase ^= 1;
+          }
+        }
+        if (!ok) break;
+        umma_commit(&tmem_full_bar[acc]);
+        if (++acc == kFpAccStages) {
+          acc = 0;
+          acc_phase ^= 1;
+        }
+      }
+    }
+  } else if (warp == 2) {
+    if (NZ && lane == 0) {
+      uint32_t buf = 0, phase = 0;
+      bool ok = true;
+      for (uint32_t tile = blockIdx.x; tile < p.tiles && ok; tile += gridDim.x) {
+        const uint32_t img = fastdiv(tile, p.d_tiles_img), t2 = tile - img * p.tiles_img;
+        const uint32_t ty = fastdiv(t2, p.d_tiles_x), tx = t2 - ty * p.tiles_x;
+        if (!(ok = mbar_wait(&nz_empty_bar[buf], phase ^ 1, abort_flag, &g_stem_error))) break;
+        mbar_expect_tx(&nz_full_bar[buf], (uint32_t)kFpNoiseBytes);
+        uint8_t* dst = sN + (size_t)buf * kFpNoiseBytes;
+        tma_load_tiled_3d(&tmN, &nz_full_bar[buf], dst, 0, (int)(tx * kPatchOW), (int)(ty * kPatchOH));
+        tma_load_tiled_3d(&tmN, &nz_full_bar[buf], dst + kFpNoiseBytes / 2, 32, (int)(tx * kPatchOW), (int)(ty * kPatchOH));
+        if (++buf == kFpNoiseBufs) {
+          buf = 0;
+          phase ^= 1;
+        }
+      }
+    }
+  } else {
+    const uint32_t et = threadIdx.x - 96;
+    for (uint32_t i = et; i < 2 * p.kh * kFpBN * 16; i += 32 * kFpEpi) {
+      const uint32_t wd = i & 15u, co = (i >> 4) & (kFpBN - 1), blk = i >> 10;
+      const uint32_t r = blk >> 1, s = wd >> 1;
+      uint32_t v = 0u;
+      if (s < p.kw && !((blk & 1u) && (wd & 1u))) {
+        const int8_t* w = p.wp + (size_t)co * p.ldw + (r * p.kw + s) * 16;
+        v = (uint32_t)(uint8_t)__ldg(w) | ((uint32_t)(uint8_t)__ldg(w + 1) << 8) | ((uint32_t)(uint8_t)__ldg(w + 2) << 16);
+      }
+      const uint32_t chunk = (wd >> 2) ^ ((co >> 1) & 3u);
+      *reinterpret_cast<uint32_t*>(sB + blk * kFpBBlock + co * kRowBytes + chunk * 16 + (wd & 3u) * 4) = v;
+    }
+    fence_proxy_async_smem();
+    mbar_arrive(&b_bar);
+
+    const uint32_t quad = warp & 3;
+    const uint32_t half = (uint32_t)(warp - 3) >> 2;
+    int e = p.exp_const;
+    if (p.ibA) e += *p.ibA;
+    if (p.ibB) e += *p.ibB;
+    const float scale = exp2i(e);
+    const bool fused = p.bnq.q.bits != 0;
+    int* my_stat = s_stat[warp - 3];
+    BnqState bst;
+    bst.tiles = 0;
+    if (fused) {
+      bst.init(p.bnq);
+      for (int i = lane; i < 2 * kFpBN; i += 32) my_stat[i] = 0;
+      __syncwarp();
+    }
+    const uint32_t m = quad * 32 + lane, ohl = m >> 4, owl = m & 15u;
+    uint32_t acc = 0, acc_phase = 0, nbuf = 0, nphase = 0;
+    bool ok = true;
+    for (uint32_t tile = blockIdx.x; tile < p.tiles && ok; tile += gridDim.x) {
+      const uint32_t img = fastdiv(tile, p.d_tiles_img), t2 = tile - img * p.tiles_img;
+      const uint32_t ty = fastdiv(t2, p.d_tiles_x), tx = t2 - ty * p.tiles_x;
+      const uint32_t oy = ty * kPatchOH + ohl, ox = tx * kPatchOW + owl;
+      const bool rvalid = oy < p.OH && ox < p.OW;
+      const uint32_t pix = oy * p.OW + ox, row = img * p.OHW + pix;
+      if (fused && !NZ) {
+#pragma unroll 1
+        for (int c0 = G * (int)half; c0 < kFpBN; c0 += kSub * G) bnq_prefetch(p.bnq, pix, kFpBN, (uint32_t)c0, rvalid);
+      }
+      ok = mbar_wait(&tmem_full_bar[acc], acc_phase, abort_flag, &g_stem_error);
+      if (NZ) ok = ok && mbar_wait(&nz_full_bar[nbuf], nphase, abort_flag, &g_stem_error);
+      ok = __all_sync(0xffffffffu, ok);
+      if (!ok) break;
+      fence_after();
+      const uint32_t taddr = tmem_base + acc * kFpBN + ((quad * 32u) << 16);
+      if (fused && bst.tiles >= (uint32_t)kBnqFlushTiles) {
+        bnq_flush(p.bnq, my_stat, 0, kFpBN, kFpBN, lane);
+        bst.tiles = 0;
+      }
+      ++bst.tiles;
+#pragma unroll 1
+      for (int c = G * (int)half; c < kFpBN; c += kSub * G) {
+        uint32_t v[16];
+        tmem_ld16(taddr + c, v);
+        if (NZ) {
+          float4 u4[4];
+          const uint8_t* nrow = sN + (size_t)nbuf * kFpNoiseBytes + (c >> 5) * (kFpNoiseBytes / 2) + m * 128;
+#pragma unroll
+          for (int g = 0; g < 4; ++g) {
+            const float4 t = *reinterpret_cast<const float4*>(nrow + (((uint32_t)(((c & 31) >> 2) + g) ^ (m & 7u)) << 4));
+            u4[g] = rvalid ? t : make_float4(0.f, 0.f, 0.f, 0.f);
+          }
+          tmem_ld_wait();
+          bnq_chunk(p.bnq, bst, v, u4, scale, p.bias ? p.bias + c : nullptr, row, rvalid, (uint32_t)c, 16u, kFpBN, my_stat, kFpBN,
+                    (uint32_t)c, lane);
+          continue;
+        }
+        tmem_ld_wait();
+        if (fused) {
+          bnq_chunk<true>(p.bnq, bst, v, scale, p.bias ? p.bias + c : nullptr, row, pix, rvalid, (uint32_t)c, 16u, kFpBN, my_stat,
+                          kFpBN, (uint32_t)c, lane);
+          continue;
+        }
+        float f[16];
+#pragma unroll
+        for (int j = 0; j < 16; ++j) f[j] = __int2float_rn((int)v[j]) * scale;
+        if (p.bias) {
+#pragma unroll
+          for (int j = 0; j < 16; ++j) f[j] = __fadd_rn(f[j], __ldg(p.bias + c + j));
+        }
+        if (rvalid) {
+          float* o = p.out + (size_t)row * p.ldc + c;
+          if ((reinterpret_cast<uintptr_t>(o) & 15u) == 0) {
+#pragma unroll
+            for (int j = 0; j < 16; j += 4) *reinterpret_cast<float4*>(o + j) = make_float4(f[j], f[j + 1], f[j + 2], f[j + 3]);
+          } else {
+#pragma unroll
+            for (int j = 0; j < 16; ++j) o[j] = f[j];
+          }
+        }
+      }
+      fence_before();
+      __syncwarp();
+      if (lane == 0) {
+        mbar_arrive(&tmem_empty_bar[acc]);
+        if (NZ) mbar_arrive(&nz_empty_bar[nbuf]);
+      }
+      if (++acc == kFpAccStages) {
+        acc = 0;
+        acc_phase ^= 1;
+      }
+      if (++nbuf == kFpNoiseBufs) {
+        nbuf = 0;
+        nphase ^= 1;
+      }
+    }
+    if (fused && ok) {
+      bnq_flush_cta(p.bnq, my_stat, s_tot, 0, kFpBN, kFpBN, lane, et, 32 * kFpEpi, 1);
+      bnq_finish(p.bnq, bst, (unsigned long long)p.M * kFpBN, warp == 3, lane);
+    }
+  }
+
+  fence_before();
+  __syncthreads();
+  fence_after();
+  if (warp == 1) tmem_dealloc(tmem_base, kFpAccStages * kFpBN);
+}
+
 typedef CUresult (*EncodeTiledFn)(CUtensorMap*, CUtensorMapDataType, cuuint32_t, void*, const cuuint64_t*, const cuuint64_t*,
                                   const cuuint32_t*, const cuuint32_t*, CUtensorMapInterleave, CUtensorMapSwizzle,
                                   CUtensorMapL2promotion, CUtensorMapFloatOOBfill);
@@ -294,6 +578,103 @@
 }
 
 namespace lbt {
+
+int stem_fprop_run(const void* src, int N, int H, int W, int C, const void* wp, int w_kind, size_t ldw, int Cout, int kh, int kw,
+                   int sh, int sw, int pad_top, int pad_left, int OH, int OW, const int32_t* ib_src, const int32_t* ib_w, int exp_const,
+                   const float* bias, float* out, size_t ldc, const lbt_qsite* q_out, int8_t* k_out, int64_t* sums,
+                   const float* addend, void* stream) {
+  if (!src || !wp) return LBT_EINVAL;
+  if (q_out) {
+    if (!k_out || !sums || !q_out->ib) return LBT_EINVAL;
+    if (q_out->bits < 2 || q_out->bits > 8) return LBT_EUNSUPPORTED;
+  } else if (!out) {
+    return LBT_EINVAL;
+  }
+  if (w_kind != LBT_MANT_S8) return LBT_EINVAL;
+  if (N <= 0 || H <= 0 || W <= 0 || C != 3 || Cout <= 0 || kh <= 0 || kw <= 0 || OH <= 0 || OW <= 0 || pad_top < 0 || pad_left < 0)
+    return LBT_EINVAL;
+  if (!q_out && ldc < (size_t)Cout) return LBT_EINVAL;
+  if (ldw < (size_t)kh * kw * 16) return LBT_EINVAL;
+  if (sh != 2 || sw != 2 || kh > 8 || kw > 8 || Cout != kFpBN || (H & 1) || addend) return LBT_EUNSUPPORTED;
+  const int Wp = 2 * OW + 6;
+  if (pad_left + W > Wp) return LBT_EUNSUPPORTED;
+  if ((reinterpret_cast<uintptr_t>(src) & 15) || ((uint64_t)N * H * Wp * 8 >= (1ull << 40))) return LBT_EUNSUPPORTED;
+  LBT_REQUIRE_ARCH();
+  const DeviceInfo& di = device_info();
+  static EncodeTiledFn enc_tiled = reinterpret_cast<EncodeTiledFn>(stem_driver_fn("cuTensorMapEncodeTiled"));
+  if (!enc_tiled) return LBT_ECUDA;
+
+  StemFpParams p{};
+  p.tiles_x = (uint32_t)((OW + kPatchOW - 1) / kPatchOW);
+  const uint32_t tiles_y = (uint32_t)((OH + kPatchOH - 1) / kPatchOH);
+  p.tiles_img = p.tiles_x * tiles_y;
+  if ((uint64_t)N * p.tiles_img >= (1ull << 31) || (uint64_t)N * OH * OW >= (1ull << 31)) return LBT_EUNSUPPORTED;
+  p.tiles = (uint32_t)N * p.tiles_img;
+  p.d_tiles_x = make_fastdiv(p.tiles_x);
+  p.d_tiles_img = make_fastdiv(p.tiles_img);
+  p.pt = pad_top;
+  p.kh = (uint32_t)kh;
+  p.kw = (uint32_t)kw;
+  p.OH = (uint32_t)OH;
+  p.OW = (uint32_t)OW;
+  p.OHW = (uint32_t)(OH * OW);
+  p.M = (uint32_t)N * p.OHW;
+  p.wp = reinterpret_cast<const int8_t*>(wp);
+  p.ldw = (uint32_t)ldw;
+  p.ibA = ib_src;
+  p.ibB = ib_w;
+  p.exp_const = exp_const;
+  p.bias = bias;
+  p.out = out;
+  p.ldc = ldc;
+  p.idesc = tc::make_idesc_i8(true, true, false, false, kFpBN, kPix);
+  p.bnq.q = site_from_abi(q_out);
+  p.bnq.k = k_out;
+  p.bnq.sums = reinterpret_cast<long long*>(sums);
+  p.bnq.rows_per_image = p.OHW;
+
+  CUtensorMap tx;
+  {
+    const size_t pitch = (size_t)Wp * 8;
+    cuuint64_t gdim[5] = {64, (cuuint64_t)OW, 2, (cuuint64_t)(H / 2), (cuuint64_t)N};
+    cuuint64_t gstr[4] = {16, (cuuint64_t)pitch, (cuuint64_t)(2 * pitch), (cuuint64_t)((size_t)H * pitch)};
+    cuuint32_t box[5] = {64, (cuuint32_t)kPatchOW, 1, (cuuint32_t)kPatchOH, 1};
+    cuuint32_t estr[5] = {1, 1, 1, 1, 1};
+    CUresult r = enc_tiled(&tx, CU_TENSOR_MAP_DATA_TYPE_UINT8, 5, const_cast<void*>(src), gdim, gstr, box, estr,
+                           CU_TENSOR_MAP_INTERLEAVE_NONE, CU_TENSOR_MAP_SWIZZLE_64B, CU_TENSOR_MAP_L2_PROMOTION_L2_128B,
+                           CU_TENSOR_MAP_FLOAT_OOB_FILL_NONE);
+    if (r != CUDA_SUCCESS) return LBT_EUNSUPPORTED;
+  }
+  CUtensorMap tn{};
+  const bool nz = q_out && q_out->noise && !(reinterpret_cast<uintptr_t>(q_out->noise) & 15);
+  if (nz) {
+    cuuint64_t gdim[3] = {(cuuint64_t)kFpBN, (cuuint64_t)OW, (cuuint64_t)OH};
+    cuuint64_t gstr[2] = {(cuuint64_t)kFpBN * 4, (cuuint64_t)OW * kFpBN * 4};
+    cuuint32_t box[3] = {32, (cuuint32_t)kPatchOW, (cuuint32_t)kPatchOH};
+    cuuint32_t estr[3] = {1, 1, 1};
+    CUresult r = enc_tiled(&tn, CU_TENSOR_MAP_DATA_TYPE_FLOAT32, 3, const_cast<float*>(q_out->noise), gdim, gstr, box, estr,
+                           CU_TENSOR_MAP_INTERLEAVE_NONE, CU_TENSOR_MAP_SWIZZLE_128B, CU_TENSOR_MAP_L2_PROMOTION_L2_128B,
+                           CU_TENSOR_MAP_FLOAT_OOB_FILL_NONE);
+    if (r != CUDA_SUCCESS) return LBT_EUNSUPPORTED;
+  }
+  const unsigned grid = p.tiles < (uint32_t)di.sm_count ? p.tiles : (unsigned)di.sm_count;
+  cudaStream_t st = reinterpret_cast<cudaStream_t>(stream);
+  auto launch = [&](auto kern, bool (&attr_done)[16]) -> int {
+    if (!attr_done[di.device]) {
+      cudaError_t e = cudaFuncSetAttribute(kern, cudaFuncAttributeMaxDynamicSharedMemorySize, (int)kFpSmem);
+      if (e != cudaSuccess) {
+        set_cuda_error(e, "cudaFuncSetAttribute(stem_fprop_kernel)");
+        return LBT_ECUDA;
+      }
+      attr_done[di.device] = true;
+    }
+    launch_pdl(kern, grid, kFpThreads, kFpSmem, st, tx, tn, p);
+    return check_launch("lbt_conv_i8_fprop (stem, 8-byte pixels)");
+  };
+  static bool attr_nz[16] = {}, attr_plain[16] = {};
+  return nz ? launch(stem_fprop_kernel<true>, attr_nz) : launch(stem_fprop_kernel<false>, attr_plain);
+}
+
 int conv_stem_debug_error() {
   int v = 0, zero = 0;
   if (cudaMemcpyFromSymbol(&v, g_stem_error, sizeof(int)) != cudaSuccess) return -1;
diff --git a/lbt_b200/csrc/quantize.cu b/lbt_b200/csrc/quantize.cu
--- a/lbt_b200/csrc/quantize.cu
+++ b/lbt_b200/csrc/quantize.cu
@@ -26,6 +26,7 @@
   int update_range;
   uint32_t n_vec, chunks, rows_per_group;
   uint64_t total_tiles;
+  uint32_t img_h, img_w, wp, ml;
 };
 
 struct QConst {
@@ -213,7 +214,19 @@
   finish_stats(n1, n2, p, ib);
 }
 
-template <int MODE>
+__device__ __forceinline__ void store_p8(const QParams& p, size_t img, uint32_t pi, const int (&k)[3]) {
+  const uint32_t h = pi / p.img_w, w = pi - h * p.img_w;
+  uint2* row = reinterpret_cast<uint2*>(p.mant) + (img * p.img_h + h) * p.wp;
+  const uint32_t hi = ((uint32_t)(k[0] >> 1) & 0xffu) | (((uint32_t)(k[1] >> 1) & 0xffu) << 8) | (((uint32_t)(k[2] >> 1) & 0xffu) << 16);
+  const uint32_t lo = ((uint32_t)k[0] & 1u) | (((uint32_t)k[1] & 1u) << 8) | (((uint32_t)k[2] & 1u) << 16);
+  row[p.ml + w] = make_uint2(hi, lo);
+  if (w == 0)
+    for (uint32_t i = 0; i < p.ml; ++i) row[i] = make_uint2(0u, 0u);
+  if (w + 1 == p.img_w)
+    for (uint32_t i = p.ml + p.img_w; i < p.wp; ++i) row[i] = make_uint2(0u, 0u);
+}
+
+template <int MODE, bool P8>
 __global__ void __launch_bounds__(kThreads) quantize_c3_kernel(const QParams p) {
   const int ib = *reinterpret_cast<volatile const int32_t*>(p.ib);
   const QConst c = make_const(p.bits, ib);
@@ -236,6 +249,10 @@
       }
       k[ch] = __float2int_rn(quant1<MODE>(p.x[row * p.n_inner + col], u, c, n1, n2));
     }
+    if (P8) {
+      store_p8(p, row, (uint32_t)(j0 / 3), k);
+      continue;
+    }
     uint32_t w[4] = {0, 0, 0, 0};
     uint8_t b[16];
 #pragma unroll
@@ -252,7 +269,7 @@
   finish_stats(n1, n2, p, ib);
 }
 
-template <int MODE>
+template <int MODE, bool P8>
 __global__ void __launch_bounds__(kThreads) quantize_c3v_kernel(const QParams p) {
   pdl_trigger();
   pdl_wait();
@@ -281,6 +298,11 @@
       int k[12];
 #pragma unroll
       for (int i = 0; i < 12; ++i) k[i] = __float2int_rn(quant1<MODE>(xs[i], u[i], c, n1, n2));
+      if (P8) {
+#pragma unroll
+        for (int q = 0; q < 4; ++q) store_p8(p, r, 4 * v + q, {k[3 * q], k[3 * q + 1], k[3 * q + 2]});
+        continue;
+      }
       uint4* o = reinterpret_cast<uint4*>(p.mant) + ((size_t)r * (nv4 / 3) * 4 + 4 * (size_t)v);
 #pragma unroll
       for (int q = 0; q < 4; ++q) {
@@ -367,10 +389,14 @@
   return LBT_OK;
 }
 
-extern "C" int lbt_quantize(const float* x, size_t n_outer, size_t n_inner, int bits, int32_t* integer_bits,
-                            float target_overflow_rate, int mode, const float* noise, uint64_t seed, uint64_t offset,
-                            const uint64_t* dev_step, float* out_fp32, void* out_mant, int mant_kind,
-                            uint64_t* counters, int update_range, void* stream) {
+namespace {
+struct Image8 {
+  uint32_t h, w, wp, ml;
+};
+
+int quantize_run(const float* x, size_t n_outer, size_t n_inner, int bits, int32_t* integer_bits, float target_overflow_rate, int mode,
+                 const float* noise, uint64_t seed, uint64_t offset, const uint64_t* dev_step, float* out_fp32, void* out_mant,
+                 int mant_kind, uint64_t* counters, int update_range, void* stream, const Image8* img8) {
   if (!x || !integer_bits) return LBT_EINVAL;
   if (bits < 1 || bits > 31) return LBT_EINVAL;
   const bool minmax = (mode & LBT_STATS_MINMAX) != 0 && target_overflow_rate == 0.0f && counters != nullptr;
@@ -378,8 +404,10 @@
   if (mode < 0 || mode > 2) return LBT_EINVAL;
   if (mode == LBT_ROUND_STOCHASTIC_NOISE && !noise) return LBT_EINVAL;
   if (!out_fp32 && !out_mant && !counters) return LBT_EINVAL;
-  if (out_mant && (mant_kind < LBT_MANT_S8 || mant_kind > LBT_MANT_S9C3)) return LBT_EINVAL;
-  if (mant_kind == LBT_MANT_S9C3 && (bits > 9 || n_inner % 3 != 0 || out_fp32 || (reinterpret_cast<uintptr_t>(out_mant) & 15)))
+  if (out_mant && (mant_kind < LBT_MANT_S8 || mant_kind > LBT_MANT_S9P8)) return LBT_EINVAL;
+  if ((mant_kind == LBT_MANT_S9P8) != (img8 != nullptr)) return LBT_EINVAL;
+  const bool c3 = mant_kind == LBT_MANT_S9C3 || mant_kind == LBT_MANT_S9P8;
+  if (c3 && (bits > 9 || n_inner % 3 != 0 || out_fp32 || !out_mant || (reinterpret_cast<uintptr_t>(out_mant) & 15)))
     return LBT_EINVAL;
   if (!out_mant) mant_kind = LBT_MANT_NONE;
   if (mant_kind == LBT_MANT_S8 && bits > 8) return LBT_EINVAL;
@@ -407,11 +435,18 @@
   p.mant_kind = mant_kind;
   p.counters = reinterpret_cast<unsigned long long*>(counters);
   p.update_range = update_range;
+  const bool p8 = img8 != nullptr;
+  if (p8) {
+    p.img_h = img8->h;
+    p.img_w = img8->w;
+    p.wp = img8->wp;
+    p.ml = img8->ml;
+  }
 
   const bool vec = (n_inner % 4 == 0) && (n_inner / 4 < 0xffffffffull) && aligned16(x) && (!out_fp32 || aligned16(out_fp32)) &&
                    (!out_mant || aligned16(out_mant)) && (mode != LBT_ROUND_STOCHASTIC_NOISE || aligned16(noise));
   const uint64_t cap = (uint64_t)di.sm_count * (uint64_t)g_blocks_per_sm;
-  if (mant_kind == LBT_MANT_S9C3 && vec && n_inner % 12 == 0 && n_outer < (1ull << 31)) {
+  if (c3 && vec && n_inner % 12 == 0 && n_outer < (1ull << 31)) {
     p.n_vec = (uint32_t)(n_inner / 12);
     p.chunks = (p.n_vec + kThreads - 1) / kThreads;
     uint64_t groups = ((uint64_t)di.sm_count * 8 + p.chunks - 1) / p.chunks;
@@ -422,20 +457,20 @@
     p.total_tiles = (uint64_t)p.chunks * ((n_outer + rpg - 1) / rpg);
     const unsigned grid = (unsigned)(p.total_tiles < cap ? p.total_tiles : cap);
     switch (mode) {
-      case LBT_ROUND_NEAREST: launch_pdl(quantize_c3v_kernel<0>, grid, kThreads, 0, st, p); break;
-      case LBT_ROUND_STOCHASTIC_NOISE: launch_pdl(quantize_c3v_kernel<1>, grid, kThreads, 0, st, p); break;
-      default: launch_pdl(quantize_c3v_kernel<2>, grid, kThreads, 0, st, p); break;
+      case LBT_ROUND_NEAREST: launch_pdl(p8 ? quantize_c3v_kernel<0, true> : quantize_c3v_kernel<0, false>, grid, kThreads, 0, st, p); break;
+      case LBT_ROUND_STOCHASTIC_NOISE: launch_pdl(p8 ? quantize_c3v_kernel<1, true> : quantize_c3v_kernel<1, false>, grid, kThreads, 0, st, p); break;
+      default: launch_pdl(p8 ? quantize_c3v_kernel<2, true> : quantize_c3v_kernel<2, false>, grid, kThreads, 0, st, p); break;
     }
     return check_launch("lbt_quantize(c3, 4 pixels per thread)");
   }
-  if (mant_kind == LBT_MANT_S9C3) {
+  if (c3) {
     const uint64_t npix = (uint64_t)n_outer * (n_inner / 3);
     const uint64_t blocks = (npix + kThreads - 1) / kThreads;
     const unsigned grid = (unsigned)(blocks < cap ? blocks : cap);
     switch (mode) {
-      case LBT_ROUND_NEAREST: quantize_c3_kernel<0><<<grid, kThreads, 0, st>>>(p); break;
-      case LBT_ROUND_STOCHASTIC_NOISE: quantize_c3_kernel<1><<<grid, kThreads, 0, st>>>(p); break;
-      default: quantize_c3_kernel<2><<<grid, kThreads, 0, st>>>(p); break;
+      case LBT_ROUND_NEAREST: (p8 ? quantize_c3_kernel<0, true> : quantize_c3_kernel<0, false>)<<<grid, kThreads, 0, st>>>(p); break;
+      case LBT_ROUND_STOCHASTIC_NOISE: (p8 ? quantize_c3_kernel<1, true> : quantize_c3_kernel<1, false>)<<<grid, kThreads, 0, st>>>(p); break;
+      default: (p8 ? quantize_c3_kernel<2, true> : quantize_c3_kernel<2, false>)<<<grid, kThreads, 0, st>>>(p); break;
     }
     return check_launch("lbt_quantize(c3)");
   }
@@ -483,6 +518,26 @@
     }
   }
   return check_launch("lbt_quantize");
+}
+}
+
+extern "C" int lbt_quantize(const float* x, size_t n_outer, size_t n_inner, int bits, int32_t* integer_bits,
+                            float target_overflow_rate, int mode, const float* noise, uint64_t seed, uint64_t offset,
+                            const uint64_t* dev_step, float* out_fp32, void* out_mant, int mant_kind,
+                            uint64_t* counters, int update_range, void* stream) {
+  return quantize_run(x, n_outer, n_inner, bits, integer_bits, target_overflow_rate, mode, noise, seed, offset, dev_step, out_fp32,
+                      out_mant, mant_kind, counters, update_range, stream, nullptr);
+}
+
+extern "C" int lbt_quantize_image8(const float* x, int N, int H, int W, int OW, int pad_left, int bits, int32_t* integer_bits,
+                                   float target_overflow_rate, int mode, const float* noise, uint64_t seed, uint64_t offset,
+                                   const uint64_t* dev_step, int8_t* out8, uint64_t* counters, int update_range, void* stream) {
+  if (!x || !out8) return LBT_EINVAL;
+  if (N <= 0 || H <= 0 || W <= 0 || OW <= 0 || pad_left < 0) return LBT_EINVAL;
+  const Image8 g{(uint32_t)H, (uint32_t)W, (uint32_t)(2 * OW + 6), (uint32_t)pad_left};
+  if ((uint64_t)pad_left + W > g.wp) return LBT_EUNSUPPORTED;
+  return quantize_run(x, (size_t)N, (size_t)H * W * 3, bits, integer_bits, target_overflow_rate, mode, noise, seed, offset, dev_step,
+                      nullptr, out8, LBT_MANT_S9P8, counters, update_range, stream, &g);
 }
 
 extern "C" int lbt_quantize_residual(const float* grad, size_t n_grad_rows, float* buffer, size_t n_outer, size_t n_inner, int bits,
diff --git a/lbt_b200/dfxp.py b/lbt_b200/dfxp.py
--- a/lbt_b200/dfxp.py
+++ b/lbt_b200/dfxp.py
@@ -305,10 +305,11 @@
         self.register_buffer('counters', torch.zeros(Q.CNT_WORDS, dtype=torch.int64))
         runtime.register(self)
 
-    def quantize(self, x, want_fp32=True, mant_kind=Q.MANT_NONE, out_mant=None):
+    def quantize(self, x, want_fp32=True, mant_kind=Q.MANT_NONE, out_mant=None, image8=None):
         rt = self.runtime
-        kw = dict(target_overflow_rate=self.target, want_fp32=want_fp32, mant_kind=mant_kind, counters=self.counters,
-                  update_range=False, out_mant=out_mant)
+        kw = dict(target_overflow_rate=self.target, counters=self.counters, update_range=False, out_mant=out_mant)
+        if image8 is None:
+            kw.update(want_fp32=want_fp32, mant_kind=mant_kind)
         if rt.noise_fn is not None:
             n_inner = Q.rows_view(x)[1]
             kw.update(mode=Q.ROUND_NOISE, noise=rt.noise_fn(self, n_inner, x.device))
@@ -316,6 +317,8 @@
             kw.update(mode=Q.ROUND_PHILOX, seed=rt.seed, offset=Q.make_offset(self.qid, 0), dev_step=rt.dev_step)
         if self.target == 0.0:
             kw['mode'] |= Q.STATS_MINMAX
+        if image8 is not None:
+            return Q.quantize_image8(x, self.bits, self.range, *image8, **kw)
         return Q.quantize(x, self.bits, self.range, **kw)
 
     def abi(self, n_inner, device, arena=False):
@@ -459,6 +462,8 @@
 
 STEM_WGRAD = os.environ.get('LBT_STEM_WGRAD', '1') != '0'
 
+STEM_FPROP = os.environ.get('LBT_STEM_FPROP', '1') != '0'
+
 _W_PREPARED = 0x100 if os.environ.get('LBT_W_PREFETCH', '0') == '1' else 0
 
 
@@ -501,7 +506,7 @@
     if xb <= 9 and not layer.input_signed:
         return Q.MANT_U8
     if xb <= 9 and Cin == 3 and layer.implicit and kh * kw * 16 <= 65536 and _implicit_ok(Cout, 1, 1):
-        return Q.MANT_S9C3
+        return Q.MANT_S9P8 if STEM_FPROP and _stem_applies(geom) else Q.MANT_S9C3
     return Q.MANT_S16
 
 
@@ -516,6 +521,8 @@
         raise _lib.LbtError('Conv2d_q: got a mantissa-only activation made for a different quantiser')
     N, H, W = geom[:3]
     x_nhwc = _mem_contig(x).permute(0, 2, 3, 1)
+    if xkind == Q.MANT_S9P8:
+        return layer.qX.quantize(x_nhwc.contiguous(), image8=(geom[12], geom[10])), xkind
     if xkind == Q.MANT_S9C3:
         xm = torch.empty(N, H, W, 16, dtype=torch.int8, device=x.device)
         layer.qX.quantize(x_nhwc, want_fp32=False, mant_kind=xkind, out_mant=xm)
@@ -589,14 +596,24 @@
     e = -(layer.qX.bits - 1) - (layer.qW.bits - 1)
     Kf = kh * kw * Cin
     ibx, ibw = layer.qX.range, layer.qW.range
-    if xkind == Q.MANT_S9C3:
+    if xkind in (Q.MANT_S9C3, Q.MANT_S9P8):
         if prep is not None:
             wt = prep['wt']
         else:
             w3 = wm.view(kh * kw, 3, Cout)
             w16 = torch.cat([w3, w3, w3, torch.zeros(kh * kw, 7, Cout, dtype=torch.int8, device=xm.device)], dim=1)
             wt = _transpose_bytes(w16.view(kh * kw * 16, Cout))
-        _conv_implicit(xm, Q.MANT_S8, wt, Cout, kh, kw, sh, sw, pt, pl, OH, OW, ibx, ibw, e, bq, out2d, bnq, w_prepared=prep is not None)
+        if xkind == Q.MANT_S9C3:
+            _conv_implicit(xm, Q.MANT_S8, wt, Cout, kh, kw, sh, sw, pt, pl, OH, OW, ibx, ibw, e, bq, out2d, bnq,
+                           w_prepared=prep is not None)
+            return
+        qs, k_out, sums = bnq if bnq is not None else (None, None, None)
+        _lib.call('lbt_conv_i8_fprop', _lib.ptr(xm), Q.MANT_S9P8, N, H, W, Cin, _lib.ptr(wt), Q.MANT_S8, wt.stride(0), Cout,
+                  kh, kw, sh, sw, pt, pl, OH, OW, _lib.ptr(ibx), _lib.ptr(ibw), int(e), _lib.ptr(bq),
+                  _lib.ptr(out2d), out2d.stride(0) if out2d is not None else Cout,
+                  ctypes.addressof(qs) if qs is not None else None, _lib.ptr(k_out), _lib.ptr(sums), None, _lib.stream(),
+                  meta=dict(ops=2 * N * OH * OW * Cout * Kf,
+                            bytes=xm.numel() + Cout * kh * kw * 16 + N * OH * OW * Cout * (1 if qs is not None else 4)))
         return
     segs = 3 if xkind == Q.MANT_S16 else 1
     wt = prep['wt'] if prep is not None else _transpose_bytes(wm.view(Kf, Cout))
@@ -631,7 +648,15 @@
       with (torch.cuda.stream(side) if fork else contextlib.nullcontext()):
           acc = rt.zeros_i64(Kf * Cout, dev).view(Kf, Cout)
           at = gt = None
-          if xkind == Q.MANT_S9C3:
+          if xkind == Q.MANT_S9P8:
+              _flush_head_beside(rt, fork, main, side)
+              acc8 = rt.zeros_i64(512 * Cout, dev)
+              _lib.call('lbt_conv_i8_wgrad_c3', _lib.ptr(xm), N, H, W, _lib.ptr(g2), Q.MANT_S8, Cout, kh, kw, pt, pl,
+                        OH, OW, _lib.ptr(xm), 0, _lib.ptr(acc8), 1, _lib.stream(),
+                        meta=dict(ops=2 * M * Cout * Kf, bytes=xm.numel() + M * Cout + 8 * 512 * Cout))
+              a = acc8.view(8, 8, 8, Cout)[:kh, :kw]
+              acc = (2 * a[:, :, 0:3] + a[:, :, 4:7]).reshape(Kf, Cout).contiguous()
+          elif xkind == Q.MANT_S9C3:
               if not _implicit_ok(Cout, 1, 1):
                   raise _lib.LbtError('first-layer implicit wgrad needs Cout in {16,32,64} or a multiple of 128')
               done = False
@@ -769,7 +794,15 @@
     if need_dw:
       with (torch.cuda.stream(side) if fork else contextlib.nullcontext()):
         acc = rt.zeros_i64(Kf * Cout, dev).view(Kf, Cout)
-        if xkind == Q.MANT_S9C3:
+        if xkind == Q.MANT_S9P8:
+            _flush_head_beside(rt, fork, main, side)
+            acc8 = rt.zeros_i64(512 * Cout, dev)
+            for g_, kind, alpha in halves:
+                _lib.call('lbt_conv_i8_wgrad_c3', _lib.ptr(xm), N, H, W, _lib.ptr(g_), kind, Cout, kh, kw, pt, pl, OH, OW, _lib.ptr(xm),
+                          0, _lib.ptr(acc8), alpha, _lib.stream(), meta=dict(ops=M * Cout * Kf, bytes=xm.numel() + M * Cout))
+            a = acc8.view(8, 8, 8, Cout)[:kh, :kw]
+            acc = (2 * a[:, :, 0:3] + a[:, :, 4:7]).reshape(Kf, Cout).contiguous()
+        elif xkind == Q.MANT_S9C3:
             if not _implicit_ok(Cout, 1, 1):
                 raise _lib.LbtError('first-layer implicit wgrad needs Cout in {16,32,64} or a multiple of 128')
             done = False
diff --git a/lbt_b200/quantizer.py b/lbt_b200/quantizer.py
--- a/lbt_b200/quantizer.py
+++ b/lbt_b200/quantizer.py
@@ -4,7 +4,7 @@
 
 ROUND_NEAREST, ROUND_NOISE, ROUND_PHILOX = 0, 1, 2
 STATS_MINMAX = 0x100
-MANT_NONE, MANT_S8, MANT_U8, MANT_S16, MANT_S9C3 = 0, 1, 2, 3, 4
+MANT_NONE, MANT_S8, MANT_U8, MANT_S16, MANT_S9C3, MANT_S9P8 = 0, 1, 2, 3, 4, 5
 _MANT_DTYPE = {MANT_S8: torch.int8, MANT_U8: torch.uint8, MANT_S16: torch.int16}
 _MANT_BYTES = {MANT_NONE: 0, MANT_S8: 1, MANT_U8: 1, MANT_S16: 2, MANT_S9C3: 6}
 CNT_WORDS = 4
@@ -48,6 +48,32 @@
                               int(mant_kind), _lib.ptr(counters), 1 if update_range else 0, _lib.stream(),
               meta=dict(bytes=n_outer * n_inner * (4 + (4 if want_fp32 else 0) + _MANT_BYTES[int(mant_kind)])))
     return (out if want_fp32 else None), out_mant
+
+
+def image8_bytes(N, H, OW):
+    return int(_lib.lib().lbt_stem_pack8_bytes(N, H, OW))
+
+
+def quantize_image8(x, bits, integer_bits, OW, pad_left, *, target_overflow_rate=0.0, mode=ROUND_NEAREST, noise=None, seed=0,
+                    offset=0, dev_step=None, counters=None, update_range=True, out_mant=None):
+    if x.dtype != torch.float32 or x.dim() != 4 or x.shape[3] != 3 or not x.is_contiguous():
+        raise _lib.LbtError('quantize_image8 takes a contiguous fp32 NHWC image with 3 channels')
+    if integer_bits.dtype != torch.int32:
+        raise _lib.LbtError('integer_bits must be an int32 CUDA tensor')
+    N, H, W, _ = x.shape
+    if out_mant is None:
+        out_mant = torch.empty(image8_bytes(N, H, OW), dtype=torch.int8, device=x.device)
+    if counters is None and update_range:
+        counters = new_counters(x.device)
+    if noise is not None:
+        if noise.numel() != H * W * 3 or noise.dtype != torch.float32:
+            raise _lib.LbtError('noise must be fp32 with X.shape[1:] elements (%d), got %d' % (H * W * 3, noise.numel()))
+        noise = noise.contiguous()
+    _lib.call('lbt_quantize_image8', _lib.ptr(x), N, H, W, int(OW), int(pad_left), int(bits), _lib.ptr(integer_bits),
+              float(target_overflow_rate), int(mode), _lib.ptr(noise), int(seed), int(offset), _lib.ptr(dev_step),
+              _lib.ptr(out_mant), _lib.ptr(counters), 1 if update_range else 0, _lib.stream(),
+              meta=dict(bytes=x.numel() * 4 + out_mant.numel()))
+    return out_mant
 
 
 class _QuantizeSTE(torch.autograd.Function):
```

New measurement: 32570 (median of 6 runs). Within noise of the previous version (+0.5%).
